# wwood/CoverM

Measured on AMD Instinct MI355X. Metric: aligned reads/s through coverm contig (mean trimmed_mean covered_fraction variance), higher is better.
Workload: dtype i32 depth / u64 sums / f32 estimators

## Files before the change

### coverm_amd/csrc/covermhip.hip

```cpp
#include "pileup_kernels.hip.h"
#include "prep_lean.hip.h"
#include "genome_kernels.hip.h"
#include "ingest_kernels.hip.h"
#include "group_kernels.hip.h"
#include "sam_kernels.hip.h"

#include <algorithm>
#include <atomic>
#include <cstddef>
#include <chrono>
#include <cstdio>
#include <dlfcn.h>
#include <functional>
#include <sched.h>
#include <cstdlib>
#include <cstring>
#include <map>
#include <mutex>
#include <string>
#include <future>
#include <thread>
#include <vector>

#include "../../include/covermhip.h"
// ... 8 lines not shown
static_assert(sizeof(cov_contig_stats) == 128 && offsetof(cov_contig_stats, sum_identity_primary) == 40 && offsetof(cov_contig_stats, win_sum_d) == 56 &&
              offsetof(cov_contig_stats, first_record) == 88 && offsetof(cov_contig_stats, win_min_d) == 104 && offsetof(cov_contig_stats, hist_len) == 112 &&
              offsetof(cov_contig_stats, hist_off) == 120, "cov_contig_stats layout");
static_assert(sizeof(cov_summary) == 32 && offsetof(cov_summary, hist_total) == 24, "cov_summary layout");
static_assert(sizeof(cov_interval) == 24 && sizeof(cov_interval_stats) == 56, "interval struct layout");
static_assert(sizeof(cov_genome_stats) == 24 && sizeof(cov_genome_stats) == sizeof(covk::DevGenomeStats) && offsetof(cov_genome_stats, genome_len) == offsetof(covk::DevGenomeStats, genome_len) &&
              offsetof(cov_genome_stats, any_nonzero) == offsetof(covk::DevGenomeStats, any_nonzero), "cov_genome_stats mirrors the device struct");
static_assert(sizeof(cov_estimator) == sizeof(covk::DevEstimator) && offsetof(cov_estimator, contig_end_exclusion) == offsetof(covk::DevEstimator, excl) &&
              offsetof(cov_estimator, trim_max) == offsetof(covk::DevEstimator, trim_max) && COV_EST_MAX == covk::EST_MAX && COV_EST_ANIR == covk::EST_ANIR, "cov_estimator mirrors the device struct");

namespace {

#define HIPCHK(call)                                                                          \
    do {                                                                                      \
        hipError_t e_ = (call);                                                               \
        if (e_ != hipSuccess) {                                                               \
            char b_[512];                                                                     \
            snprintf(b_, sizeof b_, "%s failed: %s (%s:%d)", #call, hipGetErrorString(e_), __FILE__, __LINE__); \
            s->err = b_;                                                                      \
            return COV_ERR_HIP;                                                               \
        }                                                                                     \
    } while (0)

template <typename T>
struct DevBuf {
    T *p = nullptr;
    size_t cap = 0;
    hipError_t reserve(size_t n, hipStream_t st, size_t keep = 0) {
        if (n <= cap) return hipSuccess;
        size_t nc = std::max(n, cap + cap / 2);
        T *q = nullptr;
        hipError_t e = hipMalloc(&q, nc * sizeof(T));
        if (e != hipSuccess) return e;
        if (keep && p) {
            e = hipMemcpyAsync(q, p, keep * sizeof(T), hipMemcpyDeviceToDevice, st);
            if (e != hipSuccess) return e;
            e = hipStreamSynchronize(st);
            if (e != hipSuccess) return e;
        }
        if (p) (void)hipFree(p);
        p = q; cap = nc;
        return hipSuccess;
    }
    void release() { if (p) (void)hipFree(p); p = nullptr; cap = 0; }
};

std::string g_create_error;

bool cov_timing_on() { static const bool on = getenv("COVERM_CLI_TIMING") != nullptr; return on; }

}

extern "C" int covh_timing_on(void) { return cov_timing_on() ? 1 : 0; }

struct InflateKernel { int version = 3; int lz_version = 2; u32 round_blocks = 0; u64 carry = 16ull << 20; u64 cwin = 0; u32 ext_parts = covi::EXT_PARTS; };

struct cov_session {
    cov_config cfg{};
    hipStream_t stream = nullptr;
    std::string err;
    int tile = 1024;
    bool use_fast = true;
    int chunk_tiles = 8;
    int prep_kernel = 0;
    int est_lanes = -1;
    int fast_tables = 1;
    int n_cus = 256;

    uint32_t n_targets = 0;
    std::vector<uint32_t> h_tlen;
    std::vector<uint32_t> h_tile_first;
    uint32_t n_tiles = 0;
    DevBuf<u32> d_tlen, d_tile_contig, d_tile_start;
    DevBuf<u32> d_tile_first, d_tcnt, d_fov, d_tscan, d_ttop;
    DevBuf<u32> d_slow_list;
    uint32_t tile_shift = 10;
    DevBuf<u32> d_cx_list, d_cx_cnt, d_cx_cur, d_cx_scan, d_cx_top;
    DevBuf<uint2> d_cx_runs;
    DevBuf<DevContig> d_ctg_scratch;
    DevBuf<int32_t> d_depth_all; DevBuf<u64> d_depth_off; bool depth_all_valid = false;
    DevBuf<DevInterval> d_iv; DevBuf<DevIntervalStats> d_ivst; DevBuf<unsigned long long> d_ivhist; uint64_t ivhist_total = 0;
    DevBuf<uint8_t> d_mask;
    std::vector<uint8_t> h_mask;
    bool have_mask = false;
    bool have_genomes = false, gen_valid = false;
    bool lean_finish = false;
    bool in_spill = false;
    DevBuf<u64> d_order;
    uint32_t n_genomes = 0, n_gseg = 0;
    DevBuf<u32> d_grow, d_gtids, d_gseg_genome, d_gseg_start;
    DevBuf<DevGenome> d_genomes;
    DevBuf<u64> d_ghist, d_ghist_top;
    DevBuf<uint8_t> d_gout; uint8_t *h_gout = nullptr; size_t h_gout_cap = 0;
    DevBuf<uint8_t> d_res;
    DevBuf<DevContig> d_ctg;
    DevBuf<DevGlobal> d_glob;
    DevBuf<uint4> d_desc;
    DevBuf<uint8_t> d_gather; uint8_t *h_gather = nullptr; size_t h_gather_cap = 0; uint32_t gather_n = 0; size_t gather_block = 0;

    DevBuf<int32_t> s_tid, s_pos;
    DevBuf<uint16_t> s_flag;
    DevBuf<uint8_t> s_mapq, s_nmk;
    DevBuf<u32> s_nm, s_lseq, s_coff, s_cig;
    DevBuf<int32_t> s_mtid; DevBuf<u64> s_qh1; DevBuf<u32> s_qh2;
    bool want_mates = false;
    bool want_grouping = false;
// ... 53 lines not shown
    DevBuf<u64> g_result;
    DevBuf<covi::tokpos_t> g_tok, g_tok2;
    DevBuf<u32> g_ntok, g_ntok2;
    hipStream_t ing_aux = nullptr;
    hipStream_t ing_parse = nullptr;
    hipStream_t ing_ext = nullptr;
    hipEvent_t ing_inf_done[2] = {nullptr, nullptr}, ing_lz_done[2] = {nullptr, nullptr};
    hipEvent_t ing_ver_done[4] = {}, ing_ext_done[3] = {}, ing_cdone[3] = {};
    uint64_t ing_round_start = 0, ing_prev_end = 0, ing_ccap = 0;
    uint32_t ing_round_n = 0;
    int64_t ing_copy_cleared = -1;
    long long ing_key_lo = 0, ing_key_hi = 0x80000000ll;
    bool ing_search_first = false, ing_open_end = false, ing_fed_any = false;
    uint64_t ing_span_lo = 0, ing_span_hi = 0;
    uint64_t ing_tail_key = ~0ull;
    u64 *h_winres = nullptr;
    struct WinInfo { u64 N = 0; u32 n_seg = 0; u64 comp_end = 0; };
    WinInfo ing_win[4];
    uint32_t ing_batch = 0; int ing_check_crc = 1;
    uint32_t ing_extracted = 0;
    uint64_t ing_rec_total = 0, ing_cig_total = 0;
    uint32_t ing_fail = 0;
    uint64_t ing_fail_dbg[3] = {0, 0, 0};
    uint64_t ing_first_record = 0;
    uint64_t ing_launched = 0;
    covi::BgzfBlock *h_blocks = nullptr; size_t h_blocks_cap = 0;
    uint64_t ing_comp = 0, ing_infl = 0, ing_blocks = 0;
    bool ing_active = false;
    InflateKernel ing_K;
    hipStream_t ing_copy = nullptr;
    std::future<hipError_t> ing_prep;
    hipEvent_t ing_ev[COV_INGEST_SLOTS] = {}, ing_fed = nullptr;
    double ing_s_alloc = 0;
    double ing_s_part[4] = {0, 0, 0, 0};

    bool sam_active = false, sam_seen_record = false, sam_decode_timed = false;
    uint64_t sam_window = 0, sam_expected = 0, sam_lines = 0, sam_bytes = 0, sam_err_line = 0;
    uint32_t sam_err = 0, sam_k = 0;
    DevBuf<uint8_t> m_text[2], m_blob;
    DevBuf<u64> m_nl, m_tab, m_res, m_noff;
    DevBuf<u32> m_line_end, m_cnt, m_rec_idx, m_cig_idx, m_bsum[3], m_slots;
    samc::Table m_names{};
    hipEvent_t sam_buf_free[2] = {}, sam_ev[4] = {};
    float sam_ms = 0.f; uint32_t sam_launches = 0;

    bool finished = false;
    uint8_t *h_res = nullptr; size_t h_res_cap = 0;
    std::future<std::pair<uint8_t *, size_t>> h_res_prep;
    DevContig *h_ctg = nullptr;
    DevGlobal h_glob{};
    bool last_gen_all = false;
    uint64_t algo_bytes = 0;

    hipEvent_t ev[COV_K_COUNT][2] = {};
    hipEvent_t ev_begin[COV_K_COUNT] = {};
    int ev_fresh = -1;
    float k_ms[COV_K_COUNT] = {};
    uint32_t k_launches[COV_K_COUNT] = {};
};

cov_status spill_store(cov_session *s, bool &progress);

namespace {

size_t result_block_bytes(u32 n_targets) { return sizeof(DevGlobal) + (size_t)std::max<u32>(n_targets, 1) * sizeof(DevContig); }
static size_t result_host_bytes(const cov_session *s, u32 nT) {
    return result_block_bytes(nT) + (size_t)std::max<u32>(nT, 1) * (s->have_mask ? 1u : std::max<u32>(s->est.n, 1u)) * sizeof(float);
}
static void result_host_take(cov_session *s) {
    if (!s->h_res_prep.valid()) return;
    const std::pair<uint8_t *, size_t> r = s->h_res_prep.get();
    if (!r.first) return;
    if (r.second > s->h_res_cap) {
        if (s->h_res) (void)hipHostFree(s->h_res);
        s->h_res = r.first; s->h_res_cap = r.second;
    } else (void)hipHostFree(r.first);
}

hipError_t bind_result_block(cov_session *s, u32 n_targets) {
    hipError_t e = s->d_res.reserve(result_block_bytes(n_targets) + (size_t)std::max<u32>(n_targets, 1) * COV_EST_MAX * sizeof(float), s->stream);
    if (e != hipSuccess) return e;
    s->d_glob.p = reinterpret_cast<DevGlobal *>(s->d_res.p); s->d_glob.cap = 1;
    s->d_ctg.p = reinterpret_cast<DevContig *>(s->d_res.p + sizeof(DevGlobal)); s->d_ctg.cap = std::max<u32>(n_targets, 1);
    return hipSuccess;
}

Records records_of(const cov_session *s) {
    Records r{};
    if (s->adopted) {
        const cov_batch &b = s->adopted_batch;
        r.tid = b.tid; r.pos = b.pos; r.flag = b.flag; r.mapq = b.mapq; r.nm = b.nm; r.nm_kind = b.nm_kind;
        r.l_seq = b.l_seq; r.cigar_off = b.cigar_off; r.cigar = b.cigar;
    } else {
        r.tid = s->s_tid.p; r.pos = s->s_pos.p; r.flag = s->s_flag.p; r.mapq = s->s_mapq.p; r.nm = s->s_nm.p;
        r.nm_kind = s->s_nmk.p; r.l_seq = s->s_lseq.p; r.cigar_off = s->s_coff.p; r.cigar = s->s_cig.p;
    }
    r.n = (u32)s->n_records;
    r.cigar_end = s->adopted ? s->adopted_cig_end : (u32)s->n_cigar;
    return r;
}

__global__ void k_rebase_offsets(u32 *off, u32 n, u32 sub, u32 add) {
    u32 i = blockIdx.x * blockDim.x + threadIdx.x;
    if (i < n) off[i] = off[i] - sub + add;
}

__global__ void k_count_primary(const uint16_t *__restrict__ flag, u32 lo, u32 n, unsigned long long *out) {
    u32 cnt = 0;
    for (u64 i = (u64)lo + blockIdx.x * blockDim.x + threadIdx.x; i < n; i += (u64)gridDim.x * blockDim.x) cnt += (flag[i] & 0x900u) ? 0u : 1u;
    cnt = wave_sum_u32(cnt);
    if ((threadIdx.x & 63u) == 0u && cnt) atomicAdd(out, (unsigned long long)cnt);
}

cov_status append(cov_session *s, const cov_batch *b, bool from_device) {
    const uint64_t n = b->n_records;
    if (n == 0) return COV_OK;
    const hipMemcpyKind kind = from_device ? hipMemcpyDeviceToDevice : hipMemcpyHostToDevice;
    u32 off0 = 0, offn = 0;
    if (from_device) {
        HIPCHK(hipMemcpyAsync(&off0, b->cigar_off, 4, hipMemcpyDeviceToHost, s->stream));
        HIPCHK(hipMemcpyAsync(&offn, b->cigar_off + n, 4, hipMemcpyDeviceToHost, s->stream));
        HIPCHK(hipStreamSynchronize(s->stream));
    } else {
        off0 = b->cigar_off[0]; offn = b->cigar_off[n];
    }
    const uint64_t ncig = (uint64_t)offn - off0;
    if (s->n_records && (s->n_records + n > s->cap_records || s->n_cigar + ncig > s->cap_cigar) && s->n_records >= s->spill_retry_at) {
        bool progress = false;
        const cov_status sp = spill_store(s, progress);
        if (sp != COV_OK) return sp;
        s->spill_retry_at = progress ? 0 : 2 * s->n_records;
    }
    if (s->n_records + n >= 0xfffffff0ull) { s->err = "more than 2^32 records of one reference (or of one batch) in the record store"; return COV_ERR_INVALID_ARG; }
    if (s->n_cigar + ncig >= 0xfffffff0ull) { s->err = "more than 2^32 CIGAR words of one reference (or of one batch) in the record store"; return COV_ERR_INVALID_ARG; }
    const uint64_t R = s->n_records, N = R + n;
    hipStream_t st = s->stream;
    HIPCHK(s->s_tid.reserve(N, st, R)); HIPCHK(s->s_pos.reserve(N, st, R)); HIPCHK(s->s_flag.reserve(N, st, R));
    HIPCHK(s->s_mapq.reserve(N, st, R)); HIPCHK(s->s_nmk.reserve(N, st, R)); HIPCHK(s->s_nm.reserve(N, st, R));
    HIPCHK(s->s_lseq.reserve(N, st, R)); HIPCHK(s->s_coff.reserve(N + 1, st, R + 1));
    HIPCHK(s->s_cig.reserve(s->n_cigar + ncig + 1, st, s->n_cigar));
    HIPCHK(hipMemcpyAsync(s->s_tid.p + R, b->tid, n * 4, kind, st));
    HIPCHK(hipMemcpyAsync(s->s_pos.p + R, b->pos, n * 4, kind, st));
    HIPCHK(hipMemcpyAsync(s->s_flag.p + R, b->flag, n * 2, kind, st));
    HIPCHK(hipMemcpyAsync(s->s_mapq.p + R, b->mapq, n, kind, st));
    HIPCHK(hipMemcpyAsync(s->s_nmk.p + R, b->nm_kind, n, kind, st));
    HIPCHK(hipMemcpyAsync(s->s_nm.p + R, b->nm, n * 4, kind, st));
    HIPCHK(hipMemcpyAsync(s->s_lseq.p + R, b->l_seq, n * 4, kind, st));
    HIPCHK(hipMemcpyAsync(s->s_coff.p + R, b->cigar_off, (n + 1) * 4, kind, st));
    if (ncig) HIPCHK(hipMemcpyAsync(s->s_cig.p + s->n_cigar, b->cigar + off0, ncig * 4, kind, st));
    if (off0 != (u32)s->n_cigar) {
        const u32 cnt = (u32)(n + 1);
        hipLaunchKernelGGL(k_rebase_offsets, dim3((cnt + 255) / 256), dim3(256), 0, st, s->s_coff.p + R, cnt, off0,
                           (u32)s->n_cigar);
        HIPCHK(hipGetLastError());
    }
    s->n_records = N; s->n_cigar += ncig;
    s->finished = false;
    if (!from_device) HIPCHK(hipStreamSynchronize(st));
    return COV_OK;
}

void timing_events(cov_session *s) {
    if (s->ev[0][0]) return;
    for (int k = 0; k < COV_K_COUNT; k++)
        for (int j = 0; j < 2; j++) (void)hipEventCreate(&s->ev[k][j]);
}
void time_begin(cov_session *s, int k) {
    if (s->ev_fresh >= 0) { s->ev_begin[k] = s->ev[s->ev_fresh][1]; return; }
    (void)hipEventRecord(s->ev[k][0], s->stream); s->ev_begin[k] = s->ev[k][0];
}
void time_end(cov_session *s, int k) { (void)hipEventRecord(s->ev[k][1], s->stream); s->k_launches[k]++; s->ev_fresh = k; }

template <bool H, int TABLES>
void launch_fast_v(cov_session *s, const PileupArgs &a, u32 n_tiles) {
    const auto kern = TABLES == 1 ? &k_pileup_fast<H> : &k_pileup_fast2t<H>;
    const size_t smem = pileup_fast_smem_bytes(H, TABLES == 1 ? FAST_HB : FAST_HB7, TABLES);
    static std::atomic<int> occ_dev[64];
    std::atomic<int> &occ_slot = occ_dev[(unsigned)s->cfg.device & 63u];
    int occ = occ_slot.load(std::memory_order_relaxed);
    const u32 chunk = (u32)s->chunk_tiles;
    const u32 n_chunks = (n_tiles + chunk - 1) / chunk;
    if (!occ) {
        (void)hipFuncSetAttribute(reinterpret_cast<const void *>(kern), hipFuncAttributeMaxDynamicSharedMemorySize, (int)smem);
        int nb = 0;
        if (hipOccupancyMaxActiveBlocksPerMultiprocessor(&nb, reinterpret_cast<const void *>(kern), 256, smem) != hipSuccess || nb < 1) {
            (void)hipGetLastError();
            nb = (int)std::max<size_t>(1, std::min<size_t>(8, (160 * 1024) / smem));
        }
        occ = nb; occ_slot.store(nb, std::memory_order_relaxed);
    }
    const u32 wg_per_cu = 8u * (u32)occ;
    const u32 grid = std::max(1u, std::min((n_chunks + 3) / 4, (u32)s->n_cus * wg_per_cu));
    hipLaunchKernelGGL(kern, dim3(grid), dim3(256), smem, s->stream, a, n_tiles, chunk);
}
template <bool H>
void launch_fast_t(cov_session *s, const PileupArgs &a, u32 n_tiles) {
    if (s->fast_tables == 2) launch_fast_v<H, 2>(s, a, n_tiles);
    else launch_fast_v<H, 1>(s, a, n_tiles);
}

template <bool H, bool W>
void launch_stream_t(cov_session *s, const PileupArgs &a, u32 n_tiles, bool slow_list_only = false) {
    const size_t smem = pileup_stream_smem_bytes();
    static std::atomic<int> occ_dev[64];
    std::atomic<int> &occ_slot = occ_dev[(unsigned)s->cfg.device & 63u];
    int occ = occ_slot.load(std::memory_order_relaxed);
    const u32 chunk = (u32)s->chunk_tiles;
    const u32 n_chunks = (n_tiles + chunk - 1) / chunk;
    if (!occ) {
        (void)hipFuncSetAttribute(reinterpret_cast<const void *>(&k_pileup_stream<H, W>), hipFuncAttributeMaxDynamicSharedMemorySize, (int)smem);
        int nb = 0;
        if (hipOccupancyMaxActiveBlocksPerMultiprocessor(&nb, reinterpret_cast<const void *>(&k_pileup_stream<H, W>), 256, smem) != hipSuccess || nb < 1) {
            (void)hipGetLastError();
            nb = (int)std::max<size_t>(1, std::min<size_t>(8, (160 * 1024) / smem));
        }
        occ = nb; occ_slot.store(nb, std::memory_order_relaxed);
    }
    const u32 wg_per_cu = 8u * (u32)occ;
    if (slow_list_only) {
        hipLaunchKernelGGL((k_pileup_stream<H, W>), dim3((u32)s->n_cus), dim3(256), smem, s->stream, a, 0u, 1u,
                           (const u32 *)s->d_slow_list.p, (const u32 *)&s->d_glob.p->n_slow);
        return;
    }
    const u32 grid = std::max(1u, std::min((n_chunks + 3) / 4, (u32)s->n_cus * wg_per_cu));
    hipLaunchKernelGGL((k_pileup_stream<H, W>), dim3(grid), dim3(256), smem, s->stream, a, n_tiles, chunk, (const u32 *)nullptr,
                       (const u32 *)nullptr);
}
template <bool H, bool W>
void launch_any_pileup(cov_session *s, const PileupArgs &a, u32 n_tiles) {
    if (s->use_fast && !W) {
        launch_fast_t<H>(s, a, n_tiles);
        launch_stream_t<H, W>(s, a, n_tiles, true);
    } else launch_stream_t<H, W>(s, a, n_tiles);
}

PileupArgs pileup_args(cov_session *s) {
    PileupArgs a{};
    a.tile_contig = s->d_tile_contig.p; a.tile_start = s->d_tile_start.p; a.desc = s->d_desc.p;
    a.runs = s->d_runs.p; a.cx_runs = s->d_cx_runs.p; a.r = records_of(s); a.ctg = s->d_ctg.p; a.g = s->d_glob.p;
    a.hist_arena = s->d_arena.p; a.excl = s->cfg.contig_end_exclusion; a.depth_out = nullptr; a.tile_base = 0;
    return a;
}

}

extern "C" {

int cov_abi_version(void) { return COVERMHIP_ABI_VERSION; }

const char *cov_last_error(const cov_session *s) { return s ? s->err.c_str() : g_create_error.c_str(); }

static hipError_t ingest_prepare_(cov_session *s) {
    hipError_t e = hipSetDevice(s->cfg.device);
    if (e != hipSuccess || s->ing_copy) return e;
#define PREP(x) do { e = (x); if (e != hipSuccess) return e; } while (0)
    PREP(hipStreamCreateWithFlags(&s->ing_copy, hipStreamNonBlocking));
    for (int k = 0; k < COV_INGEST_SLOTS; k++) PREP(hipEventCreateWithFlags(&s->ing_ev[k], hipEventDisableTiming));
    PREP(hipEventCreateWithFlags(&s->ing_fed, hipEventDisableTiming));
    PREP(hipStreamCreateWithFlags(&s->ing_aux, hipStreamNonBlocking));
    PREP(hipStreamCreateWithFlags(&s->ing_parse, hipStreamNonBlocking));
    s->ing_ext = s->ing_parse;
    for (int k = 0; k < 2; k++) { PREP(hipEventCreateWithFlags(&s->ing_inf_done[k], hipEventDisableTiming)); PREP(hipEventCreateWithFlags(&s->ing_lz_done[k], hipEventDisableTiming)); }
    for (int k = 0; k < 4; k++) PREP(hipEventCreateWithFlags(&s->ing_ver_done[k], hipEventDisableTiming));
    for (int k = 0; k < 3; k++) { PREP(hipEventCreateWithFlags(&s->ing_ext_done[k], hipEventDisableTiming)); PREP(hipEventCreateWithFlags(&s->ing_cdone[k], hipEventDisableTiming)); }
    PREP(hipHostMalloc((void **)&s->h_winres, 4 * 8 * sizeof(u64), hipHostMallocDefault));
    {
        const size_t nc = (size_t)3 << 19;
        PREP(hipHostMalloc((void **)&s->h_blocks, nc * sizeof(covi::BgzfBlock), hipHostMallocDefault));
        s->h_blocks_cap = nc;
    }
    {
        static const std::vector<u32> crc_tables = [] { std::vector<u32> t(covi::crcw::TABLE_WORDS); covi::crcw::build_tables(t.data()); return t; }();
        PREP(s->g_crc_tab.reserve(covi::crcw::TABLE_WORDS, s->ing_copy));
        PREP(hipMemcpyAsync(s->g_crc_tab.p, crc_tables.data(), covi::crcw::TABLE_WORDS * sizeof(u32), hipMemcpyHostToDevice, s->ing_copy));
        PREP(hipStreamSynchronize(s->ing_copy));
    }
#undef PREP
    return hipSuccess;
}
static hipError_t ingest_prep_wait(cov_session *s) { return s->ing_prep.valid() ? s->ing_prep.get() : hipSuccess; }

cov_status cov_create(const cov_config *cfg, cov_session **out) {
    if (!cfg || !out) { g_create_error = "null argument"; return COV_ERR_INVALID_ARG; }
    *out = nullptr;
    const bool timing = cov_timing_on();
    const auto tc0 = std::chrono::steady_clock::now();
    auto stamp = [&](const char *what) { if (timing) fprintf(stderr, "[covermhip] cov_create: %s at %.4fs\n", what, std::chrono::duration<double>(std::chrono::steady_clock::now() - tc0).count()); };
    int ndev = 0;
    hipError_t e = hipGetDeviceCount(&ndev);
    stamp("hipGetDeviceCount (runtime initialised)");
    if (e != hipSuccess || ndev <= 0) {
        g_create_error = std::string("no usable HIP device: ") + hipGetErrorString(e) +
                         " (the engine has no CPU fallback)";
// ... 45 lines not shown
void cov_destroy(cov_session *s) {
    if (!s) return;
    (void)ingest_prep_wait(s);
    (void)hipSetDevice(s->cfg.device);
    if (s->stream) (void)hipStreamSynchronize(s->stream);
    s->d_tlen.release(); s->d_tile_contig.release(); s->d_tile_start.release(); s->d_mask.release();
    s->d_grow.release(); s->d_gtids.release(); s->d_gseg_genome.release(); s->d_gseg_start.release(); s->d_genomes.release(); s->d_ghist.release(); s->d_ghist_top.release(); s->d_order.release();
    s->d_gout.release(); if (s->h_gout) (void)hipHostFree(s->h_gout); s->h_gout = nullptr;
    s->d_tile_first.release(); s->d_tcnt.release(); s->d_fov.release(); s->d_tscan.release(); s->d_ttop.release(); s->d_slow_list.release();
    s->d_ctg_scratch.release(); s->d_depth_all.release(); s->d_depth_off.release(); s->d_iv.release(); s->d_ivst.release(); s->d_ivhist.release();
    s->d_cx_list.release(); s->d_cx_cnt.release(); s->d_cx_cur.release(); s->d_cx_scan.release(); s->d_cx_top.release(); s->d_cx_runs.release();
    if (s->side) {
        (void)hipStreamSynchronize(s->side);
        if (s->side_owned) (void)hipStreamDestroy(s->side);
        s->side = nullptr; s->side_owned = false;
    }
    if (s->ing_aux) (void)hipStreamSynchronize(s->ing_aux);
    if (s->ing_parse) (void)hipStreamSynchronize(s->ing_parse);
    if (s->ing_ext) (void)hipStreamSynchronize(s->ing_ext);
    ingest_free_buffers(s);
    s->g_result.release();
    if (s->ing_aux) (void)hipStreamDestroy(s->ing_aux);
    if (s->ing_parse) (void)hipStreamDestroy(s->ing_parse);
    for (int k = 0; k < 2; k++) { if (s->ing_inf_done[k]) (void)hipEventDestroy(s->ing_inf_done[k]); if (s->ing_lz_done[k]) (void)hipEventDestroy(s->ing_lz_done[k]); }
    for (int k = 0; k < 4; k++) if (s->ing_ver_done[k]) (void)hipEventDestroy(s->ing_ver_done[k]);
    for (int k = 0; k < 3; k++) { if (s->ing_ext_done[k]) (void)hipEventDestroy(s->ing_ext_done[k]); if (s->ing_cdone[k]) (void)hipEventDestroy(s->ing_cdone[k]); }
    if (s->h_winres) (void)hipHostFree(s->h_winres);
    s->h_winres = nullptr;
    if (s->h_blocks) (void)hipHostFree(s->h_blocks);
    s->h_blocks = nullptr;
    if (s->ing_copy) { (void)hipStreamSynchronize(s->ing_copy); (void)hipStreamDestroy(s->ing_copy); }
    for (int k = 0; k < COV_INGEST_SLOTS; k++) if (s->ing_ev[k]) (void)hipEventDestroy(s->ing_ev[k]);
    for (hipEvent_t e : s->sam_buf_free) if (e) (void)hipEventDestroy(e);
    for (hipEvent_t e : s->sam_ev) if (e) (void)hipEventDestroy(e);
    for (auto &b : s->m_text) b.release();
    s->m_blob.release(); s->m_nl.release(); s->m_tab.release(); s->m_res.release(); s->m_noff.release(); s->m_line_end.release(); s->m_cnt.release();
    s->m_rec_idx.release(); s->m_cig_idx.release(); s->m_slots.release(); for (auto &b : s->m_bsum) b.release();
    if (s->ing_fed) (void)hipEventDestroy(s->ing_fed);
    s->d_res.release(); s->d_ctg.p = nullptr; s->d_glob.p = nullptr; s->d_desc.release(); s->d_gather.release();
    if (s->h_gather) (void)hipHostFree(s->h_gather);
    s->h_gather = nullptr;
    result_host_take(s);
    if (s->h_res) (void)hipHostFree(s->h_res);
    s->h_res = nullptr; s->h_res_cap = 0; s->h_ctg = nullptr;
    if (s->h_chist) (void)hipHostFree(s->h_chist);
    s->h_chist = nullptr; s->h_chist_cap = 0;
    s->h_estf = nullptr; s->d_spill_tmp.release();
    s->s_tid.release(); s->s_pos.release(); s->s_flag.release(); s->s_mapq.release(); s->s_nmk.release();
    s->s_nm.release(); s->s_lseq.release(); s->s_coff.release(); s->s_cig.release();
    s->s_mtid.release(); s->s_qh1.release(); s->s_qh2.release();
    s->d_runs.release(); s->d_part.release(); s->d_prep_args.release(); s->d_gen_list.release(); s->d_hist_top.release(); s->d_ident.release(); s->d_identp.release(); s->d_idch.release();
    if (s->ev_prep_done) (void)hipEventDestroy(s->ev_prep_done);
    if (s->ev_side_done) (void)hipEventDestroy(s->ev_side_done); s->d_arena.release(); s->d_chist.release(); s->d_depth.release();
    for (int k = 0; k < COV_K_COUNT; k++)
        for (int j = 0; j < 2; j++) if (s->ev[k][j]) (void)hipEventDestroy(s->ev[k][j]);
    if (s->stream) (void)hipStreamDestroy(s->stream);
    delete s;
}

static void genomes_off(cov_session *s) {
    if (s->have_genomes && (s->cfg.want & COV_WANT_IDENTITY_NONSUPP_ONLY))
        for (uint32_t k = 0; k < s->est.n; k++)
            if (s->est.e[k].kind == COV_EST_ANIR) { s->est = EstParams{}; s->est_valid = false; break; }
    s->have_genomes = false; s->gen_valid = false;
}
cov_status cov_set_targets(cov_session *s, uint32_t n_targets, const uint64_t *target_len) {
    if (!s || (!target_len && n_targets)) return COV_ERR_INVALID_ARG;
    HIPCHK(hipSetDevice(s->cfg.device));
    s->n_targets = n_targets;
    s->h_tlen.resize(n_targets);
    s->h_tile_first.assign((size_t)n_targets + 1, 0);
    uint64_t nt = 0;
    for (uint32_t c = 0; c < n_targets; c++) {
        if (target_len[c] > 0x7fffffffull) { s->err = "target length exceeds BAM's i32 range"; return COV_ERR_INVALID_ARG; }
        s->h_tlen[c] = (uint32_t)target_len[c];
        s->h_tile_first[c] = (uint32_t)nt;
        nt += (target_len[c] + (uint64_t)s->tile - 1) / (uint64_t)s->tile;
    }
    if (nt >= 0x7fffffffull) { s->err = "too many tiles"; return COV_ERR_INVALID_ARG; }
    s->h_tile_first[n_targets] = (uint32_t)nt;
    s->n_tiles = (uint32_t)nt;
    std::vector<u32> tc(nt), ts(nt);
    for (uint32_t c = 0; c < n_targets; c++) {
        u32 k = s->h_tile_first[c];
        for (uint64_t p = 0; p < target_len[c]; p += (uint64_t)s->tile, k++) { tc[k] = c; ts[k] = (u32)p; }
    }
    HIPCHK(s->d_tlen.reserve(std::max<size_t>(1, n_targets), s->stream));
    HIPCHK(s->d_tile_contig.reserve(std::max<size_t>(1, nt), s->stream));
    HIPCHK(s->d_tile_start.reserve(std::max<size_t>(1, nt), s->stream));
    HIPCHK(s->d_desc.reserve(std::max<size_t>(2, 2 * nt), s->stream));
    HIPCHK(s->d_tile_first.reserve((size_t)n_targets + 1, s->stream));
    HIPCHK(s->d_tcnt.reserve(std::max<size_t>(1, nt), s->stream)); HIPCHK(s->d_fov.reserve(std::max<size_t>(1, nt), s->stream));
    HIPCHK(s->d_tscan.reserve(std::max<size_t>(1, nt), s->stream)); HIPCHK(s->d_ttop.reserve(nt / 1024 + 2, s->stream));
    HIPCHK(s->d_slow_list.reserve(std::max<size_t>(1, nt), s->stream));
    HIPCHK(s->d_cx_cnt.reserve(std::max<size_t>(1, nt), s->stream)); HIPCHK(s->d_cx_cur.reserve(std::max<size_t>(1, nt), s->stream));
    HIPCHK(s->d_cx_scan.reserve(std::max<size_t>(1, nt), s->stream)); HIPCHK(s->d_cx_top.reserve(nt / 1024 + 2, s->stream));
    HIPCHK(hipMemcpyAsync(s->d_tile_first.p, s->h_tile_first.data(), ((size_t)n_targets + 1) * 4, hipMemcpyHostToDevice, s->stream));
    s->tile_shift = 0;
    while ((1u << s->tile_shift) < (uint32_t)s->tile) s->tile_shift++;
    HIPCHK(bind_result_block(s, n_targets));
    if (n_targets) HIPCHK(hipMemcpyAsync(s->d_tlen.p, s->h_tlen.data(), (size_t)n_targets * 4, hipMemcpyHostToDevice, s->stream));
    if (nt) {
        HIPCHK(hipMemcpyAsync(s->d_tile_contig.p, tc.data(), nt * 4, hipMemcpyHostToDevice, s->stream));
        HIPCHK(hipMemcpyAsync(s->d_tile_start.p, ts.data(), nt * 4, hipMemcpyHostToDevice, s->stream));
    }
    HIPCHK(hipStreamSynchronize(s->stream));
    s->have_mask = false;
    genomes_off(s);
// ... 275 lines not shown
        uint64_t prim = 0, cons = 0;
        for (u32 k = 0; k < COUNTER_SLOTS * 8; k++) { prim += G.prim_slots[k]; cons += G.cons_slots[k]; }
        summary->num_detected_primary_alignments = prim; summary->n_records = n_records; summary->n_considered = cons; summary->hist_total = 0;
    }
    return COV_OK;
}

static cov_status finish_once(cov_session *s, cov_contig_stats *stats, cov_summary *summary, bool &again);

static cov_status finish_store(cov_session *s, cov_contig_stats *stats, cov_summary *summary) {
    bool again = false;
    cov_status st = finish_once(s, stats, summary, again);
    if (st == COV_OK && again) st = finish_once(s, stats, summary, again);
    if (st == COV_OK && again) { s->err = "internal error: bucket sizing did not converge"; return COV_ERR_STATE; }
    return st;
}

static cov_status merge_spilled(cov_session *s, cov_contig_stats *stats, cov_summary *summary);

cov_status cov_finish(cov_session *s, cov_contig_stats *stats, cov_summary *summary) {
    covr::Range rr("cov_finish");
    if (s) s->merged_valid = false;
    cov_summary local;
    cov_status st = finish_store(s, stats, (s && s->spill.active && !summary) ? &local : summary);
    if (st == COV_OK && s->spill.active) st = merge_spilled(s, stats, summary ? summary : &local);
    return st;
}

cov_status cov_finish_genomes(cov_session *s, cov_summary *summary) {
    covr::Range rr("cov_finish_genomes");
    if (!s) return COV_ERR_INVALID_ARG;
    s->merged_valid = false;
    if (s->spill.active) { s->err = "cov_finish_genomes: part of the sample's contigs left the bounded record store: cov_finish, and aggregate on the host"; return COV_ERR_STATE; }
    s->lean_finish = true;
    const cov_status st = finish_store(s, nullptr, summary);
    s->lean_finish = false;
    return st;
}

static cov_status finish_once(cov_session *s, cov_contig_stats *stats, cov_summary *summary, bool &again) {
    again = false;
    if (!s || (!stats && s->n_targets && !s->lean_finish)) return COV_ERR_INVALID_ARG;
    const bool lean = s->lean_finish;
    s->depth_all_valid = false;
    HIPCHK(hipSetDevice(s->cfg.device));
    timing_events(s);
    hipStream_t st = s->stream;
    const u32 nT = s->n_targets;
    const u32 R = (u32)s->n_records;
    const bool want_hist = s->cfg.want & COV_WANT_HIST, want_id = s->cfg.want & COV_WANT_IDENTITY;
    for (int k = 0; k < COV_K_COUNT; k++) { s->k_launches[k] = 0; s->k_ms[k] = 0.f; }
    bool compacted = false;
    s->est_valid = false; s->gen_valid = false;
    s->ev_fresh = -1;

    HIPCHK(s->d_runs.reserve(std::max<size_t>(1, R), st));
    const uint64_t ncig_all = s->adopted ? s->adopted_ncig : s->n_cigar;
    const bool long_cigars = R && ncig_all / R >= 16;
    const int prep_kernel = s->prep_kernel;
    const int prep_passes = long_cigars ? 1 : 2 * PREP_PASSES, prep_b = 1;
    const u32 prep_chunk = (u32)(256 * prep_b * prep_passes);
    const u32 prep_grid = (R + prep_chunk - 1) / prep_chunk;
    HIPCHK(s->d_part.reserve((size_t)prep_grid + 2, st));
    if (want_id) {
        if (!(s->cfg.want & COV_WANT_IDENTITY_PRIMARY_ONLY)) HIPCHK(s->d_ident.reserve(std::max<size_t>(1, R), st));
        if (!(s->cfg.want & COV_WANT_IDENTITY_NONSUPP_ONLY)) HIPCHK(s->d_identp.reserve(std::max<size_t>(1, R), st));
        HIPCHK(s->d_idch.reserve((size_t)R / ID_CH + 2, st));
    }
    if (want_hist) HIPCHK(s->d_arena.reserve((size_t)R + nT + 1, st));

    TileIdx ti{};
    ti.tile_first = s->d_tile_first.p; ti.tcnt = s->d_tcnt.p; ti.fov = s->d_fov.p; ti.shift = s->tile_shift; ti.n_tiles = s->n_tiles;
    CxIdx cx{};
    {
        const uint64_t ncig_now = s->adopted ? s->adopted_ncig : s->n_cigar;
        HIPCHK(s->d_cx_list.reserve((size_t)(ncig_now / CX_MIN_OPS) + 64, st));
        cx.list = s->d_cx_list.p; cx.list_cap = (u32)std::min<uint64_t>(ncig_now / CX_MIN_OPS + 64, 0xffffffffull);
        cx.cnt = s->d_cx_cnt.p; cx.cur = s->d_cx_cur.p; cx.cscan = s->d_cx_scan.p; cx.ctop = s->d_cx_top.p;
        cx.runs = s->d_cx_runs.p; cx.runs_cap = s->d_cx_runs.cap;
    }
    const Records r = records_of(s);
    const uint8_t *mask = s->have_mask ? s->d_mask.p : nullptr;
    FilterCfg f{};
    f.include_improper_pairs = s->cfg.include_improper_pairs; f.include_supplementary = s->cfg.include_supplementary;
    f.include_secondary = s->cfg.include_secondary; f.filter_single = s->cfg.filter_single;
    f.min_mapq = s->cfg.min_mapq; f.min_aligned_length = s->cfg.min_aligned_length;
    f.min_percent_identity = s->cfg.min_percent_identity; f.min_aligned_percent = s->cfg.min_aligned_percent;
    double *idp = (want_id && !(s->cfg.want & COV_WANT_IDENTITY_NONSUPP_ONLY)) ? s->d_identp.p : nullptr;
    double *idn = (want_id && !(s->cfg.want & COV_WANT_IDENTITY_PRIMARY_ONLY)) ? s->d_ident.p : nullptr;
    HIPCHK(s->d_prep_args.reserve(1, st));
    HIPCHK(s->d_gen_list.reserve((size_t)R / 64 + 2, st));
    PrepArgs pa{};
    {
        PrepHot &ph = pa.hot;
        ph.tid = r.tid; ph.pos = r.pos; ph.flag = r.flag; ph.nmk = r.nm_kind; ph.nm = r.nm; ph.coff = r.cigar_off; ph.cigar = r.cigar; ph.mapq = r.mapq; ph.lseq = r.l_seq;
        ph.runs = s->d_runs.p; ph.tcnt = ti.tcnt; ph.fov = ti.fov; ph.identp = idp; ph.identn = idn;
        ph.n = r.n; ph.cigar_end = r.cigar_end; ph.n_targets = nT; ph.shift = ti.shift; ph.steps = (u32)prep_chunk / 256u;
        ph.gate_mask = 0x4u | (f.include_secondary ? 0u : 0x100u) | (f.include_supplementary ? 0u : 0x800u) | (f.include_improper_pairs ? 0u : 0x2u);
        ph.p1_mask = 0x4u | (f.include_secondary ? 0u : 0x100u) | (f.include_supplementary ? 0u : 0x800u);
        ph.min_mapq = f.min_mapq; ph.min_aligned_length = f.min_aligned_length; ph.min_percent_identity = f.min_percent_identity; ph.min_aligned_percent = f.min_aligned_percent;
        PrepCold &pc = pa.cold;
        pc.ctg = s->d_ctg.p; pc.g = s->d_glob.p; pc.part = s->d_part.p; pc.cx_list = cx.list; pc.mask = mask; pc.tlen = s->d_tlen.p; pc.tile_first = s->d_tile_first.p;
        pc.cx_list_cap = cx.list_cap; pc.gen_list = s->d_gen_list.p;
    }
    hipLaunchKernelGGL(k_init, dim3((std::max(std::max(nT, COUNTER_SLOTS * 8), s->n_tiles) + 255) / 256), dim3(256), 0, st, s->d_ctg.p,
                       nT, s->d_glob.p, ti, cx, s->d_prep_args.p, pa);
    HIPCHK(hipGetLastError());

    if (R) {
        time_begin(s, COV_K_PREP);
        const u32 n_steps = (R + 63u) / 64u;
        const bool gen_all = prep_kernel != 7 && (uint64_t)R < (uint64_t)nT * 128u;
        s->last_gen_all = gen_all;
        const u32 gen_grid = gen_all ? std::min<u32>((u32)s->n_cus * 64u, (n_steps + 3u) / 4u) : std::min<u32>((u32)s->n_cus * 8u, (n_steps + 3u) / 4u);
#define COV_LAUNCH_PREP(ID, FI, MA)                                                                                                       \
        do {                                                                                                                              \
            if (prep_kernel == 7)                                                                                                         \
                hipLaunchKernelGGL((k_prep7s<ID, FI, MA>), dim3(prep_grid), dim3(256), 0, st, r, s->d_tlen.p, nT, mask, f, s->d_ctg.p,   \
                                   s->d_glob.p, s->d_runs.p, idp, idn, s->d_part.p, ti, prep_passes, prep_b, cx.list, cx.list_cap);      \
            else if (gen_all)                                                                                                             \
                hipLaunchKernelGGL((k_prep_generic<ID, FI, MA>), dim3(gen_grid), dim3(256), 0, st, (const PrepArgs *)s->d_prep_args.p, n_steps); \
            else {                                                                                                                        \
                hipLaunchKernelGGL((k_prep_lean<ID, FI, MA>), dim3(prep_grid), dim3(256), 0, st, pa.hot, (const PrepArgs *)s->d_prep_args.p); \
                hipLaunchKernelGGL((k_prep_generic<ID, FI, MA>), dim3(gen_grid), dim3(256), 0, st, (const PrepArgs *)s->d_prep_args.p, 0u); \
            }                                                                                                                             \
        } while (0)
        {
            const int key = (want_id ? 4 : 0) | (s->cfg.filter_single ? 2 : 0) | (mask != nullptr ? 1 : 0);
            switch (key) {
            case 0: COV_LAUNCH_PREP(false, false, false); break;
            case 1: COV_LAUNCH_PREP(false, false, true); break;
            case 2: COV_LAUNCH_PREP(false, true, false); break;
            case 3: COV_LAUNCH_PREP(false, true, true); break;
            case 4: COV_LAUNCH_PREP(true, false, false); break;
            case 5: COV_LAUNCH_PREP(true, false, true); break;
            case 6: COV_LAUNCH_PREP(true, true, false); break;
            default: COV_LAUNCH_PREP(true, true, true); break;
            }
        }
#undef COV_LAUNCH_PREP
        if (nT) {
            const u32 n_red = gen_all ? 0u : (nT + 3u) / 4u, cx_grid0 = (u32)s->n_cus * 8u;
            hipLaunchKernelGGL(k_post_prep, dim3(n_red + cx_grid0), dim3(256), 0, st, r, s->d_tlen.p, s->d_glob.p, cx, ti, s->d_ctg.p, nT, (const PrepPartial *)s->d_part.p,
                               prep_grid, prep_chunk, n_red);
        }
        time_end(s, COV_K_PREP);
        HIPCHK(hipGetLastError());
        if (want_id && nT) {
            if (!s->side) {
                (void)ingest_prep_wait(s);
                if (s->ing_aux && !s->ing_active) s->side = s->ing_aux;
                else { HIPCHK(hipStreamCreateWithFlags(&s->side, hipStreamNonBlocking)); s->side_owned = true; }
            }
            HIPCHK(hipEventRecord(s->ev_prep_done, st));
            HIPCHK(hipStreamWaitEvent(s->side, s->ev_prep_done, 0));
            (void)hipEventRecord(s->ev[COV_K_IDENTITY][0], s->side);
            if (s->id_mode) {
                const u32 nch = (R + ID_CH - 1) / ID_CH;
                hipLaunchKernelGGL(k_id_approx, dim3(nch), dim3(256), 0, s->side, idp, idn, R, s->d_idch.p);
                hipLaunchKernelGGL(k_id_predict, dim3(nT), dim3(64), 0, s->side, s->d_ctg.p, nT, idp, idn, s->d_idch.p);
                hipLaunchKernelGGL(k_id_exact, dim3(nch), dim3(256), 0, s->side, idp, idn, R, s->d_idch.p);
                hipLaunchKernelGGL(k_id_combine, dim3(nT), dim3(64), 0, s->side, s->d_ctg.p, nT, idp, idn, r.tid, s->d_idch.p);
            } else
                hipLaunchKernelGGL(k_identity, dim3(nT), dim3(64), 0, s->side, s->d_ctg.p, nT, idp, idn, r.tid);
            (void)hipEventRecord(s->ev[COV_K_IDENTITY][1], s->side);
            s->k_launches[COV_K_IDENTITY]++;
            HIPCHK(hipGetLastError());
            HIPCHK(hipEventRecord(s->ev_side_done, s->side));
            s->ev_fresh = -1;
        }
    }
    if (R && s->n_tiles) {
        time_begin(s, COV_K_RANGES);
        const u32 n_blocks = (s->n_tiles + 1023u) / 1024u;
        const u32 cx_grid = (u32)s->n_cus * 8u;
        ScanPair sp{};
        sp.cnt[0] = s->d_tcnt.p; sp.scan[0] = s->d_tscan.p; sp.top[0] = s->d_ttop.p; sp.total[0] = nullptr;
        sp.cnt[1] = s->d_cx_cnt.p; sp.scan[1] = s->d_cx_scan.p; sp.top[1] = s->d_cx_top.p; sp.total[1] = &s->d_glob.p->cx_total;
        hipLaunchKernelGGL(k_tile_scan1, dim3(2u * n_blocks), dim3(1024), 0, st, sp, s->n_tiles, n_blocks);
        hipLaunchKernelGGL(k_tile_scan2, dim3(2), dim3(1024), 0, st, sp, n_blocks);
        hipLaunchKernelGGL((k_cx_expand<true>), dim3(cx_grid), dim3(256), 0, st, r, s->d_tlen.p, s->d_glob.p, cx, ti);
        u32 *slow_list = s->use_fast ? s->d_slow_list.p : nullptr;
        if (want_hist)
            hipLaunchKernelGGL((k_ranges<true>), dim3((s->n_tiles + 255) / 256), dim3(256), 0, st, s->d_tile_contig.p,
                               s->d_tile_start.p, s->n_tiles, s->d_tlen.p, mask, s->d_ctg.p, s->d_desc.p, ti, s->d_tscan.p,
                               s->d_ttop.p, cx, s->d_glob.p, slow_list);
        else
            hipLaunchKernelGGL((k_ranges<false>), dim3((s->n_tiles + 255) / 256), dim3(256), 0, st, s->d_tile_contig.p,
                               s->d_tile_start.p, s->n_tiles, s->d_tlen.p, mask, s->d_ctg.p, s->d_desc.p, ti, s->d_tscan.p,
                               s->d_ttop.p, cx, s->d_glob.p, slow_list);
        time_end(s, COV_K_RANGES);
        HIPCHK(hipGetLastError());
        if (want_hist) {
            time_begin(s, COV_K_HIST);
            const u32 hb = (nT + 1023u) / 1024u;
            HIPCHK(s->d_hist_top.reserve(hb, st));
            hipLaunchKernelGGL((k_hist_sum<0>), dim3(hb), dim3(1024), 0, st, (const DevContig *)s->d_ctg.p, nT, s->d_tlen.p, mask, (u64)s->cfg.contig_end_exclusion, s->d_hist_top.p);
            hipLaunchKernelGGL((k_hist_off<0>), dim3(hb), dim3(1024), 0, st, s->d_ctg.p, nT, s->d_tlen.p, mask, (u64)s->cfg.contig_end_exclusion, (const u64 *)s->d_hist_top.p, s->d_glob.p);
            hipLaunchKernelGGL(k_zero_u32, dim3(2048), dim3(256), 0, st, s->d_arena.p, &s->d_glob.p->hist_cap_total);
            time_end(s, COV_K_HIST);
            HIPCHK(hipGetLastError());
        }
        PileupArgs a = pileup_args(s);
        time_begin(s, COV_K_PILEUP);
        if (want_hist) launch_any_pileup<true, false>(s, a, s->n_tiles);
        else launch_any_pileup<false, false>(s, a, s->n_tiles);
        time_end(s, COV_K_PILEUP);
        HIPCHK(hipGetLastError());
        if (want_hist) {
            compacted = s->est.n == 0 || s->hist_fetch_seen;
            s->hist_prefetched = 0;
            if (compacted) {
                HIPCHK(s->d_chist.reserve((size_t)R + nT + 1, st));
                time_begin(s, COV_K_HIST_COMPACT);
                const u32 hb = (nT + 1023u) / 1024u;
                hipLaunchKernelGGL((k_hist_sum<1>), dim3(hb), dim3(1024), 0, st, (const DevContig *)s->d_ctg.p, nT, s->d_tlen.p, mask, (u64)s->cfg.contig_end_exclusion, s->d_hist_top.p);
                hipLaunchKernelGGL((k_hist_off<1>), dim3(hb), dim3(1024), 0, st, s->d_ctg.p, nT, s->d_tlen.p, mask, (u64)s->cfg.contig_end_exclusion, (const u64 *)s->d_hist_top.p, s->d_glob.p);
                hipLaunchKernelGGL(k_hist_compact, dim3((nT + 3u) / 4u), dim3(256), 0, st, s->d_ctg.p, nT, s->d_tlen.p, (u64)s->cfg.contig_end_exclusion, s->d_arena.p, s->d_chist.p);
                time_end(s, COV_K_HIST_COMPACT);
                HIPCHK(hipGetLastError());
                const u64 guess = s->hist_fetch_seen ? std::min<u64>({s->last_chist_total + s->last_chist_total / 16, (u64)R + nT + 1, (u64)(64u << 20) / 8}) : 0;
                if (guess) {
                    if (guess > s->h_chist_cap) {
                        if (s->h_chist) (void)hipHostFree(s->h_chist);
                        s->h_chist = nullptr; s->h_chist_cap = 0;
                        HIPCHK(hipHostMalloc((void **)&s->h_chist, (size_t)guess * 8, hipHostMallocDefault));
                        s->h_chist_cap = guess;
                    }
                    HIPCHK(hipMemcpyAsync(s->h_chist, s->d_chist.p, (size_t)guess * 8, hipMemcpyDeviceToHost, st));
                    s->hist_prefetched = guess;
                }
            }
            s->hist_fetch_seen = false;
        }
    }
    const size_t block = result_block_bytes(nT), nf = s->have_mask ? 0 : (size_t)nT * s->est.n;
    {
        result_host_take(s);
        const size_t need = lean ? sizeof(DevGlobal) + sizeof(DevContig) : result_host_bytes(s, nT);
        if (need > s->h_res_cap) {
            if (s->h_res) (void)hipHostFree(s->h_res);
            s->h_res = nullptr; s->h_res_cap = 0;
            const size_t cap = need < ((size_t)64 << 20) ? need + need / 2 : need;
            HIPCHK(hipHostMalloc((void **)&s->h_res, cap, hipHostMallocDefault));
            s->h_res_cap = cap;
        }
        s->h_ctg = (DevContig *)(s->h_res + sizeof(DevGlobal));
        s->h_estf = reinterpret_cast<float *>(s->h_res + block);
    }
    if (want_id && R && nT) { HIPCHK(hipStreamWaitEvent(st, s->ev_side_done, 0)); s->ev_fresh = -1; }
    if (nf) {
        time_begin(s, COV_K_ESTIMATE);
        if (s->est_lanes < 0 ? nT >= 65536u : s->est_lanes == 1)
            hipLaunchKernelGGL(k_estimate_lanes, dim3((nT + 255) / 256), dim3(256), 0, st, (const DevContig *)s->d_ctg.p, nT, (const u32 *)s->d_tlen.p, (u64)s->cfg.contig_end_exclusion,
                               (const u32 *)s->d_arena.p, s->est, reinterpret_cast<float *>(s->d_res.p + block));
        else
            hipLaunchKernelGGL(k_estimate, dim3((nT + 3) / 4), dim3(256), 0, st, (const DevContig *)s->d_ctg.p, nT, (const u32 *)s->d_tlen.p, (u64)s->cfg.contig_end_exclusion,
                               (const u32 *)s->d_arena.p, s->est, reinterpret_cast<float *>(s->d_res.p + block));
        time_end(s, COV_K_ESTIMATE);
        HIPCHK(hipGetLastError());
    }
    const bool genomes = s->have_genomes && s->est.n != 0 && !s->spill.active && !s->in_spill;
    if (lean && !genomes) { s->err = "cov_finish_genomes: cov_set_genomes and cov_set_estimators first, and no spill of the bounded record store (cov_finish then)"; return COV_ERR_STATE; }
    if (genomes) {
        const u32 nG = s->n_genomes, n_seg = s->n_gseg;
        GenomeTable gt{s->d_grow.p, s->d_gtids.p, s->d_gseg_genome.p, s->d_gseg_start.p, nG, n_seg};
        const u64 excl = s->cfg.contig_end_exclusion;
        const u64 ghist_cap = (u64)R + nT + 1;
        if (want_hist) HIPCHK(s->d_ghist.reserve((size_t)ghist_cap, st));
        time_begin(s, COV_K_GENOME);
        hipLaunchKernelGGL(k_genome_init, dim3((nG + 255u) / 256u), dim3(256), 0, st, s->d_genomes.p, nG);
        if (n_seg) hipLaunchKernelGGL(k_genome_reduce, dim3((n_seg + 3u) / 4u), dim3(256), 0, st, (const DevContig *)s->d_ctg.p, (const u32 *)s->d_tlen.p, excl, gt, s->d_genomes.p);
        if (want_id && !(s->cfg.want & COV_WANT_IDENTITY_PRIMARY_ONLY))
            hipLaunchKernelGGL(k_genome_identity, dim3(nG), dim3(64), 0, st, (const DevContig *)s->d_ctg.p, gt, s->d_genomes.p);
        if (want_hist) {
            const u32 gb = (nG + 1023u) / 1024u;
            u64 *total = s->d_ghist_top.p + gb;
            hipLaunchKernelGGL(k_genome_hist_sum, dim3(gb), dim3(1024), 0, st, (const DevGenome *)s->d_genomes.p, nG, s->d_ghist_top.p);
            hipLaunchKernelGGL(k_genome_hist_off, dim3(gb), dim3(1024), 0, st, s->d_genomes.p, nG, (const u64 *)s->d_ghist_top.p, total, ghist_cap, s->d_glob.p);
            hipLaunchKernelGGL(k_zero_u64, dim3(1024), dim3(256), 0, st, s->d_ghist.p, (const u64 *)total, ghist_cap);
            if (n_seg && R && s->n_tiles)
                hipLaunchKernelGGL(k_genome_hist_merge, dim3((n_seg + 3u) / 4u), dim3(256), 0, st, (const DevContig *)s->d_ctg.p, (const u32 *)s->d_tlen.p, excl,
                                   (const u32 *)s->d_arena.p, gt, (const DevGenome *)s->d_genomes.p, s->d_ghist.p, ghist_cap);
        }
        DevGenomeStats *gstats = reinterpret_cast<DevGenomeStats *>(s->d_gout.p);
        float *gest = reinterpret_cast<float *>(s->d_gout.p + (size_t)nG * sizeof(DevGenomeStats));
        if (nG >= 65536u)
            hipLaunchKernelGGL(k_genome_estimate_lanes, dim3((nG + 255u) / 256u), dim3(256), 0, st, (const DevGenome *)s->d_genomes.p, nG, (const u64 *)s->d_ghist.p, s->est, gest, gstats);
        else
            hipLaunchKernelGGL(k_genome_estimate, dim3((nG + 3u) / 4u), dim3(256), 0, st, (const DevGenome *)s->d_genomes.p, nG, (const u64 *)s->d_ghist.p, s->est, gest, gstats);
        time_end(s, COV_K_GENOME);
        HIPCHK(hipGetLastError());
        HIPCHK(hipMemcpyAsync(s->h_gout, s->d_gout.p, (size_t)nG * (sizeof(DevGenomeStats) + s->est.n * sizeof(float)), hipMemcpyDeviceToHost, st));
    }
    if (lean) {
        const u32 ob = (nT + 1023u) / 1024u;
        HIPCHK(s->d_order.reserve((size_t)ob + 2, st));
        hipLaunchKernelGGL(k_order_max, dim3(std::max(ob, 1u)), dim3(1024), 0, st, (const DevContig *)s->d_ctg.p, nT, s->d_order.p);
        hipLaunchKernelGGL(k_order_check, dim3(std::max(ob, 1u)), dim3(1024), 0, st, (const DevContig *)s->d_ctg.p, nT, s->d_order.p);
        HIPCHK(hipGetLastError());
        HIPCHK(hipMemcpyAsync(s->h_res, s->d_res.p, sizeof(DevGlobal), hipMemcpyDeviceToHost, st));
        HIPCHK(hipMemcpyAsync(s->h_res + sizeof(DevGlobal), s->d_order.p, 8, hipMemcpyDeviceToHost, st));
    } else
    HIPCHK(hipMemcpyAsync(s->h_res, s->d_res.p, sizeof(DevGlobal) + (size_t)nT * sizeof(DevContig) + (nf ? (block - sizeof(DevGlobal) - (size_t)nT * sizeof(DevContig)) + nf * sizeof(float) : 0),
                          hipMemcpyDeviceToHost, st));
    {
        const auto t_spin = std::chrono::steady_clock::now();
        for (;;) {
            const hipError_t q = hipStreamQuery(st);
            if (q == hipSuccess) break;
            if (q != hipErrorNotReady) { (void)hipGetLastError(); break; }
            (void)hipGetLastError();
            if (std::chrono::steady_clock::now() - t_spin > std::chrono::milliseconds(4)) break;
            __builtin_ia32_pause();
        }
    }
    HIPCHK(hipStreamSynchronize(st));
    memcpy(&s->h_glob, s->h_res, sizeof(DevGlobal));
    if (s->h_glob.cx_total > s->d_cx_runs.cap) {
        const uint64_t need = s->h_glob.cx_total + s->h_glob.cx_total / 8 + 1024;
        s->d_cx_runs.release();
        HIPCHK(s->d_cx_runs.reserve((size_t)need, st));
        again = true;
        return COV_OK;
    }
    for (int k = 0; k < COV_K_COUNT; k++)
        if (s->k_launches[k]) (void)hipEventElapsedTime(&s->k_ms[k], k == COV_K_IDENTITY ? s->ev[k][0] : s->ev_begin[k], s->ev[k][1]);

    {
        const uint64_t ncig = s->adopted ? s->adopted_ncig : s->n_cigar;
        s->algo_bytes = (uint64_t)R * 24 + ncig * 4 + (uint64_t)nT * sizeof(DevContig);
    }

    if (lean) {
        u64 unsorted_at; memcpy(&unsorted_at, s->h_res + sizeof(DevGlobal), 8);
        const cov_status cst = verdict_results(s, s->h_glob, unsorted_at, R, summary);
        if (cst != COV_OK) return cst;
        s->last_chist_total = 0; s->hist_compacted = false; s->est_valid = false; s->gen_valid = true; s->finished = true;
        return COV_OK;
    }
    const cov_status cst = convert_results(s, s->h_glob, s->h_ctg, R, stats, summary, s->spill.inflight, s->spill.records);
    if (cst != COV_OK) return cst;
    s->last_chist_total = 0;
    if (want_hist) for (u32 c = 0; c < nT; c++) s->last_chist_total += stats[c].hist_len;
    s->hist_compacted = compacted;
    s->est_valid = s->est.n != 0 && !s->have_mask;
    s->gen_valid = genomes;
    s->finished = true;
    return COV_OK;
}


static cov_status fetch_chunk_hist(cov_session *s, uint64_t *hist);

extern "C++" {
namespace {
template <typename T>
cov_status move_front(cov_session *s, T *p, size_t from, size_t n) {
    if (!n || !from) return COV_OK;
    hipStream_t st = s->stream;
    if (n <= from) { HIPCHK(hipMemcpyAsync(p, p + from, n * sizeof(T), hipMemcpyDeviceToDevice, st)); return COV_OK; }
    HIPCHK(s->d_spill_tmp.reserve(n * sizeof(T), st));
    HIPCHK(hipMemcpyAsync(s->d_spill_tmp.p, p + from, n * sizeof(T), hipMemcpyDeviceToDevice, st));
    HIPCHK(hipMemcpyAsync(p, s->d_spill_tmp.p, n * sizeof(T), hipMemcpyDeviceToDevice, st));
    return COV_OK;
}

cov_status spill_store_impl(cov_session *s, bool &progress) {
    progress = false;
    if (s->adopted || s->n_records == 0 || s->want_mates || s->n_targets == 0) return COV_OK;
    covr::Range rr("bounded store: spill");
    const u32 nT = s->n_targets;
    const bool want_hist = s->cfg.want & COV_WANT_HIST;
    std::vector<cov_contig_stats> st(nT);
    cov_summary sm{};
    s->in_spill = true;
    const bool lean_was = s->lean_finish; s->lean_finish = false;
    cov_status rc = finish_store(s, st.data(), &sm);
    s->in_spill = false; s->lean_finish = lean_was;
    if (rc != COV_OK) return rc;
    const u64 R = s->n_records;
    cov_session::Spill &S = s->spill;
    int64_t cstar = -1; u64 best = 0;
    for (u32 c = 0; c < nT; c++)
        if (st[c].n_pass && (cstar < 0 || st[c].last_record >= best)) { cstar = c; best = st[c].last_record; }
    const u64 keep_from = cstar >= 0 ? st[cstar].first_record - S.records : R;
    if (keep_from == 0) { s->finished = false; return COV_OK; }
    if (!S.active) { S.stats.assign(nT, cov_contig_stats{}); S.ctg.assign(nT, DevContig{}); S.have.assign(nT, 0); S.active = true; }
    std::vector<uint64_t> h;
    if (want_hist && sm.hist_total) { h.resize(sm.hist_total); rc = fetch_chunk_hist(s, h.data()); if (rc != COV_OK) return rc; }
    for (u32 c = 0; c < nT; c++) {
        if ((int64_t)c == cstar || !st[c].n_pass) continue;
        if (S.have[c]) { s->err = "BAM file appears to be unsorted. Input BAM files must be sorted by reference (i.e. by samtools sort)"; return COV_ERR_UNSORTED; }
        S.stats[c] = st[c]; S.ctg[c] = s->h_ctg[c]; S.have[c] = 1;
        if (s->est.n && !s->have_mask) {
            if (s->spill_est.size() != (size_t)nT * s->est.n) s->spill_est.assign((size_t)nT * s->est.n, 0.0f);
            memcpy(&s->spill_est[(size_t)c * s->est.n], s->h_estf + (size_t)c * s->est.n, s->est.n * sizeof(float));
// ... 953 lines not shown
                HIPCHK(d_pairs.reserve(pairs.size(), st));
                HIPCHK(hipMemcpyAsync(d_pairs.p, pairs.data(), pairs.size() * sizeof(uint2), hipMemcpyHostToDevice, st));
                hipLaunchKernelGGL(covp::k_pair_judge_list, dim3((u32)((pairs.size() + 255) / 256)), dim3(256), 0, st, C, (const uint2 *)d_pairs.p, (u32)pairs.size(), F, d_partner.p,
                                   d_w.p + 1, (u32)COV_ERR_NM_MISSING, (u32)COV_ERR_NM_BADTYPE);
                HIPCHK(hipGetLastError());
                HIPCHK(hipStreamSynchronize(st));
            }
        }
    }
    const u32 nb = (R + covp::SCAN_BLOCK - 1) / covp::SCAN_BLOCK;
    HIPCHK(d_bsum.reserve((size_t)nb + 1, st));
    const covp::PairSlots slots{d_partner.p};
    hipLaunchKernelGGL((covp::k_scan_sums<covp::PairSlots>), dim3(nb), dim3(256), 0, st, slots, R, d_bsum.p);
    hipLaunchKernelGGL(covp::k_scan_offsets, dim3(1), dim3(1024), 0, st, d_bsum.p, nb, d_w.p + 2);
    HIPCHK(hipGetLastError());
    u64 hw[4];
    HIPCHK(hipMemcpyAsync(hw, d_w.p, sizeof hw, hipMemcpyDeviceToHost, st));
    HIPCHK(hipStreamSynchronize(st));
    if (hw[1] != ~0ull) {
        const u32 code = (u32)(hw[1] & 0xffu);
        s->err = code == (u32)COV_ERR_NM_MISSING ? "Mapping record encountered that does not have an 'NM' auxiliary tag in the SAM/BAM format" : "Unexpected data type of NM aux tag";
        return (cov_status)code;
    }
    const u64 n_sel = hw[2];
    if (n_primary) *n_primary = hw[0];
    if (n_selected) *n_selected = n_sel;
    if (n_sel == 0) { s->n_records = 0; s->n_cigar = 0; s->mates_valid = 0; return COV_OK; }
    const u32 S = (u32)n_sel;
    HIPCHK(d_order.reserve(S, st));
    const covp::PairEmit emit{d_partner.p, d_order.p};
    hipLaunchKernelGGL((covp::k_scan_apply<covp::PairSlots, covp::PairEmit>), dim3(nb), dim3(256), 0, st, slots, emit, R, (const u32 *)d_bsum.p);
    HIPCHK(hipGetLastError());
    { const cov_status g = gather_store(s, d_order.p, S, false); if (g != COV_OK) return g; }
    s->mates_valid = 0;
    return COV_OK;
}

cov_status cov_group_records(cov_session *s, uint64_t *n_moved) {
    if (!s) return COV_ERR_INVALID_ARG;
    covr::Range rr("group records by reference (cov_group_records)");
    if (n_moved) *n_moved = 0;
    if (s->ing_active) { s->err = "cov_group_records: a device ingest is still open (cov_ingest_end first)"; return COV_ERR_STATE; }
    if (s->adopted) { s->err = "cov_group_records: needs the session's own record store, not an adopted device batch (cov_push_batch_device)"; return COV_ERR_STATE; }
    if (s->ing_was_span) { s->err = "cov_group_records: the store holds one tid span of a file (cov_ingest_span), which is cut where a file sorted by reference changes tid"; return COV_ERR_STATE; }
    if (s->spill.active) { s->err = "cov_group_records: a sample that is not sorted by reference must fit the record store (part of it already left the bounded store, judged in file order)"; return COV_ERR_STATE; }
    HIPCHK(hipSetDevice(s->cfg.device));
    timing_events(s);
    hipStream_t st = s->stream;
    const u32 R = (u32)s->n_records, nT = s->n_targets;
    for (float &m : s->grp_ms) m = 0.f;
    s->grp_launches = 0;
    if (R < 2) return COV_OK;
    const bool mates = s->mates_valid == s->n_records && s->mates_valid != 0;
    hipEvent_t *ev = s->ev[COV_K_GROUP];
    hipEvent_t ev_mid[2] = {nullptr, nullptr};
    DevBuf<u32> d_flag, d_hist, d_key[2], d_idx[2]; DevBuf<u64> d_cnt;
    struct Rel { std::function<void()> f; ~Rel() { f(); } } rel{[&] {
        d_flag.release(); d_hist.release(); d_key[0].release(); d_key[1].release(); d_idx[0].release(); d_idx[1].release(); d_cnt.release();
        for (hipEvent_t e : ev_mid) if (e) (void)hipEventDestroy(e); }};
    for (hipEvent_t &e : ev_mid) HIPCHK(hipEventCreate(&e));
    auto elapsed = [&](hipEvent_t a, hipEvent_t b) { float ms = 0.f; (void)hipEventElapsedTime(&ms, a, b); return ms; };

    HIPCHK(d_flag.reserve(1, st));
    HIPCHK(hipMemsetAsync(d_flag.p, 0, sizeof(u32), st));
    HIPCHK(hipEventRecord(ev[0], st));
    hipLaunchKernelGGL(covg::k_group_check, dim3(std::min<u32>((R + 255u) / 256u, 8192u)), dim3(256), 0, st, (const int32_t *)s->s_tid.p, R, nT, d_flag.p);
    HIPCHK(hipGetLastError());
    HIPCHK(hipEventRecord(ev_mid[0], st));
    s->grp_launches++;
    u32 decreasing = 0;
    HIPCHK(hipMemcpyAsync(&decreasing, d_flag.p, sizeof decreasing, hipMemcpyDeviceToHost, st));
    HIPCHK(hipStreamSynchronize(st));
    s->grp_ms[1] = elapsed(ev[0], ev_mid[0]);
    if (!decreasing) { s->grp_ms[0] = s->grp_ms[1]; return COV_OK; }

    const u32 P = grpk::n_passes(nT), n_wg = grpk::n_tiles(R), n_hist = n_wg * grpk::RADIX;
    const u32 nb = (n_hist + covp::SCAN_BLOCK - 1) / covp::SCAN_BLOCK;
    DevBuf<u32> d_bsum;
    struct Rel1 { DevBuf<u32> &a; ~Rel1() { a.release(); } } rel1{d_bsum};
    HIPCHK(d_hist.reserve(n_hist, st)); HIPCHK(d_bsum.reserve((size_t)nb + 1, st)); HIPCHK(d_cnt.reserve(2, st));
    HIPCHK(d_idx[0].reserve(R, st));
    if (P > 1) { HIPCHK(d_key[0].reserve(R, st)); HIPCHK(d_idx[1].reserve(R, st)); }
    if (P > 2) HIPCHK(d_key[1].reserve(R, st));
    HIPCHK(hipMemsetAsync(d_cnt.p, 0, 2 * sizeof(u64), st));
    const int32_t *tid = s->s_tid.p;
    for (u32 p = 0; p < P; p++) {
        const bool first = p == 0, last = p + 1 == P;
        const u32 *key_in = first ? nullptr : d_key[(p - 1) & 1u].p, *idx_in = first ? nullptr : d_idx[(p - 1) & 1u].p;
        u32 *key_out = last ? nullptr : d_key[p & 1u].p, *idx_out = d_idx[p & 1u].p;
        if (first) hipLaunchKernelGGL(covg::k_group_hist<true>, dim3(n_wg), dim3(256), 0, st, tid, key_in, R, nT, p, d_hist.p, n_wg);
        else hipLaunchKernelGGL(covg::k_group_hist<false>, dim3(n_wg), dim3(256), 0, st, tid, key_in, R, nT, p, d_hist.p, n_wg);
        const covg::HistVal hv{d_hist.p}; const covg::HistPut hp{d_hist.p};
        hipLaunchKernelGGL((covp::k_scan_sums<covg::HistVal>), dim3(nb), dim3(256), 0, st, hv, n_hist, d_bsum.p);
        hipLaunchKernelGGL(covp::k_scan_offsets, dim3(1), dim3(1024), 0, st, d_bsum.p, nb, d_cnt.p + 1);
        hipLaunchKernelGGL((covp::k_scan_apply<covg::HistVal, covg::HistPut>), dim3(nb), dim3(256), 0, st, hv, hp, n_hist, (const u32 *)d_bsum.p);
        const dim3 g(n_wg), b(256);
        if (first && last) hipLaunchKernelGGL((covg::k_group_scatter<true, true>), g, b, 0, st, tid, key_in, idx_in, key_out, idx_out, R, nT, p, (const u32 *)d_hist.p, n_wg);
        else if (first) hipLaunchKernelGGL((covg::k_group_scatter<true, false>), g, b, 0, st, tid, key_in, idx_in, key_out, idx_out, R, nT, p, (const u32 *)d_hist.p, n_wg);
        else if (last) hipLaunchKernelGGL((covg::k_group_scatter<false, true>), g, b, 0, st, tid, key_in, idx_in, key_out, idx_out, R, nT, p, (const u32 *)d_hist.p, n_wg);
        else hipLaunchKernelGGL((covg::k_group_scatter<false, false>), g, b, 0, st, tid, key_in, idx_in, key_out, idx_out, R, nT, p, (const u32 *)d_hist.p, n_wg);
        HIPCHK(hipGetLastError());
        s->grp_launches += 5;
    }
    const u32 *order = d_idx[(P - 1) & 1u].p;
    hipLaunchKernelGGL(covg::k_group_moved, dim3(std::min<u32>((R + 255u) / 256u, 4096u)), dim3(256), 0, st, order, R, d_cnt.p);
    HIPCHK(hipGetLastError());
    HIPCHK(hipEventRecord(ev_mid[1], st));
    s->grp_launches++;
    { const cov_status g = gather_store(s, order, R, mates); if (g != COV_OK) return g; }
    HIPCHK(hipEventRecord(ev[1], st));
    s->grp_launches += mates ? 4 : 3;
    u64 moved = 0;
    HIPCHK(hipMemcpyAsync(&moved, d_cnt.p, sizeof moved, hipMemcpyDeviceToHost, st));
    HIPCHK(hipStreamSynchronize(st));
    s->grp_ms[0] = elapsed(ev[0], ev[1]); s->grp_ms[2] = elapsed(ev_mid[0], ev_mid[1]); s->grp_ms[3] = elapsed(ev_mid[1], ev[1]);
    if (cov_timing_on())
        fprintf(stderr, "[covermhip] group: %u records, %u passes, %llu moved; order check %.3f ms, sort %.3f ms, gather %.3f ms\n", R, P, (unsigned long long)moved, s->grp_ms[1], s->grp_ms[2],
                s->grp_ms[3]);
    if (n_moved) *n_moved = moved;
    s->finished = false; s->depth_all_valid = false; s->ev_fresh = -1;
    return COV_OK;
}

cov_status cov_copy_records(cov_session *s, const cov_batch *host, uint64_t *n_records, uint64_t *n_cigar) {
    if (!s || s->adopted) return COV_ERR_STATE;
    if (s->spill.active) { s->err = "cov_copy_records: part of the sample's records already left the bounded record store"; return COV_ERR_STATE; }
    HIPCHK(hipSetDevice(s->cfg.device));
    if (n_records) *n_records = s->n_records;
    if (n_cigar) *n_cigar = s->n_cigar;
    if (!host) return COV_OK;
    const uint64_t n = s->n_records;
    hipStream_t st = s->stream;
    if (n) {
        HIPCHK(hipMemcpyAsync((void *)host->tid, s->s_tid.p, n * 4, hipMemcpyDeviceToHost, st));
        HIPCHK(hipMemcpyAsync((void *)host->pos, s->s_pos.p, n * 4, hipMemcpyDeviceToHost, st));
        HIPCHK(hipMemcpyAsync((void *)host->flag, s->s_flag.p, n * 2, hipMemcpyDeviceToHost, st));
        HIPCHK(hipMemcpyAsync((void *)host->mapq, s->s_mapq.p, n, hipMemcpyDeviceToHost, st));
        HIPCHK(hipMemcpyAsync((void *)host->nm, s->s_nm.p, n * 4, hipMemcpyDeviceToHost, st));
        HIPCHK(hipMemcpyAsync((void *)host->nm_kind, s->s_nmk.p, n, hipMemcpyDeviceToHost, st));
        HIPCHK(hipMemcpyAsync((void *)host->l_seq, s->s_lseq.p, n * 4, hipMemcpyDeviceToHost, st));
        HIPCHK(hipMemcpyAsync((void *)host->cigar_off, s->s_coff.p, (n + 1) * 4, hipMemcpyDeviceToHost, st));
        if (s->n_cigar) HIPCHK(hipMemcpyAsync((void *)host->cigar, s->s_cig.p, s->n_cigar * 4, hipMemcpyDeviceToHost, st));
    }
    HIPCHK(hipStreamSynchronize(st));
    return COV_OK;
}

cov_status cov_copy_mates(cov_session *s, int32_t *mtid, uint64_t *qh1, uint32_t *qh2) {
    if (!s || s->adopted || !mtid || !qh1 || !qh2) return COV_ERR_STATE;
    if (s->spill.active) { s->err = "cov_copy_mates: part of the sample's records already left the bounded record store"; return COV_ERR_STATE; }
    const uint64_t n = s->n_records;
    if (!s->want_mates || (n && (!s->s_mtid.p || !s->s_qh1.p || !s->s_qh2.p))) { s->err = "cov_copy_mates: the records were not ingested with cov_ingest_want_mates"; return COV_ERR_STATE; }
    HIPCHK(hipSetDevice(s->cfg.device));
    if (n) {
        HIPCHK(hipMemcpyAsync(mtid, s->s_mtid.p, n * 4, hipMemcpyDeviceToHost, s->stream));
        HIPCHK(hipMemcpyAsync(qh1, s->s_qh1.p, n * 8, hipMemcpyDeviceToHost, s->stream));
        HIPCHK(hipMemcpyAsync(qh2, s->s_qh2.p, n * 4, hipMemcpyDeviceToHost, s->stream));
    }
    HIPCHK(hipStreamSynchronize(s->stream));
    return COV_OK;
}

cov_status cov_ingest_release(cov_session *s) {
    if (!s) return COV_ERR_INVALID_ARG;
    HIPCHK(hipSetDevice(s->cfg.device));
    HIPCHK(hipStreamSynchronize(s->stream));
    if (s->ing_aux) HIPCHK(hipStreamSynchronize(s->ing_aux));
    if (s->ing_parse) HIPCHK(hipStreamSynchronize(s->ing_parse));
    if (s->ing_ext) HIPCHK(hipStreamSynchronize(s->ing_ext));
    ingest_free_buffers(s);
    return COV_OK;
}

cov_status cov_ingest_copy_inflated(cov_session *s, uint64_t offset, uint64_t n, void *out) {
    if (!s || offset + n > s->ing_infl || (n && !out)) return COV_ERR_INVALID_ARG;
    if (s->ing_batch != 1) { s->err = "cov_ingest_copy_inflated: the file was parsed in several windows, the stream is gone"; return COV_ERR_STATE; }
    HIPCHK(hipSetDevice(s->cfg.device));
    HIPCHK(hipMemcpyAsync(out, s->g_win[0].p + inflate_kernel(s).carry + offset, n, hipMemcpyDeviceToHost, s->stream));
    HIPCHK(hipStreamSynchronize(s->stream));
    return COV_OK;
}

cov_status cov_fetch_hist(cov_session *s, uint64_t *hist) {
    if (!s || !s->finished || !(s->cfg.want & COV_WANT_HIST)) return COV_ERR_STATE;
    if (s->merged_valid) {
        s->hist_fetch_seen = true;
        if (s->merged_hist.empty()) return COV_OK;
        if (!hist) return COV_ERR_INVALID_ARG;
        memcpy(hist, s->merged_hist.data(), s->merged_hist.size() * 8);
        return COV_OK;
    }
    return fetch_chunk_hist(s, hist);
}

static cov_status fetch_chunk_hist(cov_session *s, uint64_t *hist) {
    if (!s || !s->finished || !(s->cfg.want & COV_WANT_HIST)) return COV_ERR_STATE;
    HIPCHK(hipSetDevice(s->cfg.device));
    const uint64_t total = s->last_chist_total;
    s->hist_fetch_seen = true;
    if (total == 0) return COV_OK;
    if (!hist) return COV_ERR_INVALID_ARG;
    if (!s->hist_compacted) {
        HIPCHK(s->d_chist.reserve(total, s->stream));
        const uint8_t *mask = s->have_mask ? (const uint8_t *)s->d_mask.p : (const uint8_t *)nullptr;
        const u32 hb = (s->n_targets + 1023u) / 1024u;
        HIPCHK(s->d_hist_top.reserve(hb, s->stream));
        hipLaunchKernelGGL((k_hist_sum<1>), dim3(hb), dim3(1024), 0, s->stream, (const DevContig *)s->d_ctg.p, s->n_targets, s->d_tlen.p, mask, (u64)s->cfg.contig_end_exclusion, s->d_hist_top.p);
        hipLaunchKernelGGL((k_hist_off<1>), dim3(hb), dim3(1024), 0, s->stream, s->d_ctg.p, s->n_targets, s->d_tlen.p, mask, (u64)s->cfg.contig_end_exclusion, (const u64 *)s->d_hist_top.p, s->d_glob.p);
        hipLaunchKernelGGL(k_hist_compact, dim3((s->n_targets + 3u) / 4u), dim3(256), 0, s->stream, s->d_ctg.p, s->n_targets, s->d_tlen.p,
                           (u64)s->cfg.contig_end_exclusion, s->d_arena.p, s->d_chist.p);
        HIPCHK(hipGetLastError());
        s->hist_prefetched = 0; s->hist_compacted = true;
    }
    const u64 have = std::min<u64>(total, s->hist_prefetched);
    if (have) memcpy(hist, s->h_chist, (size_t)have * 8);
    if (have < total) {
        HIPCHK(hipMemcpyAsync(hist + have, s->d_chist.p + have, (size_t)(total - have) * 8, hipMemcpyDeviceToHost, s->stream));
        HIPCHK(hipStreamSynchronize(s->stream));
    }
    return COV_OK;
}

cov_status cov_copy_depth(cov_session *s, uint32_t tid, int32_t *depth_out) {
    if (!s || !s->finished) return COV_ERR_STATE;
    if (s->spill.active) { s->err = "cov_copy_depth: part of the sample's records already left the bounded record store"; return COV_ERR_STATE; }
    if (tid >= s->n_targets || !depth_out) return COV_ERR_INVALID_ARG;
    HIPCHK(hipSetDevice(s->cfg.device));
    const u32 L = s->h_tlen[tid];
    if (L == 0) return COV_OK;
    HIPCHK(s->d_depth.reserve(L, s->stream));
    HIPCHK(hipMemsetAsync(s->d_depth.p, 0, (size_t)L * 4, s->stream));
    PileupArgs a = pileup_args(s);
    DevBuf<DevContig> &scratch = s->d_ctg_scratch;
    HIPCHK(scratch.reserve(s->n_targets, s->stream));
    HIPCHK(hipMemcpyAsync(scratch.p, s->d_ctg.p, (size_t)s->n_targets * sizeof(DevContig), hipMemcpyDeviceToDevice, s->stream));
    a.ctg = scratch.p;
    a.depth_out = s->d_depth.p;
    a.tile_base = s->h_tile_first[tid];
    const u32 grid = s->h_tile_first[tid + 1] - s->h_tile_first[tid];
    launch_any_pileup<false, true>(s, a, grid);
    HIPCHK(hipGetLastError());
    HIPCHK(hipMemcpyAsync(depth_out, s->d_depth.p, (size_t)L * 4, hipMemcpyDeviceToHost, s->stream));
    HIPCHK(hipStreamSynchronize(s->stream));
    return COV_OK;
}

cov_status cov_interval_stats_compute(cov_session *s, const cov_interval *iv, uint64_t n, uint64_t excl, int want_hist,
                                      cov_interval_stats *out, uint64_t *hist_total) {
    if (!s || !s->finished) return COV_ERR_STATE;
    if (s->spill.active) { s->err = "cov_interval_stats_compute: part of the sample's records already left the bounded record store (per-gene coverage needs them all: raise COVERM_STORE_CAP_*)"; return COV_ERR_STATE; }
    if ((n && (!iv || !out))) return COV_ERR_INVALID_ARG;
    if (hist_total) *hist_total = 0;
    s->ivhist_total = 0;
    if (n == 0) return COV_OK;
    for (uint64_t i = 0; i < n; i++)
        if (iv[i].tid >= s->n_targets || iv[i].start >= iv[i].end || iv[i].end > s->h_tlen[iv[i].tid]) {
            s->err = "interval outside its target"; return COV_ERR_INVALID_ARG;
        }
    HIPCHK(hipSetDevice(s->cfg.device));
    hipStream_t st = s->stream;
    if (!s->depth_all_valid) {
        std::vector<u64> off((size_t)s->n_targets + 1, 0);
        for (u32 c = 0; c < s->n_targets; c++) off[c + 1] = off[c] + s->h_tlen[c];
// ... 79 lines not shown
cov_status cov_set_estimators(cov_session *s, const cov_estimator *est, uint32_t n_est) {
    if (!s || (n_est && !est)) return COV_ERR_INVALID_ARG;
    if (n_est > COV_EST_MAX) { s->err = "cov_set_estimators: more than COV_EST_MAX estimators"; return COV_ERR_INVALID_ARG; }
    if (s->spill.active) { s->err = "cov_set_estimators: set them before the sample's first records (part of it already left the bounded record store)"; return COV_ERR_STATE; }
    for (uint32_t k = 0; k < n_est; k++) {
        const int kind = est[k].kind;
        if (kind < 0 || kind > COV_EST_ANIR || kind == COV_EST_TPM || kind == COV_EST_PILEUP_COUNTS) {
            s->err = "cov_set_estimators: this estimator is evaluated on the host (TPM: f64 exp / ln of the host's libm; coverage histogram: prints the histogram itself)";
            return COV_ERR_INVALID_ARG;
        }
        if (kind == COV_EST_TRIMMED_MEAN && !(s->cfg.want & COV_WANT_HIST)) { s->err = "cov_set_estimators: a trimmed mean needs COV_WANT_HIST"; return COV_ERR_INVALID_ARG; }
        if (kind == COV_EST_ANIR && s->have_genomes) {
            if (!(s->cfg.want & COV_WANT_IDENTITY) || (s->cfg.want & COV_WANT_IDENTITY_PRIMARY_ONLY)) {
                s->err = "cov_set_estimators: ANIr of a genome needs COV_WANT_IDENTITY with the not-supplementary sum"; return COV_ERR_INVALID_ARG;
            }
        } else if (kind == COV_EST_ANIR && (!(s->cfg.want & COV_WANT_IDENTITY) || (s->cfg.want & COV_WANT_IDENTITY_NONSUPP_ONLY))) {
            s->err = "cov_set_estimators: ANIr needs COV_WANT_IDENTITY with the primary-read sum"; return COV_ERR_INVALID_ARG;
        }
    }
    s->est = EstParams{};
    for (uint32_t k = 0; k < n_est; k++) memcpy(&s->est.e[k], &est[k], sizeof(cov_estimator));
    s->est.n = n_est;
    s->est_valid = false; s->gen_valid = false;
    return COV_OK;
}

static cov_status genome_fetch_ready(cov_session *s, const char *what) {
    if (!s) return COV_ERR_INVALID_ARG;
    if (s->spill.active) { s->err = std::string(what) + ": part of the sample's contigs left the bounded record store: aggregate cov_finish's per-contig results on the host"; return COV_ERR_STATE; }
    if (!s->finished || !s->gen_valid) { s->err = std::string(what) + ": cov_set_genomes and cov_set_estimators, then cov_finish"; return COV_ERR_STATE; }
    return COV_OK;
}
cov_status cov_fetch_genome_estimates(cov_session *s, float *out) {
    const cov_status r = genome_fetch_ready(s, "cov_fetch_genome_estimates");
    if (r != COV_OK) return r;
    const size_t nf = (size_t)s->n_genomes * s->est.n;
    if (nf && !out) return COV_ERR_INVALID_ARG;
    if (nf) memcpy(out, s->h_gout + (size_t)s->n_genomes * sizeof(cov_genome_stats), nf * sizeof(float));
    return COV_OK;
}
cov_status cov_fetch_genome_stats(cov_session *s, cov_genome_stats *out) {
    const cov_status r = genome_fetch_ready(s, "cov_fetch_genome_stats");
    if (r != COV_OK) return r;
    if (!out) return COV_ERR_INVALID_ARG;
    memcpy(out, s->h_gout, (size_t)s->n_genomes * sizeof(cov_genome_stats));
    return COV_OK;
}

cov_status cov_fetch_estimates(cov_session *s, float *out) {
    if (!s || !s->finished || !s->est_valid) { if (s) s->err = "cov_fetch_estimates: cov_set_estimators, then cov_finish"; return COV_ERR_STATE; }
    if (s->have_mask) { s->err = "cov_fetch_estimates: with a target mask the entries are genomes: aggregate on the host"; return COV_ERR_STATE; }
    const size_t nf = (size_t)s->n_targets * s->est.n;
    if (nf && !out) return COV_ERR_INVALID_ARG;
    if (nf) memcpy(out, s->h_estf, nf * sizeof(float));
    return COV_OK;
}

cov_status cov_algorithmic_bytes(const cov_session *s, uint64_t *bytes) {
    if (!s || !bytes) return COV_ERR_INVALID_ARG;
    *bytes = s->algo_bytes;
    return COV_OK;
}

namespace {
struct HostPool {
    std::mutex m;
    std::map<void *, size_t> live;
    std::multimap<size_t, void *> parked;
    static size_t round_up(size_t b) { const size_t g = (size_t)16 << 20; return b < g ? g : (b + g - 1) / g * g; }
};
HostPool g_host_pool;
}

void *cov_host_alloc(size_t bytes) {
    const size_t want = HostPool::round_up(bytes);
    {
        std::lock_guard<std::mutex> lk(g_host_pool.m);
        auto it = g_host_pool.parked.lower_bound(want);
        if (it != g_host_pool.parked.end() && it->first <= 2 * want) {
            void *p = it->second; const size_t sz = it->first;
            g_host_pool.parked.erase(it);
            g_host_pool.live[p] = sz;
            return p;
        }
    }
    void *p = nullptr;
    if (hipHostMalloc(&p, want, hipHostMallocPortable) != hipSuccess) { (void)hipGetLastError(); return nullptr; }
    std::lock_guard<std::mutex> lk(g_host_pool.m);
    g_host_pool.live[p] = want;
    return p;
}

int cov_host_free(void *p) {
    if (!p) return 0;
    std::lock_guard<std::mutex> lk(g_host_pool.m);
    auto it = g_host_pool.live.find(p);
    if (it == g_host_pool.live.end()) return 0;
    g_host_pool.parked.emplace(it->second, p);
    g_host_pool.live.erase(it);
    return 1;
}

cov_status cov_host_register(cov_session *s, void *p, size_t bytes) {
    if (!s || !p || !bytes) return COV_ERR_INVALID_ARG;
    HIPCHK(hipSetDevice(s->cfg.device));
    const hipError_t e = hipHostRegister(p, bytes, hipHostRegisterDefault);
// ... 58 lines not shown
```

### coverm_amd/csrc/genome_kernels.hip.h

```cpp
#pragma once
#include "pileup_kernels.hip.h"

namespace covk {

constexpr u32 GENOME_SEG = 256;

struct DevGenome {
    u64 reads;
    u64 sum_nm, sum_indel;
    u64 sum_d, sum_d2, cov_win, cov_full;
    u64 win_len, full_len, proc_win;
    u64 unobs_win, unobs_full;
    double id;
    u64 hist_off;
    u32 min_d, nh;
    u32 n_seen, pad;
};
static_assert(sizeof(DevGenome) == 128, "DevGenome layout");

struct DevGenomeStats { u64 reads_in_genome, genome_len; u32 n_contigs_seen, any_nonzero; };

struct GenomeTable {
    const u32 *row;
    const u32 *tids;
    const u32 *seg_genome;
    const u32 *seg_start;
    u32 n_genomes, n_seg;
};

__global__ __launch_bounds__(256) void k_genome_init(DevGenome *__restrict__ G, u32 n_genomes) {
    const u32 g = blockIdx.x * 256u + threadIdx.x;
    if (g >= n_genomes) return;
    DevGenome z{};
    z.min_d = 0xffffffffu;
    G[g] = z;
}

__global__ __launch_bounds__(256) void k_genome_reduce(const DevContig *__restrict__ ctg, const u32 *__restrict__ tlen, u64 excl, GenomeTable T,
                                                       DevGenome *__restrict__ G) {
    const u32 sg = blockIdx.x * 4u + (threadIdx.x >> 6);
    if (sg >= T.n_seg) return;
    const u32 g = T.seg_genome[sg], lo = T.seg_start[sg], hi = min(lo + GENOME_SEG, T.row[g + 1]);
    u64 reads = 0, sum_nm = 0, sum_indel = 0, sum_d = 0, sum_d2 = 0, cov_win = 0, cov_full = 0, win_len = 0, full_len = 0, proc_win = 0, uw = 0, uf = 0;
    u32 min_d = 0xffffffffu, nh = 0, n_seen = 0;
    for (u32 i = lo + (u32)lane_id(); i < hi; i += 64u) {
        const u32 c = T.tids[i];
        const DevContig *C = &ctg[c];
        const u64 L = tlen[c];
        if (C->n_pass == 0) {
            uf += L; uw += L < 2 * excl ? L : L - 2 * excl;
            continue;
        }
        n_seen++;
        reads += C->n_pass; sum_nm += C->sum_nm; sum_indel += C->sum_indel;
        full_len += L; cov_full += C->cov_full;
        if (2 * excl < L) {
            const u64 wl = L - 2 * excl;
            win_len += wl; sum_d += C->sum_d; sum_d2 += C->sum_d2; cov_win += C->cov_win; proc_win += C->proc_win;
            min_d = min(min_d, (C->proc_win < wl || C->min_d == 0xffffffffu) ? 0u : C->min_d);
            nh = max(nh, C->max_d + 1u);
        }
    }
    reads = wave_sum_u64(reads); sum_nm = wave_sum_u64(sum_nm); sum_indel = wave_sum_u64(sum_indel);
    sum_d = wave_sum_u64(sum_d); sum_d2 = wave_sum_u64(sum_d2); cov_win = wave_sum_u64(cov_win); cov_full = wave_sum_u64(cov_full);
    win_len = wave_sum_u64(win_len); full_len = wave_sum_u64(full_len); proc_win = wave_sum_u64(proc_win);
    uw = wave_sum_u64(uw); uf = wave_sum_u64(uf);
    min_d = wave_min_u32(min_d); nh = wave_max_u32(nh); n_seen = wave_sum_u32(n_seen);
    if (lane_id() != 0) return;
    DevGenome *A = &G[g];
    if (uw) atomicAdd(&A->unobs_win, uw);
    if (uf) atomicAdd(&A->unobs_full, uf);
    if (n_seen == 0) return;
    atomicAdd(&A->reads, reads); atomicAdd(&A->sum_nm, sum_nm); atomicAdd(&A->sum_indel, sum_indel);
    atomicAdd(&A->sum_d, sum_d); atomicAdd(&A->sum_d2, sum_d2); atomicAdd(&A->cov_win, cov_win); atomicAdd(&A->cov_full, cov_full);
    atomicAdd(&A->win_len, win_len); atomicAdd(&A->full_len, full_len); atomicAdd(&A->proc_win, proc_win);
    atomicMin(&A->min_d, min_d); atomicMax(&A->nh, nh); atomicAdd(&A->n_seen, n_seen);
}

__global__ __launch_bounds__(64) void k_genome_identity(const DevContig *__restrict__ ctg, GenomeTable T, DevGenome *__restrict__ G) {
    const u32 g = blockIdx.x;
    if (g >= T.n_genomes) return;
    const u32 lo = T.row[g], hi = T.row[g + 1];
    double acc = 0.0;
// ... 74 lines not shown
    __syncthreads();
    return max(wbase, inc);
}
__global__ __launch_bounds__(1024) void k_order_max(const DevContig *__restrict__ ctg, u32 n_targets, u64 *__restrict__ ord) {
    __shared__ u32 wmax[16];
    const u32 c = blockIdx.x * 1024u + threadIdx.x;
    u32 total;
    (void)block_incl_max_u32((c < n_targets && ctg[c].n_pass != 0) ? ctg[c].last_rec + 1u : 0u, wmax, total);
    if (threadIdx.x == 0) ord[1 + blockIdx.x] = total;
    if (blockIdx.x == 0 && threadIdx.x == 0) ord[0] = ~0ull;
}
__global__ __launch_bounds__(1024) void k_order_check(const DevContig *__restrict__ ctg, u32 n_targets, u64 *__restrict__ ord) {
    __shared__ u32 wmax[16];
    u32 mine = 0, base;
    for (u32 b = threadIdx.x; b < blockIdx.x; b += 1024u) mine = max(mine, (u32)ord[1 + b]);
    (void)block_incl_max_u32(mine, wmax, base);
    const u32 c = blockIdx.x * 1024u + threadIdx.x;
    const bool seen = c < n_targets && ctg[c].n_pass != 0;
    const u32 v = seen ? ctg[c].last_rec + 1u : 0u;
    u32 total;
    const u32 inc = block_incl_max_u32(v, wmax, total);
    const u32 up = __shfl_up(inc, 1);
    __shared__ u32 wlast[16];
    if (lane_id() == 63) wlast[threadIdx.x >> 6] = inc;
    __syncthreads();
    u32 prev = lane_id() ? up : ((threadIdx.x >> 6) ? wlast[(threadIdx.x >> 6) - 1] : 0u);
    prev = max(prev, base);
    if (seen && prev != 0u && ctg[c].first_rec < prev - 1u) atomicMin(&ord[0], (u64)ctg[c].first_rec);
}

template <bool LANES>
__device__ __forceinline__ void genome_estimate_body(const DevGenome *__restrict__ G, u32 n_genomes, const u64 *__restrict__ ghist, const EstParams &P,
                                                     float *__restrict__ out, DevGenomeStats *__restrict__ stats) {
    const u32 g_raw = LANES ? blockIdx.x * 256u + threadIdx.x : blockIdx.x * 4u + (threadIdx.x >> 6);
    if (!LANES && g_raw >= n_genomes) return;
    const bool in = g_raw < n_genomes;
    const u32 g = in ? g_raw : n_genomes - 1u;
    const DevGenome *A = &G[g];
    EstEntry E;
    E.win_len = A->win_len; E.win_sum_d = A->sum_d; E.win_sum_d2 = A->sum_d2; E.win_covered = A->cov_win; E.win_min_d = A->min_d;
    E.full_len = A->full_len; E.full_covered = A->cov_full; E.n_reads = A->reads; E.mismatches = A->sum_nm - A->sum_indel;
    E.nh = A->nh;
    E.bin0_extra = A->win_len - A->proc_win + A->unobs_win;
    E.unobs_win = A->unobs_win; E.unobs_full = A->unobs_full;
    E.identity = A->id;
    const bool nonzero = estimate_entry<LANES, u64>(E, ghist + A->hist_off, in, true, P, out + (size_t)g * P.n);
    if (LANES ? in : lane_id() == 0) {
        DevGenomeStats o;
        o.reads_in_genome = A->reads; o.genome_len = A->full_len + A->unobs_full; o.n_contigs_seen = A->n_seen; o.any_nonzero = nonzero ? 1u : 0u;
        stats[g] = o;
    }
}
__global__ __launch_bounds__(256) void k_genome_estimate(const DevGenome *__restrict__ G, u32 n_genomes, const u64 *__restrict__ ghist, EstParams P,
                                                         float *__restrict__ out, DevGenomeStats *__restrict__ stats) {
    genome_estimate_body<false>(G, n_genomes, ghist, P, out, stats);
}
__global__ __launch_bounds__(256) void k_genome_estimate_lanes(const DevGenome *__restrict__ G, u32 n_genomes, const u64 *__restrict__ ghist, EstParams P,
                                                               float *__restrict__ out, DevGenomeStats *__restrict__ stats) {
    genome_estimate_body<true>(G, n_genomes, ghist, P, out, stats);
}

}
```

### coverm_amd/csrc/pileup_kernels.hip.h

```cpp
#pragma once
#include <hip/hip_runtime.h>
#include <stdint.h>

namespace covk {

typedef unsigned long long u64;
typedef unsigned int u32;

constexpr u32 F_POS_UNSORTED = 1u;
constexpr u32 RW_SINGLE = 0u, RW_DOUBLE = 1u, RW_COMPLEX = 2u, RW_BUCKET = 3u;
constexpr u32 FAST_MAX_CAND = 8191u;
constexpr u32 TILE_F_GENERIC = 1u, TILE_F_SLOW = 2u;
constexpr u32 CX_MIN_OPS = 16;

struct DevContig {
    u64 n_primary, n_pass, n_nonsupp, sum_nm, sum_indel;
    double id_primary, id_nonsupp;
    u64 sum_d, sum_d2, cov_win, cov_full, proc_win;
    u64 hist_off;
    u32 first_rec, last_rec;
    u32 rec_start, rec_end;
    u32 n_groups;
    u32 max_span;
    u32 flags;
    u32 hist_cap;
    u32 min_d, max_d;
    u32 hist_len;
    u32 pad;
    u64 chist_off;
};
static_assert(sizeof(DevContig) == 160, "DevContig layout");

constexpr u32 COUNTER_SLOTS = 64;
struct DevGlobal {
    u64 first_error;
    u64 hist_cap_total;
    u64 chist_total;
    u32 internal_error;
    u32 n_cx;
    u64 cx_total;
    u32 n_slow;
    u32 n_gen;
    u64 pad2[2];
    u64 prim_slots[COUNTER_SLOTS * 8];
    u64 cons_slots[COUNTER_SLOTS * 8];
    u32 pad_q[8 * 16];
};

struct FilterCfg {
    u32 include_improper_pairs, include_supplementary, include_secondary;
    u32 filter_single, min_mapq, min_aligned_length;
    float min_percent_identity, min_aligned_percent;
};

struct Records {
    const int32_t *tid, *pos;
    const uint16_t *flag;
    const uint8_t *mapq;
    const u32 *nm;
    const uint8_t *nm_kind;
    const u32 *l_seq;
    const u32 *cigar_off;
    const u32 *cigar;
    u32 n;
    u32 cigar_end;
};

__device__ __forceinline__ int lane_id() { return threadIdx.x & 63; }

__device__ __forceinline__ int wave_incl_scan(int v) {
    v += __builtin_amdgcn_update_dpp(0, v, 0x111, 0xf, 0xf, false);
    v += __builtin_amdgcn_update_dpp(0, v, 0x112, 0xf, 0xf, false);
    v += __builtin_amdgcn_update_dpp(0, v, 0x114, 0xf, 0xf, false);
    v += __builtin_amdgcn_update_dpp(0, v, 0x118, 0xf, 0xf, false);
    v += __builtin_amdgcn_update_dpp(0, v, 0x142, 0xa, 0xf, false);
    v += __builtin_amdgcn_update_dpp(0, v, 0x143, 0xc, 0xf, false);
    return v;
}
__device__ __forceinline__ int wave_incl_max(int v) {
    const int NEG = (int)0x80000000;
    v = max(v, __builtin_amdgcn_update_dpp(NEG, v, 0x111, 0xf, 0xf, false));
    v = max(v, __builtin_amdgcn_update_dpp(NEG, v, 0x112, 0xf, 0xf, false));
    v = max(v, __builtin_amdgcn_update_dpp(NEG, v, 0x114, 0xf, 0xf, false));
    v = max(v, __builtin_amdgcn_update_dpp(NEG, v, 0x118, 0xf, 0xf, false));
    v = max(v, __builtin_amdgcn_update_dpp(NEG, v, 0x142, 0xa, 0xf, false));
    v = max(v, __builtin_amdgcn_update_dpp(NEG, v, 0x143, 0xc, 0xf, false));
    return v;
}
__device__ __forceinline__ u64 wave_sum_u64(u64 v) {
#pragma unroll
    for (int o = 32; o > 0; o >>= 1) v += __shfl_xor(v, o);
    return v;
}
__device__ __forceinline__ u32 wave_sum_u32(u32 v) {
#pragma unroll
    for (int o = 32; o > 0; o >>= 1) v += __shfl_xor(v, o);
    return v;
}
__device__ __forceinline__ u32 wave_min_u32(u32 v) {
#pragma unroll
    for (int o = 32; o > 0; o >>= 1) v = min(v, (u32)__shfl_xor(v, o));
    return v;
}
__device__ __forceinline__ u32 wave_max_u32(u32 v) {
#pragma unroll
    for (int o = 32; o > 0; o >>= 1) v = max(v, (u32)__shfl_xor(v, o));
    return v;
}

__device__ __forceinline__ u32 wave_sum_u32_dpp(u32 v) { return (u32)__builtin_amdgcn_readlane(wave_incl_scan((int)v), 63); }
__device__ __forceinline__ u64 wave_sum_u56(u64 v) {
    const u32 lo = (u32)v & 0xffffffu, hi = (u32)(v >> 24);
    return (u64)wave_sum_u32_dpp(lo) + ((u64)wave_sum_u32_dpp(hi) << 24);
}
__device__ __forceinline__ u32 wave_max_u32_dpp(u32 v) {
    return (u32)__builtin_amdgcn_readlane(wave_incl_max((int)(v ^ 0x80000000u)), 63) ^ 0x80000000u;
}
__device__ __forceinline__ u32 wave_min_u32_dpp(u32 v) { return ~wave_max_u32_dpp(~v); }

__device__ __forceinline__ double bcast_f64(double v, int q) {
    const long long b = __double_as_longlong(v);
    const u32 lo = __builtin_amdgcn_readlane((u32)b, q), hi = __builtin_amdgcn_readlane((u32)(b >> 32), q);
    return __longlong_as_double((long long)(((u64)hi << 32) | lo));
}
__device__ __forceinline__ u64 bcast_u64(u64 v, int q) {
    const u32 lo = __builtin_amdgcn_readlane((u32)v, q), hi = __builtin_amdgcn_readlane((u32)(v >> 32), q);
    return ((u64)hi << 32) | lo;
}

__device__ __forceinline__ void report_error(DevGlobal *g, u32 rec, u32 code) {
    atomicMin(&g->first_error, ((u64)rec << 8) | code);
}

struct TileIdx {
    const u32 *tile_first;
    u32 *tcnt, *fov;
    u32 shift;
    u32 n_tiles;
};

struct CxIdx {
    u32 *list; u32 list_cap;
    u32 *cnt, *cur;
    const u32 *cscan, *ctop;
    uint2 *runs; u64 runs_cap;
};

struct PrepPartial;
struct PrepCold {
    DevContig *ctg; DevGlobal *g; PrepPartial *part; u32 *cx_list;
    const uint8_t *mask; const u32 *tlen; const u32 *tile_first;
    u32 *gen_list;
    u32 cx_list_cap, pad;
};
struct PrepHot {
    const int32_t *tid, *pos;
    const uint16_t *flag;
    const uint8_t *nmk;
    const u32 *nm, *coff, *cigar;
    const uint8_t *mapq;
    const u32 *lseq;
    uint2 *runs;
    u32 *tcnt, *fov;
    double *identp, *identn;
    u32 n, cigar_end, n_targets, shift, steps;
    u32 gate_mask;
    u32 p1_mask;
    u32 min_mapq, min_aligned_length;
    float min_percent_identity, min_aligned_percent;
};
struct PrepArgs { PrepHot hot; PrepCold cold; };

__global__ void k_init(DevContig *ctg, u32 n_targets, DevGlobal *g, TileIdx ti, CxIdx cx, PrepArgs *pa_out, PrepArgs pa) {
    u32 c = blockIdx.x * blockDim.x + threadIdx.x;
    if (c == 0 && pa_out != nullptr) *pa_out = pa;
    if (c < ti.n_tiles) { ti.tcnt[c] = 0u; ti.fov[c] = 0xffffffffu; cx.cnt[c] = 0u; cx.cur[c] = 0u; }
    if (c == 0) {
        g->first_error = ~0ull; g->hist_cap_total = 0; g->chist_total = 0; g->internal_error = 0;
        g->n_cx = 0; g->cx_total = 0; g->n_slow = 0; g->n_gen = 0;
    }
    if (c < COUNTER_SLOTS * 8) { g->prim_slots[c] = 0; g->cons_slots[c] = 0; }
    if (c >= n_targets) return;
    DevContig z;
    z.n_primary = z.n_pass = z.n_nonsupp = z.sum_nm = z.sum_indel = 0;
    z.id_primary = z.id_nonsupp = 0.0;
    z.sum_d = z.sum_d2 = z.cov_win = z.cov_full = z.proc_win = 0;
    z.hist_off = 0;
    z.first_rec = 0xffffffffu; z.last_rec = 0;
    z.rec_start = 0xffffffffu; z.rec_end = 0;
    z.n_groups = 0; z.max_span = 0; z.flags = 0; z.hist_cap = 0;
    z.min_d = 0xffffffffu; z.max_d = 0; z.hist_len = 0; z.pad = 0; z.chist_off = 0;
    ctg[c] = z;
}

constexpr int PREP_B = 2;
constexpr int PREP_PASSES = 8;
constexpr int PREP_CHUNK = 256 * PREP_B * PREP_PASSES;

constexpr u32 CIG_FAST_OPS = 128;
__device__ __forceinline__ void cigar_walk_slow(const u32 *__restrict__ cigar, u32 co0, u32 nops, int pos, u32 L, u64 &aligned,
                                             u64 &indel, u32 &run_start, u32 &run_len, u32 &run2_start, u32 &run2_len,
                                             u32 &n_runs, u32 &span, bool &oob, bool &badcig) {
    aligned = 0; indel = 0; run_start = run_len = run2_start = run2_len = n_runs = span = 0; oob = false; badcig = false;
    long long cursor = pos;
    long long cur_e = -1;
    for (u32 c = 0; c < nops; c++) {
        const u32 wd = cigar[co0 + c];
        const u32 op = wd & 15u, len = wd >> 4;
        if (op == 0u || op == 7u || op == 8u) {
            if (cursor < 0 || cursor >= (long long)L) oob = true;
            if (n_runs > 0 && cursor == cur_e) {
                cur_e += len;
                if (n_runs == 1) run_len += len; else if (n_runs == 2) run2_len += len;
            } else {
                n_runs++;
                cur_e = cursor + len;
                if (n_runs == 1) { run_start = (u32)cursor; run_len = len; }
                else if (n_runs == 2) { run2_start = (u32)cursor; run2_len = len; }
            }
            cursor += len; aligned += len;
        } else if (op == 2u) { cursor += len; indel += len; aligned += len; }
        else if (op == 3u) { cursor += len; }
        else if (op == 1u) { indel += len; aligned += len; }
        else if (op > 8u) badcig = true;
    }
    const long long sp = cursor - (long long)pos;
    span = sp > 0 ? (u32)min(sp, (long long)0xffffffffu) : 0u;
}

struct WalkOut {
    u64 aligned, indel;
    u32 run_start, run_len, run2_start, run2_len, n_runs, span;
    bool oob, badcig, absurd;
// ... 374 lines not shown
                    }
                }
            }
        }
    }
    {
        PrepPartial pw;
        pw.tid = flushed_early ? -2 : cur;
        pw.prim = acc.prim; pw.pass = acc.pass; pw.nons = acc.nons;
        pw.span = wave_max_u32(acc.span); pw.first = wave_min_u32(acc.first); pw.last = wave_max_u32(acc.last);
        pw.nm = wave_sum_u64(acc.nm); pw.indel = wave_sum_u64(acc.indel); pw.pad = 0;
        if (lane == 0) wpart[w] = pw;
    }
    if (lane == 0) { blk_cnt[0][w] = g_prim; blk_cnt[1][w] = g_cons; }
    __syncthreads();
    bool uniform_wg = true;
    {
        int t0 = -1;
        for (int k = 0; k < 4; k++) {
            const int t = wpart[k].tid;
            if (t == -2) uniform_wg = false;
            else if (t >= 0) { if (t0 < 0) t0 = t; else if (t != t0) uniform_wg = false; }
        }
        if (threadIdx.x == 0) {
            PrepPartial o; o.tid = -1; o.prim = o.pass = o.nons = o.span = 0; o.first = 0xffffffffu; o.last = 0; o.pad = 0; o.nm = o.indel = 0;
            if (uniform_wg && t0 >= 0) {
                o.tid = t0;
                for (int k = 0; k < 4; k++) {
                    const PrepPartial &q = wpart[k];
                    if (q.tid < 0) continue;
                    o.prim += q.prim; o.pass += q.pass; o.nons += q.nons; o.span = max(o.span, q.span);
                    o.first = min(o.first, q.first); o.last = max(o.last, q.last); o.nm += q.nm; o.indel += q.indel;
                }
            }
            part[blockIdx.x] = o;
        }
    }
    if (!uniform_wg) prep_flush(ctg, cur, acc);
    if (threadIdx.x == 0) {
        const u32 p = blk_cnt[0][0] + blk_cnt[0][1] + blk_cnt[0][2] + blk_cnt[0][3];
        const u32 c = blk_cnt[1][0] + blk_cnt[1][1] + blk_cnt[1][2] + blk_cnt[1][3];
        const u32 slot = (blockIdx.x % COUNTER_SLOTS) * 8u;
        if (p) atomicAdd(&g->prim_slots[slot], (u64)p);
        if (c) atomicAdd(&g->cons_slots[slot], (u64)c);
    }
}

#define COV_PREP_KERNEL(NAME, ATTR, PF, PB)                                                                                                           \
    template <bool WANT_IDENTITY, bool FILTER, bool MASKED>                                                                                      \
    __global__ __launch_bounds__(256) ATTR void NAME(Records r, const u32 *__restrict__ tlen, u32 n_targets, const uint8_t *__restrict__ mask,   \
                                                     FilterCfg f, DevContig *ctg, DevGlobal *g, uint2 *__restrict__ runs,                        \
                                                     double *__restrict__ identp, double *__restrict__ identn, PrepPartial *__restrict__ part,   \
                                                     TileIdx ti, int passes, int b_active, u32 *__restrict__ cx_list, u32 cx_list_cap) {         \
        prep_body<WANT_IDENTITY, FILTER, MASKED, PF, PB>(r, tlen, n_targets, mask, f, ctg, g, runs, identp, identn, part, ti, passes, b_active, cx_list, \
                                                 cx_list_cap);                                                                                   \
    }
COV_PREP_KERNEL(k_prep7s, __attribute__((amdgpu_waves_per_eu(7, 7))), true, 1)
#undef COV_PREP_KERNEL

__device__ __forceinline__ void prep_reduce_body(u32 c, DevContig *ctg, u32 n_targets, const PrepPartial *__restrict__ part, u32 n_parts, u32 chunk_recs) {
    if (c >= n_targets) return;
    DevContig *C = &ctg[c];
    const u32 rs = C->rec_start, re = C->rec_end;
    if (rs >= re) return;
    const u32 b0 = rs / chunk_recs, b1 = min((re - 1) / chunk_recs, n_parts - 1);
    u32 prim = 0, pass = 0, nons = 0, span = 0, first = 0xffffffffu, last = 0;
    u64 nm = 0, indel = 0;
    for (u32 b = b0 + (threadIdx.x & 63); b <= b1; b += 64) {
        const PrepPartial q = part[b];
        if (q.tid != (int)c) continue;
        prim += q.prim; pass += q.pass; nons += q.nons; span = max(span, q.span);
        first = min(first, q.first); last = max(last, q.last); nm += q.nm; indel += q.indel;
    }
    prim = wave_sum_u32(prim); pass = wave_sum_u32(pass); nons = wave_sum_u32(nons); span = wave_max_u32(span);
    first = wave_min_u32(first); last = wave_max_u32(last); nm = wave_sum_u64(nm); indel = wave_sum_u64(indel);
    if ((threadIdx.x & 63) == 0 && pass) {
        C->n_primary += prim; C->n_pass += pass; C->n_nonsupp += nons; C->sum_nm += nm; C->sum_indel += indel;
        C->max_span = max(C->max_span, span); C->first_rec = min(C->first_rec, first); C->last_rec = max(C->last_rec, last);
    }
}

__device__ __forceinline__ u32 lower_bound_pos(const int32_t *__restrict__ pos, u32 lo, u32 hi, long long key) {
    while (lo < hi) {
        const u32 mid = lo + ((hi - lo) >> 1);
        if ((long long)pos[mid] < key) lo = mid + 1; else hi = mid;
    }
    return lo;
}

struct ScanPair { const u32 *cnt[2]; u32 *scan[2]; u32 *top[2]; u64 *total[2]; };
__global__ __launch_bounds__(1024) void k_tile_scan1(ScanPair sp, u32 n_tiles, u32 n_blocks) {
    __shared__ u32 wtot[16];
    const u32 which = blockIdx.x >= n_blocks ? 1u : 0u, blk = blockIdx.x - which * n_blocks;
    const u32 *__restrict__ tcnt = sp.cnt[which];
    const u32 t = blk * 1024u + threadIdx.x;
    const int lane = lane_id(), w = threadIdx.x >> 6;
    const u32 v = t < n_tiles ? tcnt[t] : 0u;
    const u32 inc = (u32)wave_incl_scan((int)v);
    if (lane == 63) wtot[w] = inc;
    __syncthreads();
    u32 wbase = 0, tot = 0;
    for (int k = 0; k < 16; k++) { const u32 x = wtot[k]; if (k < w) wbase += x; tot += x; }
    if (t < n_tiles) sp.scan[which][t] = wbase + inc - v;
    if (threadIdx.x == 0) sp.top[which][blk] = tot;
}

__global__ __launch_bounds__(1024) void k_tile_scan2(ScanPair sp, u32 n_blocks) {
    __shared__ u32 wtot[16];
    __shared__ u32 carry_s;
    u32 *ttop = sp.top[blockIdx.x];
    u64 *total = sp.total[blockIdx.x];
    if (threadIdx.x == 0) carry_s = 0;
    __syncthreads();
    const int lane = lane_id(), w = threadIdx.x >> 6;
    for (u32 base = 0; base < n_blocks; base += 1024u) {
        const u32 b = base + threadIdx.x;
        const u32 v = b < n_blocks ? ttop[b] : 0u;
        const u32 inc = (u32)wave_incl_scan((int)v);
        if (lane == 63) wtot[w] = inc;
        __syncthreads();
        u32 wbase = 0, tot = 0;
        for (int k = 0; k < 16; k++) { const u32 x = wtot[k]; if (k < w) wbase += x; tot += x; }
        const u32 carry = carry_s;
        if (b < n_blocks) ttop[b] = carry + wbase + inc - v;
        __syncthreads();
        if (threadIdx.x == 0) carry_s = carry + tot;
        __syncthreads();
    }
    if (total != nullptr && threadIdx.x == 0) *total = carry_s;
}

template <bool FILL>
__device__ __forceinline__ void cx_expand_body(const Records &r, const u32 *__restrict__ tlen, DevGlobal *g, const CxIdx &cx, const TileIdx &ti, u32 wave, u32 n_waves) {
    const int lane = lane_id();
    const u32 n = min(g->n_cx, cx.list_cap);
    if (FILL && g->cx_total > cx.runs_cap) return;
    const u64 lt = lane == 0 ? 0ull : (~0ull >> (64 - lane));
    for (u32 j = wave; j < n; j += n_waves) {
        const u32 i = cx.list[j];
        const int tid = r.tid[i];
        const u32 co0 = r.cigar_off[i], nops = r.cigar_off[i + 1] - co0;
        const u32 L = tlen[tid], t0 = ti.tile_first[tid];
        long long cur0 = r.pos[i];
        u32 wd_next = (u32)lane < nops ? r.cigar[co0 + (u32)lane] : 4u;
        for (u32 base = 0; base < nops; base += 64) {
            const u32 wd = wd_next;
            const u32 idn = base + 64u + (u32)lane;
            wd_next = idn < nops ? r.cigar[co0 + idn] : 4u;
            const u32 len = wd >> 4, bit = 1u << (wd & 15u);
            const u32 fr = (bit & 0x18du) ? len : 0u;
            const u32 incl = (u32)wave_incl_scan((int)fr), excl = incl - fr;
            const long long sj = cur0 + (long long)excl;
            const bool m = (bit & 0x181u) != 0u && len > 0u && sj >= 0 && sj < (long long)L;
            const u32 sv = (u32)sj, ev = sv + len;
            const u32 ts = sv >> ti.shift, te = m ? (min(ev, L) - 1u) >> ti.shift : 0u;
            for (u32 k = 0; __any(m && ts + k <= te); k++) {
                const bool v = m && ts + k <= te;
                const u32 key = t0 + ts + k;
                u32 slot = 0;
                for (u64 todo = __ballot(v); todo != 0;) {
                    const int l = __ffsll((long long)todo) - 1;
                    const u32 k0 = __builtin_amdgcn_readlane(key, l);
                    const u64 grp = __ballot(v && key == k0);
                    u32 b = 0;
                    if (lane == l) b = atomicAdd(FILL ? &cx.cur[k0] : &cx.cnt[k0], (u32)__popcll(grp));
                    if (FILL) {
                        b = __builtin_amdgcn_readlane(b, l);
                        if (v && key == k0) slot = b + (u32)__popcll(grp & lt);
                    }
                    todo &= ~grp;
                }
                if (FILL && v) cx.runs[(u64)cx.cscan[key] + cx.ctop[key >> 10] + slot] = make_uint2(sv, ev);
            }
            cur0 += (long long)__builtin_amdgcn_readlane(incl, 63);
        }
    }
}

template <bool FILL>
__global__ __launch_bounds__(256) void k_cx_expand(Records r, const u32 *__restrict__ tlen, DevGlobal *g, CxIdx cx, TileIdx ti) {
    cx_expand_body<FILL>(r, tlen, g, cx, ti, blockIdx.x * 4u + (threadIdx.x >> 6), gridDim.x * 4u);
}

__global__ __launch_bounds__(256) void k_post_prep(Records r, const u32 *__restrict__ tlen, DevGlobal *g, CxIdx cx, TileIdx ti, DevContig *ctg, u32 n_targets,
                                                   const PrepPartial *__restrict__ part, u32 n_parts, u32 chunk_recs, u32 n_red) {
    if (blockIdx.x < n_red) prep_reduce_body(blockIdx.x * 4u + (threadIdx.x >> 6), ctg, n_targets, part, n_parts, chunk_recs);
    else cx_expand_body<false>(r, tlen, g, cx, ti, (blockIdx.x - n_red) * 4u + (threadIdx.x >> 6), (gridDim.x - n_red) * 4u);
}

template <bool WANT_HIST>
__global__ __launch_bounds__(256) void k_ranges(const u32 *__restrict__ tile_contig, const u32 *__restrict__ tile_start,
                                                u32 n_tiles, const u32 *__restrict__ tlen, const uint8_t *__restrict__ mask,
                                                DevContig *ctg, uint4 *__restrict__ desc, TileIdx ti,
                                                const u32 *__restrict__ tscan, const u32 *__restrict__ ttop, CxIdx cx,
                                                DevGlobal *__restrict__ g, u32 *__restrict__ slow_list) {
    const u32 t = blockIdx.x * blockDim.x + threadIdx.x;
    if (t >= n_tiles) return;
    const u32 c = tile_contig[t];
    DevContig *C = &ctg[c];
    uint4 out = make_uint4(0u, 0u, tlen[c], 0u);
    u32 cxn = 0, cxo = 0;
    if (C->n_pass != 0 && (mask == nullptr || mask[c])) {
        const u32 rs = C->rec_start, re = C->rec_end;
        cxn = g->cx_total <= cx.runs_cap ? cx.cnt[t] : 0u;
        cxo = cx.cscan[t] + cx.ctop[t >> 10];
        if (C->n_groups != 1u) out.w = 1u;
        if (C->n_groups != 1u || (C->flags & F_POS_UNSORTED)) {
            out.x = rs; out.y = re;
        } else {
            const u32 tf = ti.tile_first[c];
            const u32 before = (tscan[t] + ttop[t >> 10]) - (tscan[tf] + ttop[tf >> 10]);
            const u32 f = rs + before;
            out.y = min(f + ti.tcnt[t], re);
            out.x = max(min(f, ti.fov[t]), rs);
            out.x = min(out.x, out.y);
        }
    }
    if (out.x < out.y || cxn) {
        if (out.w || out.y - out.x + cxn > FAST_MAX_CAND) {
            out.w |= TILE_F_SLOW;
            if (slow_list != nullptr) slow_list[atomicAdd(&g->n_slow, 1u)] = t;
        }
    }
    if (WANT_HIST) {
        const u32 npass = (u32)min(C->n_pass, (u64)0xffffffffu);
        const u32 cap = min(out.y - out.x + cxn, npass);
        if (__all(c == (u32)__builtin_amdgcn_readfirstlane((int)c))) {
            const u32 m = wave_max_u32(cap);
            if (lane_id() == 0 && m) atomicMax(&C->hist_cap, m);
        } else if (cap) atomicMax(&C->hist_cap, cap);
    }
    desc[2 * t] = out;
    desc[2 * t + 1] = make_uint4(c, tile_start[t], cxo, cxn);
}

template <int MODE>
__device__ __forceinline__ u64 hist_bins_of(const DevContig *C, u32 c, const u32 *__restrict__ tlen, const uint8_t *__restrict__ mask, u64 excl) {
    const bool live = C->n_pass != 0 && (mask == nullptr || mask[c]);
    if (MODE == 0) return live ? (u64)C->hist_cap + 1 : 0;
    return (live && 2 * excl < (u64)tlen[c]) ? (u64)C->max_d + 1 : 0;
}
__device__ __forceinline__ u64 block_incl_scan_u64(u64 v, u64 *wtot, u64 &total) {
    const int lane = lane_id(), w = threadIdx.x >> 6;
    u64 inc = v;
#pragma unroll
    for (int o = 1; o < 64; o <<= 1) {
        const u64 t = __shfl_up(inc, o);
        if (lane >= o) inc += t;
    }
    if (lane == 63) wtot[w] = inc;
    __syncthreads();
    u64 wbase = 0; total = 0;
    for (int k = 0; k < 16; k++) { const u64 x = wtot[k]; if (k < w) wbase += x; total += x; }
    __syncthreads();
    return wbase + inc;
}
template <int MODE>
__global__ __launch_bounds__(1024) void k_hist_sum(const DevContig *__restrict__ ctg, u32 n_targets, const u32 *__restrict__ tlen,
                                                   const uint8_t *__restrict__ mask, u64 excl, u64 *__restrict__ top) {
    __shared__ u64 wtot[16];
    const u32 c = blockIdx.x * 1024u + threadIdx.x;
    u64 total;
    (void)block_incl_scan_u64(c < n_targets ? hist_bins_of<MODE>(&ctg[c], c, tlen, mask, excl) : 0, wtot, total);
    if (threadIdx.x == 0) top[blockIdx.x] = total;
}
template <int MODE>
__global__ __launch_bounds__(1024) void k_hist_off(DevContig *ctg, u32 n_targets, const u32 *__restrict__ tlen, const uint8_t *__restrict__ mask,
                                                   u64 excl, const u64 *__restrict__ top, DevGlobal *g) {
    __shared__ u64 wtot[16];
    u64 mine = 0, base;
    for (u32 b = threadIdx.x; b < blockIdx.x; b += 1024u) mine += top[b];
    (void)block_incl_scan_u64(mine, wtot, base);
    const u32 c = blockIdx.x * 1024u + threadIdx.x;
    const u64 v = c < n_targets ? hist_bins_of<MODE>(&ctg[c], c, tlen, mask, excl) : 0;
    u64 total;
    const u64 inc = block_incl_scan_u64(v, wtot, total);
    if (c < n_targets) {
        if (MODE == 0) ctg[c].hist_off = base + inc - v;
        else { ctg[c].chist_off = base + inc - v; ctg[c].hist_len = (u32)v; }
    }
    if (blockIdx.x == gridDim.x - 1 && threadIdx.x == 0) {
        if (MODE == 0) g->hist_cap_total = base + total; else g->chist_total = base + total;
    }
}

__global__ void k_zero_u32(u32 *__restrict__ p, const u64 *__restrict__ n_ptr) {
    const u64 n = *n_ptr;
    for (u64 i = (u64)blockIdx.x * blockDim.x + threadIdx.x; i < n; i += (u64)gridDim.x * blockDim.x) p[i] = 0u;
}

__global__ __launch_bounds__(256) void k_hist_compact(const DevContig *__restrict__ ctg, u32 n_targets,
                                                      const u32 *__restrict__ tlen, u64 excl,
                                                      const u32 *__restrict__ arena, u64 *__restrict__ out) {
    const u32 c = blockIdx.x * 4u + (threadIdx.x >> 6);
    if (c >= n_targets) return;
    const DevContig *C = &ctg[c];
    const u32 n = C->hist_len;
    if (n == 0) return;
    const u64 win_len = (u64)tlen[c] - 2 * excl;
    for (u32 d = threadIdx.x & 63u; d < n; d += 64u) {
        u64 v = arena[C->hist_off + d];
        if (d == 0) v += win_len - C->proc_win;
        out[C->chist_off + d] = v;
    }
}

__global__ __launch_bounds__(64) void k_identity(DevContig *ctg, u32 n_targets, const double *__restrict__ identp,
                                                 const double *__restrict__ identn, const int32_t *__restrict__ tidv) {
    const u32 c = blockIdx.x;
    if (c >= n_targets) return;
    DevContig *C = &ctg[c];
    if (C->n_pass == 0) return;
    const u32 rs = C->rec_start, re = C->rec_end;
    const bool generic = C->n_groups != 1u;
    double accp = 0.0, accn = 0.0;
    const int lane = lane_id();
    u32 i = rs + (u32)lane;
    double xp = 0.0, xn = 0.0;
    if (i < re && (!generic || tidv[i] == (int)c)) { if (identp) xp = identp[i]; if (identn) xn = identn[i]; }
    for (u32 b = rs; b < re; b += 64) {
        const double cp = xp, cn = xn;
        i += 64;
        xp = 0.0; xn = 0.0;
        if (i < re && (!generic || tidv[i] == (int)c)) { if (identp) xp = identp[i]; if (identn) xn = identn[i]; }
#pragma unroll 16
        for (int k = 0; k < 64; k++) {
            accn += __shfl(cn, k);
            accp += __shfl(cp, k);
        }
    }
    if (lane == 0) { C->id_primary = accp; C->id_nonsupp = accn; }
}

constexpr u32 ID_CH = 1024;
struct IdChunk {
    double ap, an;
    u64 tp, tn;
    int ep, en;
    u32 flags;
    u32 pad;
};
constexpr int ID_SERIAL = -2147483647 - 1;

__device__ __forceinline__ int f64_exp(double v) { return (int)((__double_as_longlong(v) >> 52) & 0x7ff) - 1023; }

__global__ __launch_bounds__(256) void k_id_approx(const double *__restrict__ identp, const double *__restrict__ identn,
                                                   u32 n, IdChunk *__restrict__ ch) {
    __shared__ double sp[4], sn[4];
    __shared__ u32 sf[4];
    const u32 k = blockIdx.x, base = k * ID_CH;
    double ap = 0.0, an = 0.0;
    u32 fl = 0;
#pragma unroll
    for (int j = 0; j < (int)(ID_CH / 256); j++) {
        const u32 i = base + (u32)j * 256u + threadIdx.x;
        if (i < n) {
            const double xp = identp ? identp[i] : 0.0, xn = identn ? identn[i] : 0.0;
// ... 169 lines not shown
        for (u32 kb = k0; kb < k1; kb += 64) {
            const u32 kk = kb + (u32)lane;
            IdChunk x;
            if (kk < k1) x = ch[kk]; else { x.tp = x.tn = 0; x.ep = x.en = ID_SERIAL; x.flags = 15u; }
            const u32 nb = min(64u, k1 - kb);
            auto run_stream = [&](double &S, const int e_l, const u64 t_l, const bool bad_l, const bool is_p) {
                u32 q = 0;
                while (q < nb) {
                    const u64 bits = (u64)__double_as_longlong(S);
                    const int e_cur = (int)((bits >> 52) & 0x7ff) - 1023;
                    const u64 m = (bits & 0xfffffffffffffull) | (1ull << 52);
                    const bool in_range = (u32)lane >= q && (u32)lane < nb;
                    u64 P = in_range ? t_l : 0ull;
#pragma unroll
                    for (int o = 1; o < 64; o <<= 1) { const u64 t = __shfl_up(P, o); if (lane >= o) P += t; }
                    const bool fits = in_range && !bad_l && !(bits >> 63) && e_l == e_cur && t_l < (1ull << 53) &&
                                      P < (1ull << 53) && m + P < (1ull << 53);
                    const u64 failm = __ballot(in_range && !fits);
                    const u32 jstar = failm ? (u32)(__ffsll((long long)failm) - 1) : nb;
                    if (jstar > q) {
                        const u64 T = bcast_u64(P, (int)(jstar - 1));
                        S = __longlong_as_double((long long)((bits & 0xfff0000000000000ull) | ((m + T) & 0xfffffffffffffull)));
                    }
                    if (jstar < nb) serial((kb + jstar) * ID_CH, (kb + jstar + 1) * ID_CH, is_p, !is_p);
                    q = jstar + 1;
                }
            };
            if (identp != nullptr) run_stream(Sp, x.ep, x.tp, (x.flags & (1u | 4u)) != 0u, true);
            if (identn != nullptr) run_stream(Sn, x.en, x.tn, (x.flags & (2u | 8u)) != 0u, false);
        }
        serial(k1 * ID_CH, re, true, true);
    }
    if (lane == 0) { C->id_primary = Sp; C->id_nonsupp = Sn; }
}

__device__ __attribute__((noinline)) void hist_add_overflow(u32 *arena, u64 hoff, u32 hcap, DevGlobal *g, u32 d, u32 x) {
    if (d <= hcap) atomicAdd(&arena[hoff + d], x);
    else atomicOr(&g->internal_error, 1u);
}

struct PileupArgs {
    const u32 *tile_contig, *tile_start;
    const uint4 *desc;
    const uint2 *runs;
    const uint2 *cx_runs;
    Records r;
    DevContig *ctg;
    DevGlobal *g;
    u32 *hist_arena;
    u64 excl;
    int32_t *depth_out;
    const u64 *depth_off;
    u32 tile_base;
};


__device__ __forceinline__ void lds_fence() { asm volatile("s_waitcnt lgkmcnt(0)" ::: "memory"); }

constexpr int STREAM_TW = 1024, STREAM_HB = 512, STREAM_CAP = 512;

template <bool WANT_HIST, bool WRITE_DEPTH>
__global__ __launch_bounds__(256) void k_pileup_stream(PileupArgs a, u32 n_tiles, u32 chunk_tiles,
                                                       const u32 *__restrict__ tile_list, const u32 *__restrict__ n_list) {
    if (tile_list != nullptr) n_tiles = *n_list;
    constexpr int TW = STREAM_TW, HBW = STREAM_HB, CAP = STREAM_CAP, ROWS = TW / 64;
    extern __shared__ __attribute__((aligned(16))) char smem[];
    const int lane = threadIdx.x & 63, w = threadIdx.x >> 6;
    int *tile = reinterpret_cast<int *>(smem + (size_t)w * (TW * 4 + HBW * 4));
    u32 *lhist = reinterpret_cast<u32 *>(tile + TW);
    int4 *t4 = reinterpret_cast<int4 *>(tile);
    int2 *ent = reinterpret_cast<int2 *>(tile);
    const u32 wave_id = blockIdx.x * 4u + (u32)w, n_waves = gridDim.x * 4u;
    if (WANT_HIST) {
#pragma unroll
        for (int b = lane; b < HBW; b += 64) lhist[b] = 0u;
    }
    u64 sum_d = 0, sum_d2 = 0, proc_win = 0;
    u32 cov_w = 0, cov_f = 0, mn = 0xffffffffu, mx = 0;
    int cur_c = -1;
    u64 hoff = 0; u32 hcap = 0;
    const u64 excl = a.excl;

    auto hist_add = [&](u32 d, u32 x) {
        if (__builtin_expect(d < (u32)HBW, 1)) atomicAdd(&lhist[d], x);
        else hist_add_overflow(a.hist_arena, hoff, hcap, a.g, d, x);
    };
    auto flush = [&]() {
        if (cur_c >= 0) {
            const u64 s1 = wave_sum_u64(sum_d), s2 = wave_sum_u64(sum_d2);
            const u32 c1 = wave_sum_u32(cov_w), c2 = wave_sum_u32(cov_f);
            const u32 m1 = wave_min_u32(mn), m2 = wave_max_u32(mx);
            DevContig *C = &a.ctg[cur_c];
            if (lane == 0) {
                if (s1) atomicAdd(&C->sum_d, s1);
                if (s2) atomicAdd(&C->sum_d2, s2);
                if (c1) atomicAdd(&C->cov_win, (u64)c1);
                if (c2) atomicAdd(&C->cov_full, (u64)c2);
                if (proc_win) {
                    atomicAdd(&C->proc_win, proc_win);
                    atomicMin(&C->min_d, m1);
                    atomicMax(&C->max_d, m2);
                }
            }
            if (WANT_HIST && proc_win) {
                lds_fence();
                const u32 hi_b = min(m2, (u32)HBW - 1u);
                for (u32 b = m1 + (u32)lane; b <= hi_b; b += 64) {
                    const u32 x = lhist[b];
                    if (x) { atomicAdd(&a.hist_arena[hoff + b], x); lhist[b] = 0u; }
                }
                lds_fence();
            }
        }
        sum_d = sum_d2 = 0; proc_win = 0; cov_w = cov_f = 0; mn = 0xffffffffu; mx = 0;
    };

// ... 100 lines not shown
                    const int2 en = live ? ent[e] : make_int2(0, 0);
                    const u32 nxt = (e + 1 < E) ? (u32)ent[e + 1].x : tlen_t;
                    const int inc = wave_incl_scan(en.y);
                    const int d = carry + inc;
                    carry += __builtin_amdgcn_readlane(inc, 63);
                    const u32 du = (u32)d;
                    const bool small = !__any(live && du >= 1024u);
                    if (live) {
                        const u32 s = min((u32)en.x, tlen_t), t_ = min(nxt, tlen_t);
                        if (d > 0) cov_f += t_ - s;
                        const u32 a0 = max(s, wl0), a1 = min(t_, wl1);
                        if (a1 > a0) {
                            const u32 len = a1 - a0;
                            if (small) { s1t += __umul24(du, len); s2t += __umul24(__umul24(du, du), len); }
                            else { sum_d += (u64)du * len; sum_d2 += (u64)du * du * len; }
                            if (d > 0) cov_w += len;
                            mn = min(mn, du); mx = max(mx, du);
                            if (WANT_HIST) hist_add(du, len);
                        }
                    }
                }
                sum_d += s1t; sum_d2 += s2t;
            } else {
                int carry = 0;
#pragma unroll
                for (int j = 0; j < ROWS; j++) {
                    const int inc = wave_incl_scan(x[j]);
                    const int d = carry + inc;
                    carry += __builtin_amdgcn_readlane(inc, 63);
                    const u32 p = lo + (u32)(j * 64 + lane);
                    const u32 du = (u32)d;
                    if (p < L) {
                        cov_f += d > 0;
                        if (WRITE_DEPTH) a.depth_out[dbase + p] = d;
                        if (win_any && p >= wst && p < wet) {
                            sum_d += du;
                            sum_d2 += (u64)du * du;
                            cov_w += d > 0;
                            mn = min(mn, du); mx = max(mx, du);
                            if (WANT_HIST) {
                                const u32 rel = p - wst;
                                if (x[j] != 0 && rel) { hist_add((u32)(d - x[j]), rel); hist_add(du, 0u - rel); }
                                if (p == wet - 1) hist_add(du, wet - wst);
                            }
                        }
                    }
                }
            }
        }
        flush();
        cur_c = -1;
        ch = ch_next;
    }
}

constexpr size_t pileup_stream_smem_bytes() { return (size_t)4 * ((size_t)STREAM_TW * 4 + STREAM_HB * 4); }

constexpr int FAST_TW = 1024, FAST_HB = 512;
constexpr int FAST_HB7 = 384;
constexpr size_t pileup_fast_smem_bytes(bool hist, int hb = FAST_HB, int tables = 2) { return (size_t)4 * ((size_t)FAST_TW * 2 * tables + (hist ? (size_t)hb * 4 : 0)); }

typedef short v2i16 __attribute__((ext_vector_type(2)));
typedef __attribute__((address_space(3))) u32 lds_u32_t;
__device__ __forceinline__ u32 lds_addr_of(const u32 *p) { return (u32)(uintptr_t)(lds_u32_t *)p; }
__device__ __forceinline__ void lds_atomic_add(u32 addr, u32 x) { (void)__hip_atomic_fetch_add((lds_u32_t *)(uintptr_t)addr, x, __ATOMIC_RELAXED, __HIP_MEMORY_SCOPE_WORKGROUP); }

template <bool WANT_HIST, int HB, int TABLES>
__device__ __forceinline__ void pileup_fast_body(const PileupArgs &a, u32 n_tiles, u32 chunk_tiles) {
    constexpr int TW = FAST_TW, HBW = HB;
    constexpr int DS = TABLES == 1 ? 2 : 0;
    constexpr size_t WB = (size_t)TW * 2 * TABLES + (WANT_HIST ? (size_t)HBW * 4 : 0);
    extern __shared__ __attribute__((aligned(16))) char smem[];
    const int lane = threadIdx.x & 63, w = threadIdx.x >> 6;
    u32 *S = reinterpret_cast<u32 *>(smem + (size_t)w * WB);
    u32 *E = TABLES == 2 ? S + TW / 2 : S;
    u32 *lhist = S + (TW / 2) * TABLES;
    uint4 *S4 = reinterpret_cast<uint4 *>(S), *E4 = reinterpret_cast<uint4 *>(E);
    const u32 wave_id = (u32)__builtin_amdgcn_readfirstlane((int)(blockIdx.x * 4u + (u32)w)), n_waves = gridDim.x * 4u;
    if (WANT_HIST) {
#pragma unroll
        for (int b = lane; b < HBW; b += 64) lhist[b] = 0u;
    }
    u64 sum_d = 0, sum_d2 = 0, proc_win = 0;
    u32 cov_w = 0, cov_f = 0, mn = 0xffffffffu, mx = 0;
    int cur_c = -1;
    u64 hoff = 0; u32 hcap = 0;
    const u64 excl = a.excl;
    bool lh_explicit = false;
    u32 hbound = 0;
    auto drain = [&](bool derive) {
        lds_fence();
        for (u32 b = (u32)lane; b <= hbound; b += 64) {
            const u32 x = lhist[b];
            if (x) {
                atomicAdd(&a.hist_arena[hoff + b], x); lhist[b] = 0u;
                if (derive) {
                    const u32 cv = b ? x : 0u;
                    sum_d += (u64)b * x; sum_d2 += (u64)(b * b) * x; cov_w += cv; cov_f += cv;
                    mn = min(mn, b); mx = max(mx, b);
                }
            }
        }
        lds_fence();
        hbound = 0;
    };

// ... 363 lines not shown
            r = est_f32(n_reads * 1000000000ull) / est_f32(T);
            break;
        }
        case EST_VARIANCE: {
            const u64 T = win_len + E.unobs_win;
            if (T == 0) break;
            if ((est_f32(win_covered) / est_f32(T)) < e.min_frac || T < 3 || win_len == 0) break;
            const u64 kk = E.unobs_win > 0 ? 0ull : win_min_d, N = T;
            const u64 ex = win_sum_d - kk * N;
            const u64 ex2 = win_sum_d2 - 2 * kk * win_sum_d + kk * kk * N;
            r = (est_f32(ex2) - est_f32(ex * ex) / est_f32(T)) / est_f32(T - 1);
            break;
        }
        case EST_LENGTH: r = est_f32(full_len + E.unobs_full); break;
        case EST_READ_COUNT: r = est_f32(n_reads); break;
        case EST_READS_PER_BASE: r = est_f32(n_reads) / est_f32(full_len + E.unobs_full); break;
        case EST_ANIR: r = n_reads == 0 ? 0.0f : (float)(E.identity / (double)n_reads); break;
        default: break;
        }
        if (!live) r = 0.0f;
        nonzero |= r > 0.0f;
        if (LANES) { if (in) o[k] = r; }
        else if (lane == 0) o[k] = r;
    }
    return nonzero;
}

template <bool LANES>
__device__ __forceinline__ void estimate_body(const DevContig *__restrict__ ctg, u32 n_targets, const u32 *__restrict__ tlen, u64 excl,
                                              const u32 *__restrict__ arena, const EstParams &P, float *__restrict__ out) {
    const int lane = lane_id();
    const u32 c_raw = LANES ? blockIdx.x * 256u + threadIdx.x : blockIdx.x * 4u + (threadIdx.x >> 6);
    if (!LANES && c_raw >= n_targets) return;
    const bool in = c_raw < n_targets;
    const u32 c = in ? c_raw : n_targets - 1u;
    const DevContig *C = &ctg[c];
    float *o = out + (size_t)c * P.n;
    const bool touched = C->n_pass != 0;
    if (!LANES && !touched) { if ((u32)lane < P.n) o[lane] = 0.0f; return; }
    const u64 L = tlen[c];
    const bool has_win = 2 * excl < L;
    EstEntry E;
    E.win_len = has_win ? L - 2 * excl : 0;
    E.win_sum_d = has_win ? C->sum_d : 0; E.win_sum_d2 = has_win ? C->sum_d2 : 0; E.win_covered = has_win ? C->cov_win : 0;
    E.win_min_d = has_win ? ((C->proc_win < E.win_len || C->min_d == 0xffffffffu) ? 0u : C->min_d) : 0xffffffffu;
    E.full_len = L; E.full_covered = C->cov_full; E.n_reads = C->n_primary; E.mismatches = C->sum_nm - C->sum_indel;
    E.nh = has_win ? C->max_d + 1u : 0u;
    E.bin0_extra = E.win_len - C->proc_win;
    E.unobs_win = 0; E.unobs_full = 0;
    E.identity = C->id_primary;
    (void)estimate_entry<LANES, u32>(E, arena + C->hist_off, in, touched, P, o);
}
__global__ __launch_bounds__(256) void k_estimate(const DevContig *__restrict__ ctg, u32 n_targets, const u32 *__restrict__ tlen, u64 excl,
                                                  const u32 *__restrict__ arena, EstParams P, float *__restrict__ out) {
    estimate_body<false>(ctg, n_targets, tlen, excl, arena, P, out);
}
__global__ __launch_bounds__(256) void k_estimate_lanes(const DevContig *__restrict__ ctg, u32 n_targets, const u32 *__restrict__ tlen, u64 excl,
                                                        const u32 *__restrict__ arena, EstParams P, float *__restrict__ out) {
    estimate_body<true>(ctg, n_targets, tlen, excl, arena, P, out);
}

struct DevInterval { u32 tid, pad; u64 start, end; };
struct DevIntervalStats { u64 win_sum_d, win_sum_d2, win_covered, full_covered; u32 win_min_d, win_max_d, hist_len, pad; u64 hist_off; };

__global__ __launch_bounds__(256) void k_interval_stats(const int32_t *__restrict__ depth, const u64 *__restrict__ depth_off,
                                                        const DevInterval *__restrict__ iv, u64 n, u64 excl,
                                                        DevIntervalStats *__restrict__ out) {
    const int lane = lane_id();
    const u64 wave = (u64)blockIdx.x * 4u + (threadIdx.x >> 6), n_waves = (u64)gridDim.x * 4u;
    for (u64 g = wave; g < n; g += n_waves) {
        const DevInterval I = iv[g];
        const int32_t *d = depth + depth_off[I.tid];
        const u64 len = I.end - I.start;
        const bool has_win = 2 * excl < len;
        const u64 ws = I.start + excl, we = has_win ? I.end - excl : ws;
        u64 s1 = 0, s2 = 0;
        u32 cw = 0, cf = 0, mn = 0xffffffffu, mx = 0;
        for (u64 p = I.start + (u64)lane; p < I.end; p += 64) {
            const u32 v = (u32)d[p];
            cf += v > 0u;
            if (has_win && p >= ws && p < we) { s1 += v; s2 += (u64)v * v; cw += v > 0u; mn = min(mn, v); mx = max(mx, v); }
        }
        s1 = wave_sum_u64(s1); s2 = wave_sum_u64(s2);
        cw = wave_sum_u32(cw); cf = wave_sum_u32(cf); mn = wave_min_u32(mn); mx = wave_max_u32(mx);
        if (lane == 0) {
            DevIntervalStats o;
            o.win_sum_d = s1; o.win_sum_d2 = s2; o.win_covered = cw; o.full_covered = cf;
            o.win_min_d = has_win ? mn : 0u; o.win_max_d = mx; o.hist_len = has_win ? mx + 1u : 0u; o.pad = 0; o.hist_off = 0;
            out[g] = o;
        }
    }
}

constexpr int IV_HB = 512;
__global__ __launch_bounds__(256) void k_interval_hist(const int32_t *__restrict__ depth, const u64 *__restrict__ depth_off,
                                                       const DevInterval *__restrict__ iv, u64 n, u64 excl,
                                                       const DevIntervalStats *__restrict__ st, unsigned long long *__restrict__ hist) {
    __shared__ u32 lh[4][IV_HB];
    const int lane = lane_id(), w = threadIdx.x >> 6;
    const u64 wave = (u64)blockIdx.x * 4u + (u64)w, n_waves = (u64)gridDim.x * 4u;
    for (int b = lane; b < IV_HB; b += 64) lh[w][b] = 0u;
    for (u64 g = wave; g < n; g += n_waves) {
        const DevInterval I = iv[g];
        const DevIntervalStats S = st[g];
        if (S.hist_len == 0u) continue;
        const int32_t *d = depth + depth_off[I.tid];
        unsigned long long *h = hist + S.hist_off;
        for (u64 p = I.start + excl + (u64)lane; p < I.end - excl; p += 64) {
            const u32 v = (u32)d[p];
            if (v < (u32)IV_HB) atomicAdd(&lh[w][v], 1u); else atomicAdd(&h[v], 1ull);
        }
        asm volatile("s_waitcnt lgkmcnt(0)" ::: "memory");
// ... 8 lines not shown
```

### coverm_amd/csrc/prep_lean.hip.h

```cpp
#pragma once
#include "pileup_kernels.hip.h"

namespace covk {

struct __attribute__((packed, aligned(4))) CigTriple { u32 a, b, c; };

__device__ __forceinline__ int dpp_prev(int v, int edge) { return __builtin_amdgcn_update_dpp(edge, v, 0x138, 0xf, 0xf, false); }
__device__ __forceinline__ int dpp_next(int v, int edge) { return __builtin_amdgcn_update_dpp(edge, v, 0x130, 0xf, 0xf, false); }

struct CigSum {
    u64 aligned, indel;
    u32 run_start, run_len, run2_start, run2_len, n_runs, span;
    bool oob, badcig, big;
};

__device__ __forceinline__ void cigar_sum3(u32 w0, u32 w1, u32 w2, int pos, u32 L, CigSum &o) {
    const u32 len0 = w0 >> 4, len1 = w1 >> 4, len2 = w2 >> 4;
    const u32 bit0 = 1u << (w0 & 15u), bit1 = 1u << (w1 & 15u), bit2 = 1u << (w2 & 15u);
    const bool m0 = (bit0 & 0x181u) != 0u, m1 = (bit1 & 0x181u) != 0u, m2 = (bit2 & 0x181u) != 0u;
    const u32 ref0 = (bit0 & 0x18du) ? len0 : 0u, ref1 = (bit1 & 0x18du) ? len1 : 0u, ref2 = (bit2 & 0x18du) ? len2 : 0u;
    const u32 c0 = (u32)pos, c1 = c0 + ref0, c2 = c1 + ref1;
    o.span = ref0 + ref1 + ref2;
    o.aligned = ((bit0 & 0x187u) ? len0 : 0u) + ((bit1 & 0x187u) ? len1 : 0u) + ((bit2 & 0x187u) ? len2 : 0u);
    o.indel = ((bit0 & 0x006u) ? len0 : 0u) + ((bit1 & 0x006u) ? len1 : 0u) + ((bit2 & 0x006u) ? len2 : 0u);
// ... 422 lines not shown
    }
    if (lane == 0) { blk_cnt[0][w] = g_prim; blk_cnt[1][w] = g_cons; wmask[w] = left_mask; }
    __syncthreads();
    if (w == 0u) {
        const u32 m0 = wmask[0], m1 = wmask[1], m2 = wmask[2], m3 = wmask[3];
        const u32 c0 = (u32)__popc(m0), c1 = c0 + (u32)__popc(m1), c2 = c1 + (u32)__popc(m2), total = c2 + (u32)__popc(m3);
        if (total) {
            u32 at = 0;
            if (lane == 0) at = atomicAdd(&cold->g->n_gen, total);
            at = (u32)__builtin_amdgcn_readfirstlane((int)at);
            for (u32 e = (u32)lane; e < total; e += 64u) {
                const u32 k = e < c0 ? 0u : e < c1 ? 1u : e < c2 ? 2u : 3u;
                u32 m = k == 0u ? m0 : k == 1u ? m1 : k == 2u ? m2 : m3;
                for (u32 r = e - (k == 0u ? 0u : k == 1u ? c0 : k == 2u ? c1 : c2); r != 0u; r--) m &= m - 1u;
                cold->gen_list[at + e] = (blockIdx.x * 4u + k) * wave_recs + (u32)__builtin_ctz(m) * 64u;
            }
        }
    }
    bool uniform_wg = true;
    {
        int t0 = -1;
        for (int k = 0; k < 4; k++) {
            const int t = wpart[k].tid;
            if (t == -2) uniform_wg = false;
            else if (t >= 0) { if (t0 < 0) t0 = t; else if (t != t0) uniform_wg = false; }
        }
        if (threadIdx.x == 0) {
            PrepPartial o; o.tid = -1; o.prim = o.pass = o.nons = o.span = 0; o.first = 0xffffffffu; o.last = 0; o.pad = 0; o.nm = o.indel = 0;
            if (uniform_wg && t0 >= 0) {
                o.tid = t0;
                for (int k = 0; k < 4; k++) {
                    const PrepPartial &q = wpart[k];
                    if (q.tid < 0) continue;
                    o.prim += q.prim; o.pass += q.pass; o.nons += q.nons; o.span = max(o.span, q.span);
                    o.first = min(o.first, q.first); o.last = max(o.last, q.last); o.nm += q.nm; o.indel += q.indel;
                }
            }
            cold->part[blockIdx.x] = o;
        }
    }
    if (!uniform_wg) lean_flush(cold->ctg, cur, acc);
    if (threadIdx.x == 0) {
        const u32 p = blk_cnt[0][0] + blk_cnt[0][1] + blk_cnt[0][2] + blk_cnt[0][3];
        const u32 c = blk_cnt[1][0] + blk_cnt[1][1] + blk_cnt[1][2] + blk_cnt[1][3];
        const u32 slot = (blockIdx.x % COUNTER_SLOTS) * 8u;
        DevGlobal *g = cold->g;
        if (p) atomicAdd(&g->prim_slots[slot], (u64)p);
        if (c) atomicAdd(&g->cons_slots[slot], (u64)c);
    }
}

template <bool WANT_IDENTITY, bool FILTER, bool MASKED>
__global__ __launch_bounds__(256) __attribute__((amdgpu_waves_per_eu(8, 8))) void k_prep_lean(PrepHot h, const PrepArgs *__restrict__ pa) {
    prep_lean_body<WANT_IDENTITY, FILTER, MASKED>(h, pa);
}
template <bool WANT_IDENTITY, bool FILTER, bool MASKED>
__global__ __launch_bounds__(256) void k_prep_generic(const PrepArgs *__restrict__ pa, u32 all_steps) {
    const u32 n = all_steps ? all_steps : pa->cold.g->n_gen;
    const u32 *__restrict__ list = pa->cold.gen_list;
    for (u32 j = blockIdx.x * 4u + (threadIdx.x >> 6); j < n; j += gridDim.x * 4u) {
        const u32 i0 = all_steps ? j * 64u : (u32)__builtin_amdgcn_readfirstlane((int)list[j]);
        GenFields f;
        gen_load<FILTER>(pa->hot, i0, f);
        prep_step_generic<WANT_IDENTITY, FILTER, MASKED>(pa, i0, f);
    }
}

}
```

Measured before the change: 47.17 billion.

## Fold range/scan/hist launches into fewer kernels and replace host events with device stamps

Replaces per-stage hipEvent timing with device-side begin/end timestamps written into the global struct, removing most event records from the stream. It also merges work into fewer launches: the two tile-scan passes become one k_tile_scan, cx_expand is folded into extra blocks of k_ranges, and a single-kernel k_hist_layout replaces hist_sum+hist_off when the contig count is small. The aim is lower launch and event overhead per call. In exchange, kernels gain extra stamp atomics and some redundant prefix recomputation in k_hist_layout.

Measured after the change: 45.34 billion. 0.961x the previous value.

```diff
diff --git a/coverm_amd/csrc/covermhip.hip b/coverm_amd/csrc/covermhip.hip
--- a/coverm_amd/csrc/covermhip.hip
+++ b/coverm_amd/csrc/covermhip.hip
@@ -84,6 +84,11 @@
 }
 
 extern "C" int covh_timing_on(void) { return cov_timing_on() ? 1 : 0; }
+struct HostStamp {
+    const char *what; std::chrono::steady_clock::time_point t0; bool on;
+    explicit HostStamp(const char *w) : what(w), on(cov_timing_on()) { if (on) t0 = std::chrono::steady_clock::now(); }
+    ~HostStamp() { if (on) fprintf(stderr, "[covermhip] host: %s %.1f us\n", what, std::chrono::duration<double, std::micro>(std::chrono::steady_clock::now() - t0).count()); }
+};
 
 struct InflateKernel { int version = 3; int lz_version = 2; u32 round_blocks = 0; u64 carry = 16ull << 20; u64 cwin = 0; u32 ext_parts = covi::EXT_PARTS; };
 
@@ -243,9 +248,8 @@
     bool last_gen_all = false;
     uint64_t algo_bytes = 0;
 
-    hipEvent_t ev[COV_K_COUNT][2] = {};
-    hipEvent_t ev_begin[COV_K_COUNT] = {};
-    int ev_fresh = -1;
+    hipEvent_t ev_identity[2] = {}, ev_group[2] = {};
+    int wall_clock_khz = 0;
     float k_ms[COV_K_COUNT] = {};
     uint32_t k_launches[COV_K_COUNT] = {};
 };
@@ -351,16 +355,25 @@
     return COV_OK;
 }
 
+static_assert(TG_PREP == COV_K_PREP && TG_RANGES == COV_K_RANGES && TG_PILEUP == COV_K_PILEUP && TG_HIST == COV_K_HIST && TG_HIST_COMPACT == COV_K_HIST_COMPACT &&
+              TG_ESTIMATE == COV_K_ESTIMATE && TG_GENOME == COV_K_GENOME && COV_K_GENOME < (int)STAMP_GROUPS, "kernel groups: the device's stamps are indexed by COV_K_*");
 void timing_events(cov_session *s) {
-    if (s->ev[0][0]) return;
-    for (int k = 0; k < COV_K_COUNT; k++)
-        for (int j = 0; j < 2; j++) (void)hipEventCreate(&s->ev[k][j]);
-}
-void time_begin(cov_session *s, int k) {
-    if (s->ev_fresh >= 0) { s->ev_begin[k] = s->ev[s->ev_fresh][1]; return; }
-    (void)hipEventRecord(s->ev[k][0], s->stream); s->ev_begin[k] = s->ev[k][0];
-}
-void time_end(cov_session *s, int k) { (void)hipEventRecord(s->ev[k][1], s->stream); s->k_launches[k]++; s->ev_fresh = k; }
+    if (s->ev_identity[0]) return;
+    for (int j = 0; j < 2; j++) { (void)hipEventCreate(&s->ev_identity[j]); (void)hipEventCreate(&s->ev_group[j]); }
+    int khz = 0;
+    if (hipDeviceGetAttribute(&khz, hipDeviceAttributeWallClockRate, s->cfg.device) == hipSuccess) s->wall_clock_khz = khz; else (void)hipGetLastError();
+}
+u64 stamped_end(const DevGlobal &G, int k) {
+    u64 end = 0;
+    for (u32 l = 0; l < STAMP_LINES; l++) end = std::max<u64>(end, G.t_end[l * STAMP_GROUPS + (u32)k]);
+    return end;
+}
+float stamped_ms(const cov_session *s, const DevGlobal &G, int k) {
+    const u64 end = stamped_end(G, k);
+    u64 begin = G.t_begin[k];
+    if (k == COV_K_PILEUP && !begin) begin = s->k_launches[COV_K_HIST] ? stamped_end(G, COV_K_HIST) : stamped_end(G, COV_K_RANGES);
+    return (s->wall_clock_khz > 0 && begin && end > begin) ? (float)((double)(end - begin) / (double)s->wall_clock_khz) : 0.f;
+}
 
 template <bool H, int TABLES>
 void launch_fast_v(cov_session *s, const PileupArgs &a, u32 n_tiles) {
@@ -429,7 +442,7 @@
     PileupArgs a{};
     a.tile_contig = s->d_tile_contig.p; a.tile_start = s->d_tile_start.p; a.desc = s->d_desc.p;
     a.runs = s->d_runs.p; a.cx_runs = s->d_cx_runs.p; a.r = records_of(s); a.ctg = s->d_ctg.p; a.g = s->d_glob.p;
-    a.hist_arena = s->d_arena.p; a.excl = s->cfg.contig_end_exclusion; a.depth_out = nullptr; a.tile_base = 0;
+    a.hist_arena = s->d_arena.p; a.excl = s->cfg.contig_end_exclusion; a.depth_out = nullptr; a.tile_base = 0; a.t_group = TG_NONE;
     return a;
 }
 
@@ -581,8 +594,7 @@
     s->d_runs.release(); s->d_part.release(); s->d_prep_args.release(); s->d_gen_list.release(); s->d_hist_top.release(); s->d_ident.release(); s->d_identp.release(); s->d_idch.release();
     if (s->ev_prep_done) (void)hipEventDestroy(s->ev_prep_done);
     if (s->ev_side_done) (void)hipEventDestroy(s->ev_side_done); s->d_arena.release(); s->d_chist.release(); s->d_depth.release();
-    for (int k = 0; k < COV_K_COUNT; k++)
-        for (int j = 0; j < 2; j++) if (s->ev[k][j]) (void)hipEventDestroy(s->ev[k][j]);
+    for (int j = 0; j < 2; j++) { if (s->ev_identity[j]) (void)hipEventDestroy(s->ev_identity[j]); if (s->ev_group[j]) (void)hipEventDestroy(s->ev_group[j]); }
     if (s->stream) (void)hipStreamDestroy(s->stream);
     delete s;
 }
@@ -964,7 +976,6 @@
     for (int k = 0; k < COV_K_COUNT; k++) { s->k_launches[k] = 0; s->k_ms[k] = 0.f; }
     bool compacted = false;
     s->est_valid = false; s->gen_valid = false;
-    s->ev_fresh = -1;
 
     HIPCHK(s->d_runs.reserve(std::max<size_t>(1, R), st));
     const uint64_t ncig_all = s->adopted ? s->adopted_ncig : s->n_cigar;
@@ -1020,7 +1031,6 @@
     HIPCHK(hipGetLastError());
 
     if (R) {
-        time_begin(s, COV_K_PREP);
         const u32 n_steps = (R + 63u) / 64u;
         const bool gen_all = prep_kernel != 7 && (uint64_t)R < (uint64_t)nT * 128u;
         s->last_gen_all = gen_all;
@@ -1051,12 +1061,12 @@
             }
         }
 #undef COV_LAUNCH_PREP
-        if (nT) {
+        {
             const u32 n_red = gen_all ? 0u : (nT + 3u) / 4u, cx_grid0 = (u32)s->n_cus * 8u;
             hipLaunchKernelGGL(k_post_prep, dim3(n_red + cx_grid0), dim3(256), 0, st, r, s->d_tlen.p, s->d_glob.p, cx, ti, s->d_ctg.p, nT, (const PrepPartial *)s->d_part.p,
-                               prep_grid, prep_chunk, n_red);
-        }
-        time_end(s, COV_K_PREP);
+                               prep_grid, prep_chunk, n_red, (int)COV_K_PREP);
+        }
+        s->k_launches[COV_K_PREP]++;
         HIPCHK(hipGetLastError());
         if (want_id && nT) {
             if (!s->side) {
@@ -1066,7 +1076,7 @@
             }
             HIPCHK(hipEventRecord(s->ev_prep_done, st));
             HIPCHK(hipStreamWaitEvent(s->side, s->ev_prep_done, 0));
-            (void)hipEventRecord(s->ev[COV_K_IDENTITY][0], s->side);
+            (void)hipEventRecord(s->ev_identity[0], s->side);
             if (s->id_mode) {
                 const u32 nch = (R + ID_CH - 1) / ID_CH;
                 hipLaunchKernelGGL(k_id_approx, dim3(nch), dim3(256), 0, s->side, idp, idn, R, s->d_idch.p);
@@ -1075,61 +1085,63 @@
                 hipLaunchKernelGGL(k_id_combine, dim3(nT), dim3(64), 0, s->side, s->d_ctg.p, nT, idp, idn, r.tid, s->d_idch.p);
             } else
                 hipLaunchKernelGGL(k_identity, dim3(nT), dim3(64), 0, s->side, s->d_ctg.p, nT, idp, idn, r.tid);
-            (void)hipEventRecord(s->ev[COV_K_IDENTITY][1], s->side);
+            (void)hipEventRecord(s->ev_identity[1], s->side);
             s->k_launches[COV_K_IDENTITY]++;
             HIPCHK(hipGetLastError());
             HIPCHK(hipEventRecord(s->ev_side_done, s->side));
-            s->ev_fresh = -1;
         }
     }
     if (R && s->n_tiles) {
-        time_begin(s, COV_K_RANGES);
         const u32 n_blocks = (s->n_tiles + 1023u) / 1024u;
         const u32 cx_grid = (u32)s->n_cus * 8u;
+        const u32 n_rb = (s->n_tiles + 255u) / 256u;
         ScanPair sp{};
         sp.cnt[0] = s->d_tcnt.p; sp.scan[0] = s->d_tscan.p; sp.top[0] = s->d_ttop.p; sp.total[0] = nullptr;
         sp.cnt[1] = s->d_cx_cnt.p; sp.scan[1] = s->d_cx_scan.p; sp.top[1] = s->d_cx_top.p; sp.total[1] = &s->d_glob.p->cx_total;
-        hipLaunchKernelGGL(k_tile_scan1, dim3(2u * n_blocks), dim3(1024), 0, st, sp, s->n_tiles, n_blocks);
-        hipLaunchKernelGGL(k_tile_scan2, dim3(2), dim3(1024), 0, st, sp, n_blocks);
-        hipLaunchKernelGGL((k_cx_expand<true>), dim3(cx_grid), dim3(256), 0, st, r, s->d_tlen.p, s->d_glob.p, cx, ti);
+        hipLaunchKernelGGL(k_tile_scan, dim3(2u * n_blocks), dim3(1024), 0, st, sp, s->n_tiles, n_blocks, s->d_glob.p, (int)COV_K_RANGES);
         u32 *slow_list = s->use_fast ? s->d_slow_list.p : nullptr;
         if (want_hist)
-            hipLaunchKernelGGL((k_ranges<true>), dim3((s->n_tiles + 255) / 256), dim3(256), 0, st, s->d_tile_contig.p,
+            hipLaunchKernelGGL((k_ranges<true>), dim3(n_rb + cx_grid), dim3(256), 0, st, s->d_tile_contig.p,
                                s->d_tile_start.p, s->n_tiles, s->d_tlen.p, mask, s->d_ctg.p, s->d_desc.p, ti, s->d_tscan.p,
-                               s->d_ttop.p, cx, s->d_glob.p, slow_list);
+                               s->d_ttop.p, cx, s->d_glob.p, slow_list, r, n_rb, (int)COV_K_RANGES);
         else
-            hipLaunchKernelGGL((k_ranges<false>), dim3((s->n_tiles + 255) / 256), dim3(256), 0, st, s->d_tile_contig.p,
+            hipLaunchKernelGGL((k_ranges<false>), dim3(n_rb + cx_grid), dim3(256), 0, st, s->d_tile_contig.p,
                                s->d_tile_start.p, s->n_tiles, s->d_tlen.p, mask, s->d_ctg.p, s->d_desc.p, ti, s->d_tscan.p,
-                               s->d_ttop.p, cx, s->d_glob.p, slow_list);
-        time_end(s, COV_K_RANGES);
+                               s->d_ttop.p, cx, s->d_glob.p, slow_list, r, n_rb, (int)COV_K_RANGES);
+        s->k_launches[COV_K_RANGES]++;
         HIPCHK(hipGetLastError());
         if (want_hist) {
-            time_begin(s, COV_K_HIST);
             const u32 hb = (nT + 1023u) / 1024u;
             HIPCHK(s->d_hist_top.reserve(hb, st));
-            hipLaunchKernelGGL((k_hist_sum<0>), dim3(hb), dim3(1024), 0, st, (const DevContig *)s->d_ctg.p, nT, s->d_tlen.p, mask, (u64)s->cfg.contig_end_exclusion, s->d_hist_top.p);
-            hipLaunchKernelGGL((k_hist_off<0>), dim3(hb), dim3(1024), 0, st, s->d_ctg.p, nT, s->d_tlen.p, mask, (u64)s->cfg.contig_end_exclusion, (const u64 *)s->d_hist_top.p, s->d_glob.p);
-            hipLaunchKernelGGL(k_zero_u32, dim3(2048), dim3(256), 0, st, s->d_arena.p, &s->d_glob.p->hist_cap_total);
-            time_end(s, COV_K_HIST);
+            if (hb <= HIST_LAYOUT_MAX_BLOCKS)
+                hipLaunchKernelGGL(k_hist_layout, dim3(hb), dim3(1024), 0, st, s->d_ctg.p, nT, s->d_tlen.p, mask, (u64)s->cfg.contig_end_exclusion, s->d_glob.p, (int)COV_K_HIST);
+            else {
+                hipLaunchKernelGGL((k_hist_sum<0>), dim3(hb), dim3(1024), 0, st, (const DevContig *)s->d_ctg.p, nT, s->d_tlen.p, mask, (u64)s->cfg.contig_end_exclusion, s->d_hist_top.p,
+                                   s->d_glob.p, (int)COV_K_HIST);
+                hipLaunchKernelGGL((k_hist_off<0>), dim3(hb), dim3(1024), 0, st, s->d_ctg.p, nT, s->d_tlen.p, mask, (u64)s->cfg.contig_end_exclusion, (const u64 *)s->d_hist_top.p, s->d_glob.p);
+            }
+            hipLaunchKernelGGL(k_zero_u32, dim3(2048), dim3(256), 0, st, s->d_arena.p, (const u64 *)&s->d_glob.p->hist_cap_total, s->d_glob.p, (int)COV_K_HIST);
+            s->k_launches[COV_K_HIST]++;
             HIPCHK(hipGetLastError());
         }
         PileupArgs a = pileup_args(s);
-        time_begin(s, COV_K_PILEUP);
+        a.t_group = COV_K_PILEUP;
         if (want_hist) launch_any_pileup<true, false>(s, a, s->n_tiles);
         else launch_any_pileup<false, false>(s, a, s->n_tiles);
-        time_end(s, COV_K_PILEUP);
+        s->k_launches[COV_K_PILEUP]++;
         HIPCHK(hipGetLastError());
         if (want_hist) {
             compacted = s->est.n == 0 || s->hist_fetch_seen;
             s->hist_prefetched = 0;
             if (compacted) {
                 HIPCHK(s->d_chist.reserve((size_t)R + nT + 1, st));
-                time_begin(s, COV_K_HIST_COMPACT);
                 const u32 hb = (nT + 1023u) / 1024u;
-                hipLaunchKernelGGL((k_hist_sum<1>), dim3(hb), dim3(1024), 0, st, (const DevContig *)s->d_ctg.p, nT, s->d_tlen.p, mask, (u64)s->cfg.contig_end_exclusion, s->d_hist_top.p);
+                hipLaunchKernelGGL((k_hist_sum<1>), dim3(hb), dim3(1024), 0, st, (const DevContig *)s->d_ctg.p, nT, s->d_tlen.p, mask, (u64)s->cfg.contig_end_exclusion, s->d_hist_top.p,
+                                   s->d_glob.p, (int)COV_K_HIST_COMPACT);
                 hipLaunchKernelGGL((k_hist_off<1>), dim3(hb), dim3(1024), 0, st, s->d_ctg.p, nT, s->d_tlen.p, mask, (u64)s->cfg.contig_end_exclusion, (const u64 *)s->d_hist_top.p, s->d_glob.p);
-                hipLaunchKernelGGL(k_hist_compact, dim3((nT + 3u) / 4u), dim3(256), 0, st, s->d_ctg.p, nT, s->d_tlen.p, (u64)s->cfg.contig_end_exclusion, s->d_arena.p, s->d_chist.p);
-                time_end(s, COV_K_HIST_COMPACT);
+                hipLaunchKernelGGL(k_hist_compact, dim3((nT + 3u) / 4u), dim3(256), 0, st, s->d_ctg.p, nT, s->d_tlen.p, (u64)s->cfg.contig_end_exclusion, s->d_arena.p, s->d_chist.p,
+                                   s->d_glob.p, (int)COV_K_HIST_COMPACT);
+                s->k_launches[COV_K_HIST_COMPACT]++;
                 HIPCHK(hipGetLastError());
                 const u64 guess = s->hist_fetch_seen ? std::min<u64>({s->last_chist_total + s->last_chist_total / 16, (u64)R + nT + 1, (u64)(64u << 20) / 8}) : 0;
                 if (guess) {
@@ -1160,16 +1172,15 @@
         s->h_ctg = (DevContig *)(s->h_res + sizeof(DevGlobal));
         s->h_estf = reinterpret_cast<float *>(s->h_res + block);
     }
-    if (want_id && R && nT) { HIPCHK(hipStreamWaitEvent(st, s->ev_side_done, 0)); s->ev_fresh = -1; }
+    if (want_id && R && nT) HIPCHK(hipStreamWaitEvent(st, s->ev_side_done, 0));
     if (nf) {
-        time_begin(s, COV_K_ESTIMATE);
         if (s->est_lanes < 0 ? nT >= 65536u : s->est_lanes == 1)
             hipLaunchKernelGGL(k_estimate_lanes, dim3((nT + 255) / 256), dim3(256), 0, st, (const DevContig *)s->d_ctg.p, nT, (const u32 *)s->d_tlen.p, (u64)s->cfg.contig_end_exclusion,
-                               (const u32 *)s->d_arena.p, s->est, reinterpret_cast<float *>(s->d_res.p + block));
+                               (const u32 *)s->d_arena.p, s->est, reinterpret_cast<float *>(s->d_res.p + block), s->d_glob.p, (int)COV_K_ESTIMATE);
         else
             hipLaunchKernelGGL(k_estimate, dim3((nT + 3) / 4), dim3(256), 0, st, (const DevContig *)s->d_ctg.p, nT, (const u32 *)s->d_tlen.p, (u64)s->cfg.contig_end_exclusion,
-                               (const u32 *)s->d_arena.p, s->est, reinterpret_cast<float *>(s->d_res.p + block));
-        time_end(s, COV_K_ESTIMATE);
+                               (const u32 *)s->d_arena.p, s->est, reinterpret_cast<float *>(s->d_res.p + block), s->d_glob.p, (int)COV_K_ESTIMATE);
+        s->k_launches[COV_K_ESTIMATE]++;
         HIPCHK(hipGetLastError());
     }
     const bool genomes = s->have_genomes && s->est.n != 0 && !s->spill.active && !s->in_spill;
@@ -1180,8 +1191,7 @@
         const u64 excl = s->cfg.contig_end_exclusion;
         const u64 ghist_cap = (u64)R + nT + 1;
         if (want_hist) HIPCHK(s->d_ghist.reserve((size_t)ghist_cap, st));
-        time_begin(s, COV_K_GENOME);
-        hipLaunchKernelGGL(k_genome_init, dim3((nG + 255u) / 256u), dim3(256), 0, st, s->d_genomes.p, nG);
+        hipLaunchKernelGGL(k_genome_init, dim3((nG + 255u) / 256u), dim3(256), 0, st, s->d_genomes.p, nG, s->d_glob.p, (int)COV_K_GENOME);
         if (n_seg) hipLaunchKernelGGL(k_genome_reduce, dim3((n_seg + 3u) / 4u), dim3(256), 0, st, (const DevContig *)s->d_ctg.p, (const u32 *)s->d_tlen.p, excl, gt, s->d_genomes.p);
         if (want_id && !(s->cfg.want & COV_WANT_IDENTITY_PRIMARY_ONLY))
             hipLaunchKernelGGL(k_genome_identity, dim3(nG), dim3(64), 0, st, (const DevContig *)s->d_ctg.p, gt, s->d_genomes.p);
@@ -1198,10 +1208,10 @@
         DevGenomeStats *gstats = reinterpret_cast<DevGenomeStats *>(s->d_gout.p);
         float *gest = reinterpret_cast<float *>(s->d_gout.p + (size_t)nG * sizeof(DevGenomeStats));
         if (nG >= 65536u)
-            hipLaunchKernelGGL(k_genome_estimate_lanes, dim3((nG + 255u) / 256u), dim3(256), 0, st, (const DevGenome *)s->d_genomes.p, nG, (const u64 *)s->d_ghist.p, s->est, gest, gstats);
+            hipLaunchKernelGGL(k_genome_estimate_lanes, dim3((nG + 255u) / 256u), dim3(256), 0, st, (const DevGenome *)s->d_genomes.p, nG, (const u64 *)s->d_ghist.p, s->est, gest, gstats, s->d_glob.p, (int)COV_K_GENOME);
         else
-            hipLaunchKernelGGL(k_genome_estimate, dim3((nG + 3u) / 4u), dim3(256), 0, st, (const DevGenome *)s->d_genomes.p, nG, (const u64 *)s->d_ghist.p, s->est, gest, gstats);
-        time_end(s, COV_K_GENOME);
+            hipLaunchKernelGGL(k_genome_estimate, dim3((nG + 3u) / 4u), dim3(256), 0, st, (const DevGenome *)s->d_genomes.p, nG, (const u64 *)s->d_ghist.p, s->est, gest, gstats, s->d_glob.p, (int)COV_K_GENOME);
+        s->k_launches[COV_K_GENOME]++;
         HIPCHK(hipGetLastError());
         HIPCHK(hipMemcpyAsync(s->h_gout, s->d_gout.p, (size_t)nG * (sizeof(DevGenomeStats) + s->est.n * sizeof(float)), hipMemcpyDeviceToHost, st));
     }
@@ -1228,6 +1238,7 @@
         }
     }
     HIPCHK(hipStreamSynchronize(st));
+    HostStamp hs("finish_once behind the synchronise");
     memcpy(&s->h_glob, s->h_res, sizeof(DevGlobal));
     if (s->h_glob.cx_total > s->d_cx_runs.cap) {
         const uint64_t need = s->h_glob.cx_total + s->h_glob.cx_total / 8 + 1024;
@@ -1236,8 +1247,11 @@
         again = true;
         return COV_OK;
     }
-    for (int k = 0; k < COV_K_COUNT; k++)
-        if (s->k_launches[k]) (void)hipEventElapsedTime(&s->k_ms[k], k == COV_K_IDENTITY ? s->ev[k][0] : s->ev_begin[k], s->ev[k][1]);
+    for (int k = 0; k <= COV_K_GENOME; k++)
+        if (s->k_launches[k]) {
+            if (k == COV_K_IDENTITY) (void)hipEventElapsedTime(&s->k_ms[k], s->ev_identity[0], s->ev_identity[1]);
+            else s->k_ms[k] = stamped_ms(s, s->h_glob, k);
+        }
 
     {
         const uint64_t ncig = s->adopted ? s->adopted_ncig : s->n_cigar;
@@ -1251,10 +1265,11 @@
         s->last_chist_total = 0; s->hist_compacted = false; s->est_valid = false; s->gen_valid = true; s->finished = true;
         return COV_OK;
     }
+    cov_summary own_summary;
+    if (!summary) summary = &own_summary;
     const cov_status cst = convert_results(s, s->h_glob, s->h_ctg, R, stats, summary, s->spill.inflight, s->spill.records);
     if (cst != COV_OK) return cst;
-    s->last_chist_total = 0;
-    if (want_hist) for (u32 c = 0; c < nT; c++) s->last_chist_total += stats[c].hist_len;
+    s->last_chist_total = want_hist ? summary->hist_total : 0;
     s->hist_compacted = compacted;
     s->est_valid = s->est.n != 0 && !s->have_mask;
     s->gen_valid = genomes;
@@ -2314,7 +2329,7 @@
     s->grp_launches = 0;
     if (R < 2) return COV_OK;
     const bool mates = s->mates_valid == s->n_records && s->mates_valid != 0;
-    hipEvent_t *ev = s->ev[COV_K_GROUP];
+    hipEvent_t *ev = s->ev_group;
     hipEvent_t ev_mid[2] = {nullptr, nullptr};
     DevBuf<u32> d_flag, d_hist, d_key[2], d_idx[2]; DevBuf<u64> d_cnt;
     struct Rel { std::function<void()> f; ~Rel() { f(); } } rel{[&] {
@@ -2380,7 +2395,7 @@
         fprintf(stderr, "[covermhip] group: %u records, %u passes, %llu moved; order check %.3f ms, sort %.3f ms, gather %.3f ms\n", R, P, (unsigned long long)moved, s->grp_ms[1], s->grp_ms[2],
                 s->grp_ms[3]);
     if (n_moved) *n_moved = moved;
-    s->finished = false; s->depth_all_valid = false; s->ev_fresh = -1;
+    s->finished = false; s->depth_all_valid = false;
     return COV_OK;
 }
 
@@ -2467,10 +2482,10 @@
         const uint8_t *mask = s->have_mask ? (const uint8_t *)s->d_mask.p : (const uint8_t *)nullptr;
         const u32 hb = (s->n_targets + 1023u) / 1024u;
         HIPCHK(s->d_hist_top.reserve(hb, s->stream));
-        hipLaunchKernelGGL((k_hist_sum<1>), dim3(hb), dim3(1024), 0, s->stream, (const DevContig *)s->d_ctg.p, s->n_targets, s->d_tlen.p, mask, (u64)s->cfg.contig_end_exclusion, s->d_hist_top.p);
+        hipLaunchKernelGGL((k_hist_sum<1>), dim3(hb), dim3(1024), 0, s->stream, (const DevContig *)s->d_ctg.p, s->n_targets, s->d_tlen.p, mask, (u64)s->cfg.contig_end_exclusion, s->d_hist_top.p, s->d_glob.p, (int)TG_NONE);
         hipLaunchKernelGGL((k_hist_off<1>), dim3(hb), dim3(1024), 0, s->stream, s->d_ctg.p, s->n_targets, s->d_tlen.p, mask, (u64)s->cfg.contig_end_exclusion, (const u64 *)s->d_hist_top.p, s->d_glob.p);
         hipLaunchKernelGGL(k_hist_compact, dim3((s->n_targets + 3u) / 4u), dim3(256), 0, s->stream, s->d_ctg.p, s->n_targets, s->d_tlen.p,
-                           (u64)s->cfg.contig_end_exclusion, s->d_arena.p, s->d_chist.p);
+                           (u64)s->cfg.contig_end_exclusion, s->d_arena.p, s->d_chist.p, s->d_glob.p, (int)TG_NONE);
         HIPCHK(hipGetLastError());
         s->hist_prefetched = 0; s->hist_compacted = true;
     }
@@ -2656,6 +2671,7 @@
     if (s->have_mask) { s->err = "cov_fetch_estimates: with a target mask the entries are genomes: aggregate on the host"; return COV_ERR_STATE; }
     const size_t nf = (size_t)s->n_targets * s->est.n;
     if (nf && !out) return COV_ERR_INVALID_ARG;
+    HostStamp hs("cov_fetch_estimates");
     if (nf) memcpy(out, s->h_estf, nf * sizeof(float));
     return COV_OK;
 }
diff --git a/coverm_amd/csrc/genome_kernels.hip.h b/coverm_amd/csrc/genome_kernels.hip.h
--- a/coverm_amd/csrc/genome_kernels.hip.h
+++ b/coverm_amd/csrc/genome_kernels.hip.h
@@ -28,7 +28,8 @@
     u32 n_genomes, n_seg;
 };
 
-__global__ __launch_bounds__(256) void k_genome_init(DevGenome *__restrict__ G, u32 n_genomes) {
+__global__ __launch_bounds__(256) void k_genome_init(DevGenome *__restrict__ G, u32 n_genomes, DevGlobal *glob, int tg) {
+    stamp_begin(glob, tg);
     const u32 g = blockIdx.x * 256u + threadIdx.x;
     if (g >= n_genomes) return;
     DevGenome z{};
@@ -209,12 +210,14 @@
     }
 }
 __global__ __launch_bounds__(256) void k_genome_estimate(const DevGenome *__restrict__ G, u32 n_genomes, const u64 *__restrict__ ghist, EstParams P,
-                                                         float *__restrict__ out, DevGenomeStats *__restrict__ stats) {
+                                                         float *__restrict__ out, DevGenomeStats *__restrict__ stats, DevGlobal *glob, int tg) {
     genome_estimate_body<false>(G, n_genomes, ghist, P, out, stats);
+    stamp_end(glob, tg);
 }
 __global__ __launch_bounds__(256) void k_genome_estimate_lanes(const DevGenome *__restrict__ G, u32 n_genomes, const u64 *__restrict__ ghist, EstParams P,
-                                                               float *__restrict__ out, DevGenomeStats *__restrict__ stats) {
+                                                               float *__restrict__ out, DevGenomeStats *__restrict__ stats, DevGlobal *glob, int tg) {
     genome_estimate_body<true>(G, n_genomes, ghist, P, out, stats);
-}
-
-}
+    stamp_end(glob, tg);
+}
+
+}
diff --git a/coverm_amd/csrc/pileup_kernels.hip.h b/coverm_amd/csrc/pileup_kernels.hip.h
--- a/coverm_amd/csrc/pileup_kernels.hip.h
+++ b/coverm_amd/csrc/pileup_kernels.hip.h
@@ -32,6 +32,9 @@
 static_assert(sizeof(DevContig) == 160, "DevContig layout");
 
 constexpr u32 COUNTER_SLOTS = 64;
+constexpr int TG_NONE = -1, TG_PREP = 0, TG_RANGES = 1, TG_PILEUP = 2, TG_HIST = 4, TG_HIST_COMPACT = 5, TG_ESTIMATE = 6, TG_GENOME = 7;
+constexpr u32 STAMP_GROUPS = 8, STAMP_LINES = 64;
+constexpr u32 TICKET_SCAN = 0;
 struct DevGlobal {
     u64 first_error;
     u64 hist_cap_total;
@@ -44,8 +47,11 @@
     u64 pad2[2];
     u64 prim_slots[COUNTER_SLOTS * 8];
     u64 cons_slots[COUNTER_SLOTS * 8];
-    u32 pad_q[8 * 16];
+    u64 t_begin[STAMP_GROUPS];
+    u32 ticket[16];
+    u64 t_end[STAMP_LINES * STAMP_GROUPS];
 };
+static_assert(sizeof(DevGlobal) % 64 == 0, "DevGlobal: DevContig behind it stays line-aligned");
 
 struct FilterCfg {
     u32 include_improper_pairs, include_supplementary, include_secondary;
@@ -126,6 +132,18 @@
 __device__ __forceinline__ u64 bcast_u64(u64 v, int q) {
     const u32 lo = __builtin_amdgcn_readlane((u32)v, q), hi = __builtin_amdgcn_readlane((u32)(v >> 32), q);
     return ((u64)hi << 32) | lo;
+}
+
+__device__ __forceinline__ void stamp_begin(DevGlobal *g, int k) {
+    if (k >= 0 && blockIdx.x == 0 && threadIdx.x == 0) g->t_begin[k] = wall_clock64();
+}
+__device__ __forceinline__ void stamp_end(DevGlobal *g, int k) {
+    if (k < 0) return;
+    __syncthreads();
+    if (threadIdx.x == 0) atomicMax(&g->t_end[(blockIdx.x & (STAMP_LINES - 1u)) * STAMP_GROUPS + (u32)k], (u64)wall_clock64());
+}
+__device__ __forceinline__ void stamp_end_wave(DevGlobal *g, int k) {
+    if (k >= 0 && lane_id() == 0) atomicMax(&g->t_end[(blockIdx.x & (STAMP_LINES - 1u)) * STAMP_GROUPS + (u32)k], (u64)wall_clock64());
 }
 
 __device__ __forceinline__ void report_error(DevGlobal *g, u32 rec, u32 code) {
@@ -179,6 +197,9 @@
         g->first_error = ~0ull; g->hist_cap_total = 0; g->chist_total = 0; g->internal_error = 0;
         g->n_cx = 0; g->cx_total = 0; g->n_slow = 0; g->n_gen = 0;
     }
+    if (c < STAMP_GROUPS) g->t_begin[c] = 0;
+    if (c < 16u) g->ticket[c] = 0u;
+    if (c < STAMP_LINES * STAMP_GROUPS) g->t_end[c] = 0;
     if (c < COUNTER_SLOTS * 8) { g->prim_slots[c] = 0; g->cons_slots[c] = 0; }
     if (c >= n_targets) return;
     DevContig z;
@@ -659,6 +680,7 @@
                                                      FilterCfg f, DevContig *ctg, DevGlobal *g, uint2 *__restrict__ runs,                        \
                                                      double *__restrict__ identp, double *__restrict__ identn, PrepPartial *__restrict__ part,   \
                                                      TileIdx ti, int passes, int b_active, u32 *__restrict__ cx_list, u32 cx_list_cap) {         \
+        stamp_begin(g, TG_PREP);                                                                                                                 \
         prep_body<WANT_IDENTITY, FILTER, MASKED, PF, PB>(r, tlen, n_targets, mask, f, ctg, g, runs, identp, identn, part, ti, passes, b_active, cx_list, \
                                                  cx_list_cap);                                                                                   \
     }
@@ -696,8 +718,10 @@
 }
 
 struct ScanPair { const u32 *cnt[2]; u32 *scan[2]; u32 *top[2]; u64 *total[2]; };
-__global__ __launch_bounds__(1024) void k_tile_scan1(ScanPair sp, u32 n_tiles, u32 n_blocks) {
+__global__ __launch_bounds__(1024) void k_tile_scan(ScanPair sp, u32 n_tiles, u32 n_blocks, DevGlobal *g, int tg) {
     __shared__ u32 wtot[16];
+    __shared__ u32 carry_s, last_s;
+    stamp_begin(g, tg);
     const u32 which = blockIdx.x >= n_blocks ? 1u : 0u, blk = blockIdx.x - which * n_blocks;
     const u32 *__restrict__ tcnt = sp.cnt[which];
     const u32 t = blk * 1024u + threadIdx.x;
@@ -709,20 +733,20 @@
     u32 wbase = 0, tot = 0;
     for (int k = 0; k < 16; k++) { const u32 x = wtot[k]; if (k < w) wbase += x; tot += x; }
     if (t < n_tiles) sp.scan[which][t] = wbase + inc - v;
-    if (threadIdx.x == 0) sp.top[which][blk] = tot;
-}
-
-__global__ __launch_bounds__(1024) void k_tile_scan2(ScanPair sp, u32 n_blocks) {
-    __shared__ u32 wtot[16];
-    __shared__ u32 carry_s;
-    u32 *ttop = sp.top[blockIdx.x];
-    u64 *total = sp.total[blockIdx.x];
-    if (threadIdx.x == 0) carry_s = 0;
+    if (threadIdx.x == 0) {
+        sp.top[which][blk] = tot;
+        __threadfence();
+        last_s = atomicAdd(&g->ticket[TICKET_SCAN + which], 1u) == n_blocks - 1u ? 1u : 0u;
+        carry_s = 0;
+    }
     __syncthreads();
-    const int lane = lane_id(), w = threadIdx.x >> 6;
+    if (!last_s) return;
+    __threadfence();
+    u32 *ttop = sp.top[which];
+    u64 *total = sp.total[which];
     for (u32 base = 0; base < n_blocks; base += 1024u) {
         const u32 b = base + threadIdx.x;
-        const u32 v = b < n_blocks ? ttop[b] : 0u;
+        const u32 v = b < n_blocks ? __hip_atomic_load(&ttop[b], __ATOMIC_RELAXED, __HIP_MEMORY_SCOPE_AGENT) : 0u;
         const u32 inc = (u32)wave_incl_scan((int)v);
         if (lane == 63) wtot[w] = inc;
         __syncthreads();
@@ -784,23 +808,19 @@
     }
 }
 
-template <bool FILL>
-__global__ __launch_bounds__(256) void k_cx_expand(Records r, const u32 *__restrict__ tlen, DevGlobal *g, CxIdx cx, TileIdx ti) {
-    cx_expand_body<FILL>(r, tlen, g, cx, ti, blockIdx.x * 4u + (threadIdx.x >> 6), gridDim.x * 4u);
-}
-
 __global__ __launch_bounds__(256) void k_post_prep(Records r, const u32 *__restrict__ tlen, DevGlobal *g, CxIdx cx, TileIdx ti, DevContig *ctg, u32 n_targets,
-                                                   const PrepPartial *__restrict__ part, u32 n_parts, u32 chunk_recs, u32 n_red) {
+                                                   const PrepPartial *__restrict__ part, u32 n_parts, u32 chunk_recs, u32 n_red, int tg) {
     if (blockIdx.x < n_red) prep_reduce_body(blockIdx.x * 4u + (threadIdx.x >> 6), ctg, n_targets, part, n_parts, chunk_recs);
     else cx_expand_body<false>(r, tlen, g, cx, ti, (blockIdx.x - n_red) * 4u + (threadIdx.x >> 6), (gridDim.x - n_red) * 4u);
+    stamp_end(g, tg);
 }
 
 template <bool WANT_HIST>
-__global__ __launch_bounds__(256) void k_ranges(const u32 *__restrict__ tile_contig, const u32 *__restrict__ tile_start,
-                                                u32 n_tiles, const u32 *__restrict__ tlen, const uint8_t *__restrict__ mask,
-                                                DevContig *ctg, uint4 *__restrict__ desc, TileIdx ti,
-                                                const u32 *__restrict__ tscan, const u32 *__restrict__ ttop, CxIdx cx,
-                                                DevGlobal *__restrict__ g, u32 *__restrict__ slow_list) {
+__device__ __forceinline__ void ranges_body(const u32 *__restrict__ tile_contig, const u32 *__restrict__ tile_start,
+                                            u32 n_tiles, const u32 *__restrict__ tlen, const uint8_t *__restrict__ mask,
+                                            DevContig *ctg, uint4 *__restrict__ desc, const TileIdx &ti,
+                                            const u32 *__restrict__ tscan, const u32 *__restrict__ ttop, const CxIdx &cx,
+                                            DevGlobal *g, u32 *__restrict__ slow_list) {
     const u32 t = blockIdx.x * blockDim.x + threadIdx.x;
     if (t >= n_tiles) return;
     const u32 c = tile_contig[t];
@@ -840,6 +860,16 @@
     desc[2 * t] = out;
     desc[2 * t + 1] = make_uint4(c, tile_start[t], cxo, cxn);
 }
+template <bool WANT_HIST>
+__global__ __launch_bounds__(256) void k_ranges(const u32 *__restrict__ tile_contig, const u32 *__restrict__ tile_start,
+                                                u32 n_tiles, const u32 *__restrict__ tlen, const uint8_t *__restrict__ mask,
+                                                DevContig *ctg, uint4 *__restrict__ desc, TileIdx ti,
+                                                const u32 *__restrict__ tscan, const u32 *__restrict__ ttop, CxIdx cx,
+                                                DevGlobal *g, u32 *__restrict__ slow_list, Records r, u32 n_rb, int tg) {
+    if (blockIdx.x < n_rb) ranges_body<WANT_HIST>(tile_contig, tile_start, n_tiles, tlen, mask, ctg, desc, ti, tscan, ttop, cx, g, slow_list);
+    else cx_expand_body<true>(r, tlen, g, cx, ti, (blockIdx.x - n_rb) * 4u + (threadIdx.x >> 6), (gridDim.x - n_rb) * 4u);
+    stamp_end(g, tg);
+}
 
 template <int MODE>
 __device__ __forceinline__ u64 hist_bins_of(const DevContig *C, u32 c, const u32 *__restrict__ tlen, const uint8_t *__restrict__ mask, u64 excl) {
@@ -864,8 +894,9 @@
 }
 template <int MODE>
 __global__ __launch_bounds__(1024) void k_hist_sum(const DevContig *__restrict__ ctg, u32 n_targets, const u32 *__restrict__ tlen,
-                                                   const uint8_t *__restrict__ mask, u64 excl, u64 *__restrict__ top) {
+                                                   const uint8_t *__restrict__ mask, u64 excl, u64 *__restrict__ top, DevGlobal *g, int tg) {
     __shared__ u64 wtot[16];
+    stamp_begin(g, tg);
     const u32 c = blockIdx.x * 1024u + threadIdx.x;
     u64 total;
     (void)block_incl_scan_u64(c < n_targets ? hist_bins_of<MODE>(&ctg[c], c, tlen, mask, excl) : 0, wtot, total);
@@ -891,25 +922,43 @@
     }
 }
 
-__global__ void k_zero_u32(u32 *__restrict__ p, const u64 *__restrict__ n_ptr) {
+constexpr u32 HIST_LAYOUT_MAX_BLOCKS = 64;
+__global__ __launch_bounds__(1024) void k_hist_layout(DevContig *ctg, u32 n_targets, const u32 *__restrict__ tlen, const uint8_t *__restrict__ mask,
+                                                      u64 excl, DevGlobal *g, int tg) {
+    __shared__ u64 wtot[16];
+    stamp_begin(g, tg);
+    u64 mine = 0, base;
+    for (u32 k = threadIdx.x; k < blockIdx.x * 1024u; k += 1024u) mine += hist_bins_of<0>(&ctg[k], k, tlen, mask, excl);
+    (void)block_incl_scan_u64(mine, wtot, base);
+    const u32 c = blockIdx.x * 1024u + threadIdx.x;
+    const u64 v = c < n_targets ? hist_bins_of<0>(&ctg[c], c, tlen, mask, excl) : 0;
+    u64 total;
+    const u64 inc = block_incl_scan_u64(v, wtot, total);
+    if (c < n_targets) ctg[c].hist_off = base + inc - v;
+    if (blockIdx.x == gridDim.x - 1 && threadIdx.x == 0) g->hist_cap_total = base + total;
+}
+
+__global__ void k_zero_u32(u32 *__restrict__ p, const u64 *__restrict__ n_ptr, DevGlobal *g, int tg) {
     const u64 n = *n_ptr;
     for (u64 i = (u64)blockIdx.x * blockDim.x + threadIdx.x; i < n; i += (u64)gridDim.x * blockDim.x) p[i] = 0u;
+    stamp_end(g, tg);
 }
 
 __global__ __launch_bounds__(256) void k_hist_compact(const DevContig *__restrict__ ctg, u32 n_targets,
                                                       const u32 *__restrict__ tlen, u64 excl,
-                                                      const u32 *__restrict__ arena, u64 *__restrict__ out) {
+                                                      const u32 *__restrict__ arena, u64 *__restrict__ out, DevGlobal *g, int tg) {
     const u32 c = blockIdx.x * 4u + (threadIdx.x >> 6);
-    if (c >= n_targets) return;
-    const DevContig *C = &ctg[c];
-    const u32 n = C->hist_len;
-    if (n == 0) return;
-    const u64 win_len = (u64)tlen[c] - 2 * excl;
-    for (u32 d = threadIdx.x & 63u; d < n; d += 64u) {
-        u64 v = arena[C->hist_off + d];
-        if (d == 0) v += win_len - C->proc_win;
-        out[C->chist_off + d] = v;
-    }
+    const DevContig *C = &ctg[min(c, n_targets - 1u)];
+    const u32 n = c < n_targets ? C->hist_len : 0u;
+    if (n != 0) {
+        const u64 win_len = (u64)tlen[c] - 2 * excl;
+        for (u32 d = threadIdx.x & 63u; d < n; d += 64u) {
+            u64 v = arena[C->hist_off + d];
+            if (d == 0) v += win_len - C->proc_win;
+            out[C->chist_off + d] = v;
+        }
+    }
+    stamp_end(g, tg);
 }
 
 __global__ __launch_bounds__(64) void k_identity(DevContig *ctg, u32 n_targets, const double *__restrict__ identp,
@@ -1185,6 +1234,7 @@
     int32_t *depth_out;
     const u64 *depth_off;
     u32 tile_base;
+    int t_group;
 };
 
 
@@ -1195,6 +1245,7 @@
 template <bool WANT_HIST, bool WRITE_DEPTH>
 __global__ __launch_bounds__(256) void k_pileup_stream(PileupArgs a, u32 n_tiles, u32 chunk_tiles,
                                                        const u32 *__restrict__ tile_list, const u32 *__restrict__ n_list) {
+    if (tile_list == nullptr) stamp_begin(a.g, a.t_group);
     if (tile_list != nullptr) n_tiles = *n_list;
     constexpr int TW = STREAM_TW, HBW = STREAM_HB, CAP = STREAM_CAP, ROWS = TW / 64;
     extern __shared__ __attribute__((aligned(16))) char smem[];
@@ -1401,6 +1452,7 @@
         cur_c = -1;
         ch = ch_next;
     }
+    stamp_end_wave(a.g, a.t_group);
 }
 
 constexpr size_t pileup_stream_smem_bytes() { return (size_t)4 * ((size_t)STREAM_TW * 4 + STREAM_HB * 4); }
@@ -1870,12 +1922,16 @@
     (void)estimate_entry<LANES, u32>(E, arena + C->hist_off, in, touched, P, o);
 }
 __global__ __launch_bounds__(256) void k_estimate(const DevContig *__restrict__ ctg, u32 n_targets, const u32 *__restrict__ tlen, u64 excl,
-                                                  const u32 *__restrict__ arena, EstParams P, float *__restrict__ out) {
+                                                  const u32 *__restrict__ arena, EstParams P, float *__restrict__ out, DevGlobal *g, int tg) {
+    stamp_begin(g, tg);
     estimate_body<false>(ctg, n_targets, tlen, excl, arena, P, out);
+    stamp_end(g, tg);
 }
 __global__ __launch_bounds__(256) void k_estimate_lanes(const DevContig *__restrict__ ctg, u32 n_targets, const u32 *__restrict__ tlen, u64 excl,
-                                                        const u32 *__restrict__ arena, EstParams P, float *__restrict__ out) {
+                                                        const u32 *__restrict__ arena, EstParams P, float *__restrict__ out, DevGlobal *g, int tg) {
+    stamp_begin(g, tg);
     estimate_body<true>(ctg, n_targets, tlen, excl, arena, P, out);
+    stamp_end(g, tg);
 }
 
 struct DevInterval { u32 tid, pad; u64 start, end; };
diff --git a/coverm_amd/csrc/prep_lean.hip.h b/coverm_amd/csrc/prep_lean.hip.h
--- a/coverm_amd/csrc/prep_lean.hip.h
+++ b/coverm_amd/csrc/prep_lean.hip.h
@@ -498,10 +498,12 @@
 
 template <bool WANT_IDENTITY, bool FILTER, bool MASKED>
 __global__ __launch_bounds__(256) __attribute__((amdgpu_waves_per_eu(8, 8))) void k_prep_lean(PrepHot h, const PrepArgs *__restrict__ pa) {
+    stamp_begin(pa->cold.g, TG_PREP);
     prep_lean_body<WANT_IDENTITY, FILTER, MASKED>(h, pa);
 }
 template <bool WANT_IDENTITY, bool FILTER, bool MASKED>
 __global__ __launch_bounds__(256) void k_prep_generic(const PrepArgs *__restrict__ pa, u32 all_steps) {
+    if (all_steps) stamp_begin(pa->cold.g, TG_PREP);
     const u32 n = all_steps ? all_steps : pa->cold.g->n_gen;
     const u32 *__restrict__ list = pa->cold.gen_list;
     for (u32 j = blockIdx.x * 4u + (threadIdx.x >> 6); j < n; j += gridDim.x * 4u) {
```
